# Crowsinc/LiveVisionKit

Measured on AMD Instinct MI355X. Metric: stabilized frames/sec (one 4K YUV420 stream per GPU, steady state), higher is better.
Workload: dtype f32

## Files before the change

include/lvk_hip.h:

```cpp
#ifndef LVK_HIP_H
#define LVK_HIP_H

#include <stdint.h>
#include <stddef.h>

#ifdef __cplusplus
extern "C" {
#endif

#define LVK_HIP_OK              0
#define LVK_HIP_ERR_ARG        -1
#define LVK_HIP_ERR_RUNTIME    -2
#define LVK_HIP_ERR_NO_DEVICE  -3

typedef struct lvk_hip_ctx lvk_hip_ctx;


int  lvk_hip_ctx_create(int device, lvk_hip_ctx** out);
int  lvk_hip_ctx_create_on_stream(int device, void* hip_stream, lvk_hip_ctx** out);
void lvk_hip_ctx_destroy(lvk_hip_ctx* ctx);
int  lvk_hip_sync(lvk_hip_ctx* ctx);
void* lvk_hip_stream(lvk_hip_ctx* ctx);
const char* lvk_hip_last_error(lvk_hip_ctx* ctx);
const char* lvk_hip_version(void);
// ... 154 lines not shown
int  lvk_hip_stab_push_yuv420_host(lvk_hip_stab* stab, const void* h_y, int y_step, const void* h_u, int u_step, const void* h_v, int v_step, int nv12,
                                   int rows, int cols, uint64_t timestamp,
                                   void* oh_y, int oy_step, void* oh_u, int ou_step, void* oh_v, int ov_step, int o_rows,
                                   int* produced, uint64_t* out_timestamp, lvk_frame_info* emitted);
int  lvk_hip_stab_push_obs_host(lvk_hip_stab* stab, int video_format,
                                const void* const h_planes[3], const int steps[3], int rows, int cols, uint64_t timestamp,
                                void* const oh_planes[3], const int o_steps[3], int o_rows,
                                int* produced, uint64_t* out_timestamp, lvk_frame_info* emitted);
int  lvk_hip_stab_prefetch_yuv420_host(lvk_hip_stab* stab, const void* h_y, int y_step, const void* h_u, int u_step, const void* h_v, int v_step,
                                       int nv12, int rows, int cols);
int  lvk_hip_stab_prefetch_cancel(lvk_hip_stab* stab);
int  lvk_hip_stab_set_overlap(lvk_hip_stab* stab, int enable);
int  lvk_hip_stab_set_bulk_context(lvk_hip_stab* stab, lvk_hip_ctx* bulk);
void* lvk_hip_stab_output_stream(lvk_hip_stab* stab);
int  lvk_hip_stab_set_remap_precision(lvk_hip_stab* stab, int precision);
int  lvk_hip_stab_get_remap_precision(const lvk_hip_stab* stab);


typedef struct lvk_deblock_settings
{
    uint32_t detection_levels;
    uint32_t block_size;
    uint32_t filter_size;
    float filter_scaling;
} lvk_deblock_settings;

typedef struct lvk_hip_deblock lvk_hip_deblock;

void lvk_hip_deblock_default_settings(lvk_deblock_settings* s);
int  lvk_hip_deblock_create(lvk_hip_ctx* ctx, const lvk_deblock_settings* settings, lvk_hip_deblock** out);
int  lvk_hip_deblock_configure(lvk_hip_deblock* deb, const lvk_deblock_settings* settings);
void lvk_hip_deblock_destroy(lvk_hip_deblock* deb);
int  lvk_hip_deblock_apply(lvk_hip_deblock* deb, void* d_frame, int step, int rows, int cols, int format, int region_xywh[4]);
int  lvk_hip_deblock_draw_influence(const lvk_hip_deblock* deb, void* d_frame, int step, int rows, int cols, int format);
int  lvk_hip_deblock_filter_region(const lvk_hip_deblock* deb, int region_xywh[4]);

int  lvk_hip_cas(lvk_hip_ctx* ctx, const void* d_src, int src_step, int rows, int cols, int format, void* d_dst, int dst_step, float sharpness);

int  lvk_hip_reformat(lvk_hip_ctx* ctx, const void* d_src, int src_step, int rows, int cols, int src_format, void* d_dst, int dst_step,
                      int dst_format);

int  lvk_hip_fsr_easu(lvk_hip_ctx* ctx, const void* d_src, int src_step, int rows, int cols, int format, const int region_xywh[4], void* d_dst,
                      int dst_step, int out_rows, int out_cols);
int  lvk_hip_fsr_geometry(int rows, int cols, int out_rows, int out_cols, float multiplier, int maintain_aspect_ratio, const int crop_ltrb[4],
                          int region_xywh[4], int out_rows_cols[2], int* skip);
int  lvk_hip_text_size(const char* text, int scale, int thickness, int wh[2], int* baseline);



int  lvk_hip_stab_prefetch(lvk_hip_stab* stab, const void* d_frame, int step, int rows, int cols, int format);
int  lvk_hip_stab_prefetch_yuv420(lvk_hip_stab* stab, const void* d_y, int y_step, const void* d_u, int u_step, const void* d_v, int v_step,
                                  int nv12, int rows, int cols);
long long lvk_hip_stab_lookahead_frames(lvk_hip_stab* stab);

int lvk_hip_remap_homography_gray(lvk_hip_ctx* ctx, const void* d_src, int src_step, int src_rows, int src_cols,
                                  void* d_dst, int dst_step, int dst_rows, int dst_cols, int off_x, int off_y, const float H[9], uint8_t bg);
int lvk_hip_remap_mesh_gray(lvk_hip_ctx* ctx, const void* d_src, int src_step, int src_rows, int src_cols, void* d_dst, int dst_step,
                            const float* mesh, int mesh_rows, int mesh_cols, uint8_t bg);
int lvk_hip_remap_map_gray(lvk_hip_ctx* ctx, const void* d_src, int src_step, int rows, int cols, void* d_dst, int dst_step,
                           const void* d_map, int map_step, uint8_t bg);
int lvk_hip_warpmesh_apply_gray(lvk_hip_ctx* ctx, const void* d_src, int src_step, int rows, int cols, void* d_dst, int dst_step,
                                const float* mesh, int mesh_rows, int mesh_cols, uint8_t bg);
int lvk_hip_warpmesh_apply_lens_gray(lvk_hip_ctx* ctx, const void* d_src, int src_step, int rows, int cols, void* d_dst, int dst_step,
                                     const float* mesh, int mesh_rows, int mesh_cols, uint8_t bg, const lvk_camera_params* lens);
int  lvk_hip_stab_push_gray(lvk_hip_stab* stab, const void* d_frame, int step, int rows, int cols, uint64_t timestamp,
                            void* d_out, int out_step, int out_rows, int* produced, uint64_t* out_timestamp, const void** released,
                            lvk_frame_info* emitted);
int  lvk_hip_stab_push_gray_host(lvk_hip_stab* stab, const void* h_frame, int step, int rows, int cols, uint64_t timestamp,
                                 void* oh_out, int out_step, int out_rows, int* produced, uint64_t* out_timestamp, lvk_frame_info* emitted);

int lvk_hip_remap_homography_c4(lvk_hip_ctx* ctx, const void* d_src, int src_step, int src_rows, int src_cols,
                                void* d_dst, int dst_step, int dst_rows, int dst_cols, int off_x, int off_y, const float H[9], const uint8_t bg[4]);
int lvk_hip_remap_mesh_c4(lvk_hip_ctx* ctx, const void* d_src, int src_step, int src_rows, int src_cols, void* d_dst, int dst_step,
                          const float* mesh, int mesh_rows, int mesh_cols, const uint8_t bg[4]);
int lvk_hip_remap_map_c4(lvk_hip_ctx* ctx, const void* d_src, int src_step, int rows, int cols, void* d_dst, int dst_step,
                         const void* d_map, int map_step, const uint8_t bg[4]);
int lvk_hip_warpmesh_apply_c4(lvk_hip_ctx* ctx, const void* d_src, int src_step, int rows, int cols, void* d_dst, int dst_step,
                              const float* mesh, int mesh_rows, int mesh_cols, const uint8_t bg[4]);
int lvk_hip_warpmesh_apply_lens_c4(lvk_hip_ctx* ctx, const void* d_src, int src_step, int rows, int cols, void* d_dst, int dst_step,
                                   const float* mesh, int mesh_rows, int mesh_cols, const uint8_t bg[4], const lvk_camera_params* lens);
int  lvk_hip_stab_set_background_alpha(lvk_hip_stab* stab, int alpha);
int  lvk_hip_stab_push_c4(lvk_hip_stab* stab, const void* d_frame, int step, int rows, int cols, uint64_t timestamp, int format,
                          void* d_out, int out_step, int out_rows, int* produced, uint64_t* out_timestamp, const void** released,
                          lvk_frame_info* emitted);
int  lvk_hip_stab_push_c4_host(lvk_hip_stab* stab, const void* h_frame, int step, int rows, int cols, uint64_t timestamp, int format,
                               void* oh_out, int out_step, int out_rows, int* produced, uint64_t* out_timestamp, lvk_frame_info* emitted);

int lvk_hip_upscale_gray(lvk_hip_ctx* ctx, const void* d_src, int src_step, int src_rows, int src_cols, void* d_dst, int dst_step, int dst_rows, int dst_cols);
int lvk_hip_upscale_c4(lvk_hip_ctx* ctx, const void* d_src, int src_step, int src_rows, int src_cols, void* d_dst, int dst_step, int dst_rows, int dst_cols);
int lvk_hip_sharpen_gray(lvk_hip_ctx* ctx, const void* d_src, int src_step, int rows, int cols, void* d_dst, int dst_step, float sharpness);
int lvk_hip_sharpen_c4(lvk_hip_ctx* ctx, const void* d_src, int src_step, int rows, int cols, void* d_dst, int dst_step, float sharpness);

int lvk_hip_cas_gray(lvk_hip_ctx* ctx, const void* d_src, int src_step, int rows, int cols, void* d_dst, int dst_step, float sharpness);
int lvk_hip_fsr_easu_gray(lvk_hip_ctx* ctx, const void* d_src, int src_step, int rows, int cols, const int region_xywh[4],
                          void* d_dst, int dst_step, int out_rows, int out_cols);
int lvk_hip_fsr_easu_gray_path(int rw, int rh, int out_rows, int out_cols);


#define LVK_SCHED_PUSH_FREE_RUNNING   0
#define LVK_SCHED_PUSH_SYNCHRONISED   1
#define LVK_SCHED_INGEST_ON_TRACKER   2
#define LVK_SCHED_INGEST_ON_BULK      3
#define LVK_SCHED_INGEST_INLINE       4
#define LVK_SCHED_REMAP_PERSISTENT    5
#define LVK_SCHED_REMAP_FULL          6
#define LVK_SCHED_WAIT_SIGNAL_WORD    7
#define LVK_SCHED_WAIT_EVENT          8
#define LVK_SCHED_WAIT_WORD_TIMEOUT   9
#define LVK_SCHED_COUNT              10
int  lvk_hip_stab_schedule_counters(lvk_hip_stab* stab, long long out[LVK_SCHED_COUNT], int reset);

int  lvk_hip_stab_get_stats(const lvk_hip_stab* stab, lvk_stab_stats* out);
int  lvk_hip_stab_detector_frames(const lvk_hip_stab* stab, long long* on_device, long long* on_host);
int  lvk_hip_stab_get_meshes(const lvk_hip_stab* stab, float* motion, float* correction, int cap_floats);
int  lvk_hip_stab_get_features(const lvk_hip_stab* stab, float* xy_resp_age, int cap);


#define LVK_STAGE_DOWNSCALE 0
#define LVK_STAGE_PYRAMID   1
#define LVK_STAGE_FAST      2
#define LVK_STAGE_PYRLK     3
#define LVK_STAGE_MOTION    4
#define LVK_STAGE_REMAP     5
#define LVK_STAGE_INGEST    6
#define LVK_STAGE_EGRESS    7
#define LVK_STAGE_COUNT     8
int  lvk_hip_stab_set_profiling(lvk_hip_stab* stab, int enable);
int  lvk_hip_stab_get_profile(lvk_hip_stab* stab, double total_ms[LVK_STAGE_COUNT], long long launches[LVK_STAGE_COUNT]);

int lvk_hip_native_rcp(lvk_hip_ctx* ctx, const float* d_in, float* d_out, size_t n);

typedef struct lvk_hip_mesh_solver lvk_hip_mesh_solver;
int  lvk_hip_mesh_solver_create(lvk_hip_ctx* ctx, int cols, int rows, float gen_region_w, float gen_region_h,
                                float temporal_smoothing, float local_smoothing, int max_points, lvk_hip_mesh_solver** out);
void lvk_hip_mesh_solver_destroy(lvk_hip_mesh_solver* solver);
int  lvk_hip_mesh_solver_reset(lvk_hip_mesh_solver* solver);
int  lvk_hip_mesh_solver_solve(lvk_hip_mesh_solver* solver, const float* tracked, const float* matched, int n, float region_w, float region_h,
                               float temporal_now, float threshold, uint8_t* inliers, float* offsets);

int lvk_hip_luma_area_resize(lvk_hip_ctx* ctx, const void* d_src, int src_step, int pix_stride, int channel,
                             int srows, int scols, void* d_dst, int dst_step, int drows, int dcols);

int lvk_hip_pyr_down(lvk_hip_ctx* ctx, const void* d_src, int src_step, int rows, int cols, void* d_dst, int dst_step);
int lvk_hip_scharr(lvk_hip_ctx* ctx, const void* d_src, int src_step, int rows, int cols, void* d_dst);

int lvk_hip_build_pyramid(lvk_hip_ctx* ctx, const void* d_img, int step, int rows, int cols, int max_level, int win_w, int win_h,
                          uint8_t* levels, int16_t* derivs, int* level_rows, int* level_cols);

int lvk_hip_fast_detect(lvk_hip_ctx* ctx, const void* d_img, int step, int rows, int cols,
                        const int* regions, int nregions, uint32_t* out, int cap, int* counts);

int lvk_hip_pyrlk(lvk_hip_ctx* ctx, const void* d_prev, int prev_step, const void* d_next, int next_step, int rows, int cols,
                  const float* prev_pts, int n, float* next_pts, uint8_t* status,
                  int win_w, int win_h, int max_level, int max_count, double epsilon, double min_eig_threshold);

int lvk_hip_estimate_global_motion(lvk_hip_ctx* ctx, const float* pts1, const float* pts2, int n, double threshold,
                                   double region_w, double region_h, int full_homography, double H[9], uint8_t* mask);

int lvk_hip_estimate_global_motion_lo(lvk_hip_ctx* ctx, const float* pts1, const float* pts2, int n, double threshold,
                                      double region_w, double region_h, int full_homography, int lo_mode, double H[9], uint8_t* mask,
                                      int lo_info[2]);

int lvk_hip_fast_filter(lvk_hip_ctx* ctx, const float* prev, const float* matched, const uint8_t* status, int n, float* out_prev, float* out_matched);

#define LVK_TRACK_CHAIN_GUARD 64
#define LVK_TRACK_CHAIN_FILL  0xA5
typedef struct lvk_track_chain_desc
{
    const float* prev; const float* matched; const uint8_t* status; const float* und;
    const void* d_prev_img; int prev_step; const void* d_next_img; int next_step; int rows, cols;
    int win_w, win_h, max_level, max_count; double epsilon, min_eig;
    const lvk_camera_params* lens; int lens_rows, lens_cols; double lens_sx, lens_sy;
    int n_bound, count_on_device, n_word;
    int full, model_on_device, full_word;
    int separate_compact, host_signal;
    double threshold; int region_w, region_h;
} lvk_track_chain_desc;
typedef struct lvk_track_chain_result
{
    double H[9]; int rc, signalled, count_dev, count_host;
    uint8_t* mask; float* pairs_dev; float* mirror_matched; uint8_t* mirror_status;
    float* next_pts; uint8_t* flow_status; float* flow_und;
} lvk_track_chain_result;
int lvk_hip_track_chain(lvk_hip_ctx* ctx, const lvk_track_chain_desc* desc, lvk_track_chain_result* result);

int lvk_hip_deblock_get_grid(lvk_hip_deblock* deb, uint8_t* mean, uint8_t* grid, float* keep_block, int capacity, int extent_xy[2]);


int lvk_hip_cas_const(float sharpness, float* peak);

int lvk_hip_cvt_code_target(int code, int src_format, int dcn);

int lvk_hip_fsr_easu_const(int rw, int rh, int W, int H, int ow, int oh, float con[16]);

int lvk_hip_fsr_easu_path(int rw, int rh, int out_rows, int out_cols);

enum
{
    LVK_AREA_PATH_FAST_DW_8x8_C3_BGR = 0, LVK_AREA_PATH_FAST_DW_8x8_C3_RGB = 1, LVK_AREA_PATH_FAST_DW_4x4_C3_BGR = 2, LVK_AREA_PATH_FAST_DW_4x4_C3_RGB = 3,
    LVK_AREA_PATH_FAST_DW_8x8_C3 = 4, LVK_AREA_PATH_FAST_DW_4x4_C3 = 5, LVK_AREA_PATH_FAST_DW_8x8_C1 = 6, LVK_AREA_PATH_FAST_DW_4x4_C1 = 7,
    LVK_AREA_PATH_FAST = 8, LVK_AREA_PATH_TILE_4 = 9, LVK_AREA_PATH_TILE_8 = 10, LVK_AREA_PATH_TAPS_4 = 11, LVK_AREA_PATH_TAPS_8 = 12,
    LVK_AREA_PATH_GENERAL = 13, LVK_AREA_PATH_ENLARGE = 14, LVK_AREA_PATH_COUNT = 15
};
int lvk_hip_area_resize_path(lvk_hip_ctx* ctx, const void* d_src, int src_step, int pix_stride, int channel,
// ... 25 lines not shown
```

livevisionkit_amd/_native.py:

```python
import ctypes
import os

_HERE = os.path.dirname(os.path.abspath(__file__))
LIB_PATH = os.environ.get("LVK_HIP_LIB") or os.path.join(_HERE, "liblvk_hip.so")

_c = ctypes
_P = _c.c_void_p
_SIG = {
    "lvk_hip_ctx_create": (_c.c_int, [_c.c_int, _c.POINTER(_P)]),
    "lvk_hip_ctx_create_on_stream": (_c.c_int, [_c.c_int, _P, _c.POINTER(_P)]),
    "lvk_hip_ctx_destroy": (None, [_P]),
    "lvk_hip_sync": (_c.c_int, [_P]),
    "lvk_hip_stream": (_P, [_P]),
    "lvk_hip_last_error": (_c.c_char_p, [_P]),
    "lvk_hip_version": (_c.c_char_p, []),
    "lvk_hip_abi_version": (_c.c_int, []),
    "lvk_hip_device_count": (_c.c_int, []),
    "lvk_hip_device_usable": (_c.c_int, [_c.c_int]),
    "lvk_hip_malloc": (_c.c_int, [_P, _c.c_size_t, _c.POINTER(_P)]),
    "lvk_hip_free": (_c.c_int, [_P, _P]),
    "lvk_hip_trim": (_c.c_int, [_P]),
    "lvk_hip_ctx_wait": (_c.c_int, [_P, _P]),
    "lvk_hip_upload": (_c.c_int, [_P, _P, _P, _c.c_size_t]),
    "lvk_hip_download": (_c.c_int, [_P, _P, _P, _c.c_size_t]),
# ... 17 lines not shown
    "lvk_hip_stab_set_remap_precision": (_c.c_int, [_P, _c.c_int]),
    "lvk_hip_stab_get_remap_precision": (_c.c_int, [_P]),
    "lvk_hip_remap_homography_c4": (_c.c_int, [_P, _P, _c.c_int, _c.c_int, _c.c_int, _P, _c.c_int, _c.c_int, _c.c_int,
                                               _c.c_int, _c.c_int, _c.POINTER(_c.c_float), _c.POINTER(_c.c_uint8)]),
    "lvk_hip_remap_mesh_c4": (_c.c_int, [_P, _P, _c.c_int, _c.c_int, _c.c_int, _P, _c.c_int, _c.POINTER(_c.c_float), _c.c_int, _c.c_int, _c.POINTER(_c.c_uint8)]),
    "lvk_hip_remap_map_c4": (_c.c_int, [_P, _P, _c.c_int, _c.c_int, _c.c_int, _P, _c.c_int, _P, _c.c_int, _c.POINTER(_c.c_uint8)]),
    "lvk_hip_warpmesh_apply_c4": (_c.c_int, [_P, _P, _c.c_int, _c.c_int, _c.c_int, _P, _c.c_int, _c.POINTER(_c.c_float), _c.c_int, _c.c_int, _c.POINTER(_c.c_uint8)]),
    "lvk_hip_warpmesh_apply_lens_c4": (_c.c_int, [_P, _P, _c.c_int, _c.c_int, _c.c_int, _P, _c.c_int, _c.POINTER(_c.c_float), _c.c_int, _c.c_int, _c.POINTER(_c.c_uint8), _P]),
    "lvk_hip_stab_set_background_alpha": (_c.c_int, [_P, _c.c_int]),
    "lvk_hip_stab_push_c4": (_c.c_int, [_P, _P, _c.c_int, _c.c_int, _c.c_int, _c.c_uint64, _c.c_int, _P, _c.c_int, _c.c_int,
                                        _c.POINTER(_c.c_int), _c.POINTER(_c.c_uint64), _c.POINTER(_P), _P]),
    "lvk_hip_stab_push_c4_host": (_c.c_int, [_P, _P, _c.c_int, _c.c_int, _c.c_int, _c.c_uint64, _c.c_int, _P, _c.c_int, _c.c_int,
                                             _c.POINTER(_c.c_int), _c.POINTER(_c.c_uint64), _P]),
    "lvk_hip_upscale": (_c.c_int, [_P, _P, _c.c_int, _c.c_int, _c.c_int, _P, _c.c_int, _c.c_int, _c.c_int, _c.c_int]),
    "lvk_hip_sharpen": (_c.c_int, [_P, _P, _c.c_int, _c.c_int, _c.c_int, _P, _c.c_int, _c.c_float]),
    "lvk_hip_upscale_gray": (_c.c_int, [_P, _P, _c.c_int, _c.c_int, _c.c_int, _P, _c.c_int, _c.c_int, _c.c_int]),
    "lvk_hip_upscale_c4": (_c.c_int, [_P, _P, _c.c_int, _c.c_int, _c.c_int, _P, _c.c_int, _c.c_int, _c.c_int]),
    "lvk_hip_sharpen_gray": (_c.c_int, [_P, _P, _c.c_int, _c.c_int, _c.c_int, _P, _c.c_int, _c.c_float]),
    "lvk_hip_sharpen_c4": (_c.c_int, [_P, _P, _c.c_int, _c.c_int, _c.c_int, _P, _c.c_int, _c.c_float]),
    "lvk_hip_native_rcp": (_c.c_int, [_P, _P, _P, _c.c_size_t]),
    "lvk_hip_mesh_solver_create": (_c.c_int, [_P, _c.c_int, _c.c_int, _c.c_float, _c.c_float, _c.c_float, _c.c_float, _c.c_int, _c.POINTER(_P)]),
    "lvk_hip_mesh_solver_destroy": (None, [_P]),
    "lvk_hip_mesh_solver_reset": (_c.c_int, [_P]),
    "lvk_hip_mesh_solver_solve": (_c.c_int, [_P, _c.POINTER(_c.c_float), _c.POINTER(_c.c_float), _c.c_int, _c.c_float, _c.c_float, _c.c_float, _c.c_float,
                                             _c.POINTER(_c.c_uint8), _c.POINTER(_c.c_float)]),
    "lvk_hip_lens_map_create": (_c.c_int, [_P, _P, _c.c_int, _c.c_int, _c.POINTER(_P), _c.POINTER(_c.c_int)]),
    "lvk_hip_lens_map_destroy": (_c.c_int, [_P, _P]),
    "lvk_hip_warpmesh_apply_lens": (_c.c_int, [_P, _P, _c.c_int, _c.c_int, _c.c_int, _P, _c.c_int, _c.POINTER(_c.c_float), _c.c_int, _c.c_int, _c.POINTER(_c.c_uint8), _c.c_int, _P]),
    "lvk_hip_lens_undistort_points": (_c.c_int, [_P, _P, _c.c_int, _c.c_int, _c.c_double, _c.c_double, _c.POINTER(_c.c_float), _c.c_int, _c.POINTER(_c.c_float)]),
    "lvk_hip_stab_set_lens": (_c.c_int, [_P, _P]),
    "lvk_hip_stab_output_stream": (_P, [_P]),
    "lvk_hip_fast_filter": (_c.c_int, [_P, _c.POINTER(_c.c_float), _c.POINTER(_c.c_float), _c.POINTER(_c.c_uint8), _c.c_int, _c.POINTER(_c.c_float), _c.POINTER(_c.c_float)]),
    "lvk_hip_stab_draw_trackers": (_c.c_int, [_P]),
    "lvk_hip_stab_draw_motion_mesh": (_c.c_int, [_P]),
    "lvk_hip_draw_grid": (_c.c_int, [_P, _P, _c.c_int, _c.c_int, _c.c_int, _c.c_int, _c.c_int, _c.POINTER(_c.c_uint8), _c.c_int]),
    "lvk_hip_draw_crosses": (_c.c_int, [_P, _P, _c.c_int, _c.c_int, _c.c_int, _c.POINTER(_c.c_float), _c.c_int, _c.c_float, _c.c_float,
                                        _c.POINTER(_c.c_uint8), _c.c_int, _c.c_int]),
    "lvk_hip_draw_points": (_c.c_int, [_P, _P, _c.c_int, _c.c_int, _c.c_int, _c.POINTER(_c.c_float), _c.c_int, _c.c_float, _c.c_float,
                                       _c.POINTER(_c.c_uint8), _c.c_int]),
    "lvk_hip_draw_rect": (_c.c_int, [_P, _P, _c.c_int, _c.c_int, _c.c_int, _c.POINTER(_c.c_int), _c.POINTER(_c.c_uint8), _c.c_int]),
    "lvk_hip_draw_text": (_c.c_int, [_P, _P, _c.c_int, _c.c_int, _c.c_int, _c.c_char_p, _c.c_int, _c.c_int, _c.POINTER(_c.c_uint8), _c.c_int, _c.c_int]),
    "lvk_hip_text_size": (_c.c_int, [_c.c_char_p, _c.c_int, _c.c_int, _c.POINTER(_c.c_int), _c.POINTER(_c.c_int)]),
    "lvk_hip_warpmesh_apply_yuv420": (_c.c_int, [_P, _P, _c.c_int, _c.c_int, _c.c_int, _P, _c.c_int, _P, _c.c_int, _P, _c.c_int, _c.c_int,
                                                 _c.POINTER(_c.c_float), _c.c_int, _c.c_int, _c.POINTER(_c.c_uint8)]),
    "lvk_hip_warpmesh_apply": (_c.c_int, [_P, _P, _c.c_int, _c.c_int, _c.c_int, _P, _c.c_int,
                                          _c.POINTER(_c.c_float), _c.c_int, _c.c_int, _c.POINTER(_c.c_uint8), _c.c_int]),
    "lvk_hip_luma_area_resize": (_c.c_int, [_P, _P, _c.c_int, _c.c_int, _c.c_int, _c.c_int, _c.c_int, _P, _c.c_int, _c.c_int, _c.c_int]),
    "lvk_hip_pyr_down": (_c.c_int, [_P, _P, _c.c_int, _c.c_int, _c.c_int, _P, _c.c_int]),
    "lvk_hip_scharr": (_c.c_int, [_P, _P, _c.c_int, _c.c_int, _c.c_int, _P]),
    "lvk_hip_build_pyramid": (_c.c_int, [_P, _P, _c.c_int, _c.c_int, _c.c_int, _c.c_int, _c.c_int, _c.c_int,
                                         _c.POINTER(_c.c_uint8), _c.POINTER(_c.c_int16), _c.POINTER(_c.c_int), _c.POINTER(_c.c_int)]),
    "lvk_hip_fast_detect": (_c.c_int, [_P, _P, _c.c_int, _c.c_int, _c.c_int, _c.POINTER(_c.c_int), _c.c_int,
                                       _c.POINTER(_c.c_uint32), _c.c_int, _c.POINTER(_c.c_int)]),
    "lvk_hip_pyrlk": (_c.c_int, [_P, _P, _c.c_int, _P, _c.c_int, _c.c_int, _c.c_int, _c.POINTER(_c.c_float), _c.c_int,
                                 _c.POINTER(_c.c_float), _c.POINTER(_c.c_uint8), _c.c_int, _c.c_int, _c.c_int, _c.c_int,
                                 _c.c_double, _c.c_double]),
    "lvk_hip_ingest_yuv420": (_c.c_int, [_P, _P, _c.c_int, _P, _c.c_int, _P, _c.c_int, _c.c_int, _c.c_int, _c.c_int, _P, _c.c_int]),
    "lvk_hip_egress_yuv420": (_c.c_int, [_P, _P, _c.c_int, _c.c_int, _c.c_int, _P, _c.c_int, _P, _c.c_int, _P, _c.c_int, _c.c_int]),
    "lvk_hip_ingest_obs": (_c.c_int, [_P, _c.c_int, _P * 3, _c.c_int * 3, _c.c_int, _c.c_int, _P, _c.c_int]),
    "lvk_hip_egress_obs": (_c.c_int, [_P, _c.c_int, _P, _c.c_int, _c.c_int, _c.c_int, _P * 3, _c.c_int * 3]),
    "lvk_hip_obs_frame_format": (_c.c_int, [_c.c_int]),
    "lvk_hip_estimate_global_motion": (_c.c_int, [_P, _c.POINTER(_c.c_float), _c.POINTER(_c.c_float), _c.c_int, _c.c_double,
                                                  _c.c_double, _c.c_double, _c.c_int, _c.POINTER(_c.c_double), _c.POINTER(_c.c_uint8)]),
    "lvk_hip_estimate_global_motion_lo": (_c.c_int, [_P, _c.POINTER(_c.c_float), _c.POINTER(_c.c_float), _c.c_int, _c.c_double,
                                                     _c.c_double, _c.c_double, _c.c_int, _c.c_int, _c.POINTER(_c.c_double), _c.POINTER(_c.c_uint8),
                                                     _c.POINTER(_c.c_int)]),
    "lvk_hip_track_chain": (_c.c_int, [_P, _P, _P]),
    "lvk_stab_default_settings": (None, [_P]),
    "lvk_hip_stab_create": (_c.c_int, [_P, _P, _c.POINTER(_P)]),
    "lvk_hip_stab_destroy": (None, [_P]),
    "lvk_hip_stab_configure": (_c.c_int, [_P, _P]),
    "lvk_hip_stab_restart": (_c.c_int, [_P]),
    "lvk_hip_stab_reset_context": (_c.c_int, [_P]),
    "lvk_hip_stab_ready": (_c.c_int, [_P]),
    "lvk_hip_stab_frame_delay": (_c.c_int, [_P]),
    "lvk_hip_stab_stable_region": (_c.c_int, [_P, _c.c_int, _c.c_int, _c.POINTER(_c.c_int)]),
    "lvk_hip_stab_next_output": (_c.c_int, [_P, _c.c_int, _c.c_int, _c.c_int, _P]),
    "lvk_hip_stab_push": (_c.c_int, [_P, _P, _c.c_int, _c.c_int, _c.c_int, _c.c_uint64, _c.c_int, _P, _c.c_int, _c.c_int,
                                     _c.POINTER(_c.c_int), _c.POINTER(_c.c_uint64), _c.POINTER(_P), _P]),
    "lvk_hip_stab_push_yuv420": (_c.c_int, [_P, _P, _c.c_int, _P, _c.c_int, _P, _c.c_int, _c.c_int, _c.c_int, _c.c_int, _c.c_uint64,
                                            _P, _c.c_int, _P, _c.c_int, _P, _c.c_int, _c.c_int, _c.POINTER(_c.c_int), _c.POINTER(_c.c_uint64), _P]),
    "lvk_hip_stab_push_obs": (_c.c_int, [_P, _c.c_int, _P * 3, _c.c_int * 3, _c.c_int, _c.c_int, _c.c_uint64, _P * 3, _c.c_int * 3, _c.c_int,
                                         _c.POINTER(_c.c_int), _c.POINTER(_c.c_uint64), _P]),
    "lvk_hip_stab_push_yuv420_host": (_c.c_int, [_P, _P, _c.c_int, _P, _c.c_int, _P, _c.c_int, _c.c_int, _c.c_int, _c.c_int, _c.c_uint64,
                                            _P, _c.c_int, _P, _c.c_int, _P, _c.c_int, _c.c_int, _c.POINTER(_c.c_int), _c.POINTER(_c.c_uint64), _P]),
    "lvk_hip_stab_push_obs_host": (_c.c_int, [_P, _c.c_int, _P * 3, _c.c_int * 3, _c.c_int, _c.c_int, _c.c_uint64, _P * 3, _c.c_int * 3, _c.c_int,
                                              _c.POINTER(_c.c_int), _c.POINTER(_c.c_uint64), _P]),
    "lvk_hip_stab_prefetch_yuv420_host": (_c.c_int, [_P, _P, _c.c_int, _P, _c.c_int, _P, _c.c_int, _c.c_int, _c.c_int, _c.c_int]),
    "lvk_hip_stab_prefetch_cancel": (_c.c_int, [_P]),
    "lvk_hip_stab_prefetch": (_c.c_int, [_P, _P, _c.c_int, _c.c_int, _c.c_int, _c.c_int]),
    "lvk_hip_stab_prefetch_yuv420": (_c.c_int, [_P, _P, _c.c_int, _P, _c.c_int, _P, _c.c_int, _c.c_int, _c.c_int, _c.c_int]),
    "lvk_hip_stab_lookahead_frames": (_c.c_longlong, [_P]),
    "lvk_hip_stab_schedule_counters": (_c.c_int, [_P, _c.POINTER(_c.c_longlong), _c.c_int]),
    "lvk_hip_stab_detector_frames": (_c.c_int, [_P, _c.POINTER(_c.c_longlong), _c.POINTER(_c.c_longlong)]),
    "lvk_hip_host_malloc": (_c.c_int, [_P, _c.c_size_t, _c.POINTER(_P)]),
    "lvk_hip_host_free": (_c.c_int, [_P, _P]),
    "lvk_hip_stab_get_stats": (_c.c_int, [_P, _P]),
    "lvk_hip_stab_get_meshes": (_c.c_int, [_P, _c.POINTER(_c.c_float), _c.POINTER(_c.c_float), _c.c_int]),
    "lvk_hip_stab_get_features": (_c.c_int, [_P, _c.POINTER(_c.c_float), _c.c_int]),
    "lvk_hip_stab_set_overlap": (_c.c_int, [_P, _c.c_int]),
    "lvk_hip_stab_set_bulk_context": (_c.c_int, [_P, _P]),
    "lvk_hip_stab_set_profiling": (_c.c_int, [_P, _c.c_int]),
    "lvk_hip_stab_get_profile": (_c.c_int, [_P, _c.POINTER(_c.c_double), _c.POINTER(_c.c_longlong)]),
    "lvk_hip_deblock_default_settings": (None, [_P]),
    "lvk_hip_deblock_create": (_c.c_int, [_P, _P, _c.POINTER(_P)]),
    "lvk_hip_deblock_configure": (_c.c_int, [_P, _P]),
    "lvk_hip_deblock_destroy": (None, [_P]),
    "lvk_hip_deblock_apply": (_c.c_int, [_P, _P, _c.c_int, _c.c_int, _c.c_int, _c.c_int, _c.POINTER(_c.c_int)]),
    "lvk_hip_deblock_draw_influence": (_c.c_int, [_P, _P, _c.c_int, _c.c_int, _c.c_int, _c.c_int]),
    "lvk_hip_deblock_filter_region": (_c.c_int, [_P, _c.POINTER(_c.c_int)]),
    "lvk_hip_deblock_get_grid": (_c.c_int, [_P, _c.POINTER(_c.c_uint8), _c.POINTER(_c.c_uint8), _c.POINTER(_c.c_float), _c.c_int, _c.POINTER(_c.c_int)]),
    "lvk_hip_cas": (_c.c_int, [_P, _P, _c.c_int, _c.c_int, _c.c_int, _c.c_int, _P, _c.c_int, _c.c_float]),
    "lvk_hip_cas_const": (_c.c_int, [_c.c_float, _c.POINTER(_c.c_float)]),
    "lvk_hip_reformat": (_c.c_int, [_P, _P, _c.c_int, _c.c_int, _c.c_int, _c.c_int, _P, _c.c_int, _c.c_int]),
    "lvk_hip_cvt_code_target": (_c.c_int, [_c.c_int, _c.c_int, _c.c_int]),
    "lvk_hip_fsr_easu": (_c.c_int, [_P, _P, _c.c_int, _c.c_int, _c.c_int, _c.c_int, _c.POINTER(_c.c_int), _P, _c.c_int, _c.c_int, _c.c_int]),
    "lvk_hip_fsr_geometry": (_c.c_int, [_c.c_int, _c.c_int, _c.c_int, _c.c_int, _c.c_float, _c.c_int, _c.POINTER(_c.c_int), _c.POINTER(_c.c_int),
                                        _c.POINTER(_c.c_int), _c.POINTER(_c.c_int)]),
    "lvk_hip_fsr_easu_const": (_c.c_int, [_c.c_int, _c.c_int, _c.c_int, _c.c_int, _c.c_int, _c.c_int, _c.POINTER(_c.c_float)]),
    "lvk_hip_fsr_easu_path": (_c.c_int, [_c.c_int, _c.c_int, _c.c_int, _c.c_int]),
    "lvk_hip_cas_gray": (_c.c_int, [_P, _P, _c.c_int, _c.c_int, _c.c_int, _P, _c.c_int, _c.c_float]),
    "lvk_hip_fsr_easu_gray": (_c.c_int, [_P, _P, _c.c_int, _c.c_int, _c.c_int, _c.POINTER(_c.c_int), _P, _c.c_int, _c.c_int, _c.c_int]),
    "lvk_hip_fsr_easu_gray_path": (_c.c_int, [_c.c_int, _c.c_int, _c.c_int, _c.c_int]),
    "lvk_hip_area_resize_path": (_c.c_int, [_P, _P, _c.c_int, _c.c_int, _c.c_int, _c.c_int, _c.c_int, _c.c_int, _c.c_int]),
    "lvk_hip_remap_map_yuv420": (_c.c_int, [_P, _P, _c.c_int, _c.c_int, _c.c_int, _P, _c.c_int, _P, _c.c_int, _P, _c.c_int, _c.c_int,
                                            _P, _c.c_int, _c.POINTER(_c.c_uint8)]),
    "lvk_hip_lens_create": (_c.c_int, [_P, _P, _c.c_int, _c.POINTER(_P)]),
    "lvk_hip_lens_configure": (_c.c_int, [_P, _P, _c.c_int]),
    "lvk_hip_lens_destroy": (None, [_P]),
    "lvk_hip_lens_view": (_c.c_int, [_P, _c.c_int, _c.c_int, _c.POINTER(_c.c_int)]),
    "lvk_hip_lens_apply": (_c.c_int, [_P, _P, _c.c_int, _c.c_int, _c.c_int, _c.c_int, _P, _c.c_int]),
    "lvk_hip_lens_apply_gray": (_c.c_int, [_P, _P, _c.c_int, _c.c_int, _c.c_int, _P, _c.c_int]),
    "lvk_hip_lens_apply_c4": (_c.c_int, [_P, _P, _c.c_int, _c.c_int, _c.c_int, _c.c_int, _P, _c.c_int]),
    "lvk_hip_lens_apply_yuv420": (_c.c_int, [_P, _P, _c.c_int, _P, _c.c_int, _P, _c.c_int, _P, _c.c_int, _P, _c.c_int, _P, _c.c_int,
                                             _c.c_int, _c.c_int, _c.c_int]),
}

_SIG_DEBLOCK_PX = {
    "lvk_hip_deblock_apply_gray": (_c.c_int, [_P, _P, _c.c_int, _c.c_int, _c.c_int, _c.POINTER(_c.c_int)]),
    "lvk_hip_deblock_apply_c4": (_c.c_int, [_P, _P, _c.c_int, _c.c_int, _c.c_int, _c.c_int, _c.POINTER(_c.c_int)]),
}

_SIG_DEBLOCK_420 = {
    "lvk_hip_deblock_apply_yuv420": (_c.c_int, [_P, _P, _c.c_int, _P, _c.c_int, _P, _c.c_int, _P, _c.c_int, _P, _c.c_int, _P, _c.c_int,
                                                _c.c_int, _c.c_int, _c.c_int, _c.POINTER(_c.c_int)]),
# ... 43 lines not shown
```

livevisionkit_amd/context.py:

```python
import ctypes

import numpy as np

from . import _native


class LvkHipError(RuntimeError):
    pass


def _f32(a):
    a = np.ascontiguousarray(a, dtype=np.float32)
    return a, a.ctypes.data_as(ctypes.POINTER(ctypes.c_float))


def _u8x3(bg):
    a = np.ascontiguousarray(bg, dtype=np.uint8).reshape(3)
    return a, a.ctypes.data_as(ctypes.POINTER(ctypes.c_uint8))


def _u8x4(bg):
    a = np.ascontiguousarray(bg, dtype=np.uint8).reshape(4)
    return a, a.ctypes.data_as(ctypes.POINTER(ctypes.c_uint8))

# ... 190 lines not shown
        return out

    def area_resize_path(self, frame, drows, dcols, channel=0):
        pix = frame.shape[2] if frame.dim() == 3 else 1
        path = self.lib.lvk_hip_area_resize_path(self.handle, frame.data_ptr(), frame.stride(0), pix, channel, frame.shape[0], frame.shape[1], drows, dcols)
        self._check(min(path, 0))
        return path

    def pyr_down(self, img, out=None):
        import torch
        if out is None:
            out = torch.empty(((img.shape[0] + 1) // 2, (img.shape[1] + 1) // 2), dtype=torch.uint8, device=img.device)
        self._check(self.lib.lvk_hip_pyr_down(self.handle, img.data_ptr(), img.stride(0), img.shape[0], img.shape[1],
                                              out.data_ptr(), out.stride(0)))
        return out

    def scharr(self, img, out=None):
        import torch
        if out is None:
            out = torch.empty((img.shape[0], img.shape[1], 2), dtype=torch.int16, device=img.device)
        self._check(self.lib.lvk_hip_scharr(self.handle, img.data_ptr(), img.stride(0), img.shape[0], img.shape[1], out.data_ptr()))
        return out

    def build_pyramid(self, img, max_level=3, win=(11, 11)):
        rows, cols = img.shape
        lv = np.zeros(rows * cols * 2, np.uint8); dv = np.zeros(rows * cols * 4, np.int16)
        lr = np.zeros(8, np.int32); lc = np.zeros(8, np.int32)
        n = self.lib.lvk_hip_build_pyramid(self.handle, img.data_ptr(), img.stride(0), rows, cols, max_level, win[0], win[1],
                                           lv.ctypes.data_as(ctypes.POINTER(ctypes.c_uint8)), dv.ctypes.data_as(ctypes.POINTER(ctypes.c_int16)),
                                           lr.ctypes.data_as(ctypes.POINTER(ctypes.c_int)), lc.ctypes.data_as(ctypes.POINTER(ctypes.c_int)))
        self._check(min(n, 0))
        out, lo, do = [], 0, 0
        for i in range(n):
            r, c = int(lr[i]), int(lc[i])
            out.append((lv[lo:lo + r * c].reshape(r, c).copy(), dv[do:do + r * c * 2].reshape(r, c, 2).copy()))
            lo += r * c; do += r * c * 2
        return out

    def fast_detect(self, img, regions, cap=None):
        rg = np.ascontiguousarray(regions, dtype=np.int32).reshape(-1, 6)
        n = rg.shape[0]
        cap = cap or int(max(1, (rg[:, 2] * rg[:, 3]).max()))
        out = np.zeros((n, cap), np.uint32)
        counts = np.zeros(n, np.int32)
        self._check(self.lib.lvk_hip_fast_detect(self.handle, img.data_ptr(), img.stride(0), img.shape[0], img.shape[1],
                                                 rg.ctypes.data_as(ctypes.POINTER(ctypes.c_int)), n,
                                                 out.ctypes.data_as(ctypes.POINTER(ctypes.c_uint32)), cap,
                                                 counts.ctypes.data_as(ctypes.POINTER(ctypes.c_int))))
        res = []
        for i in range(n):
            e = out[i, :min(cap, counts[i])]
            res.append(np.stack([e & 0xFFF, (e >> 12) & 0xFFF, e >> 24], axis=1).astype(np.int32))
        return res, counts

    def pyrlk(self, prev, nxt, pts, win=(11, 11), max_level=3, max_count=5, epsilon=0.01, min_eig=1e-4):
        pts = np.ascontiguousarray(pts, np.float32).reshape(-1, 2)
        out = np.zeros_like(pts)
        st = np.zeros(len(pts), np.uint8)
        self._check(self.lib.lvk_hip_pyrlk(self.handle, prev.data_ptr(), prev.stride(0), nxt.data_ptr(), nxt.stride(0),
                                           prev.shape[0], prev.shape[1],
                                           pts.ctypes.data_as(ctypes.POINTER(ctypes.c_float)), len(pts),
                                           out.ctypes.data_as(ctypes.POINTER(ctypes.c_float)),
                                           st.ctypes.data_as(ctypes.POINTER(ctypes.c_uint8)),
                                           win[0], win[1], max_level, max_count, float(epsilon), float(min_eig)))
        return out, st

    def estimate_global_motion(self, p1, p2, threshold, region=(480, 270), full_homography=True):
        p1 = np.ascontiguousarray(p1, np.float32).reshape(-1, 2); p2 = np.ascontiguousarray(p2, np.float32).reshape(-1, 2)
        H = np.zeros(9, np.float64); mask = np.zeros(len(p1), np.uint8)
        rc = self.lib.lvk_hip_estimate_global_motion(self.handle, p1.ctypes.data_as(ctypes.POINTER(ctypes.c_float)),
                                                     p2.ctypes.data_as(ctypes.POINTER(ctypes.c_float)), len(p1), float(threshold),
                                                     float(region[0]), float(region[1]), 1 if full_homography else 0,
                                                     H.ctypes.data_as(ctypes.POINTER(ctypes.c_double)),
                                                     mask.ctypes.data_as(ctypes.POINTER(ctypes.c_uint8)))
        if rc in (-1, -2, -3):
            self._check(rc)
        return rc, H.reshape(3, 3), mask

    def estimate_global_motion_lo(self, p1, p2, threshold, lo_mode, region=(480, 270), full_homography=True):
        p1 = np.ascontiguousarray(p1, np.float32).reshape(-1, 2); p2 = np.ascontiguousarray(p2, np.float32).reshape(-1, 2)
        H = np.zeros(9, np.float64); mask = np.zeros(len(p1), np.uint8); info = (ctypes.c_int * 2)(-1, -1)
        rc = self.lib.lvk_hip_estimate_global_motion_lo(self.handle, p1.ctypes.data_as(ctypes.POINTER(ctypes.c_float)),
                                                        p2.ctypes.data_as(ctypes.POINTER(ctypes.c_float)), len(p1), float(threshold),
                                                        float(region[0]), float(region[1]), 1 if full_homography else 0, int(lo_mode),
                                                        H.ctypes.data_as(ctypes.POINTER(ctypes.c_double)),
                                                        mask.ctypes.data_as(ctypes.POINTER(ctypes.c_uint8)), info)
        if rc in (-1, -2, -3):
            self._check(rc)
        return rc, H.reshape(3, 3), mask, info[0], info[1]

    def ingest_yuv420(self, y, u, v=None, out=None):
        import torch
        rows, cols = y.shape
        if out is None:
            out = torch.empty((rows, cols, 3), dtype=torch.uint8, device=y.device)
        nv12 = v is None
        self._check(self.lib.lvk_hip_ingest_yuv420(self.handle, *_planes420_args((y, u, v), nv12), 1 if nv12 else 0, rows, cols, out.data_ptr(), out.stride(0)))
        return out

    def egress_yuv420(self, frame, nv12=False, out=None):
        rows, cols = frame.shape[:2]
        if out is None:
            out = _planes420_empty(rows, cols, nv12, frame.device)
        y, u, v = out if not nv12 else (out[0], out[1], None)
        self._check(self.lib.lvk_hip_egress_yuv420(self.handle, frame.data_ptr(), frame.stride(0), rows, cols, *_planes420_args((y, u, v), nv12), 1 if nv12 else 0))
        return (y, u) if nv12 else (y, u, v)
# ... 252 lines not shown
```

livevisionkit_amd/csrc/fast.hip:

```cpp
#include "lvk_hip_internal.hpp"

namespace {

constexpr int TW = 64, TH = 8;
constexpr int AP = 4;
constexpr int IW = TW + 2 * AP, IH = TH + 2 * AP;
constexpr int SW = TW + 2, SH = TH + 2;

__device__ __forceinline__ int fast_score(const uint8_t* c, int stride, int threshold)
{
    const int v = c[0];
    int d[16];
    d[0] = v - c[3 * stride];          d[1] = v - c[1 + 3 * stride];   d[2] = v - c[2 + 2 * stride];   d[3] = v - c[3 + stride];
    d[4] = v - c[3];                   d[5] = v - c[3 - stride];       d[6] = v - c[2 - 2 * stride];   d[7] = v - c[1 - 3 * stride];
    d[8] = v - c[-3 * stride];         d[9] = v - c[-1 - 3 * stride];  d[10] = v - c[-2 - 2 * stride]; d[11] = v - c[-3 - stride];
    d[12] = v - c[-3];                 d[13] = v - c[-3 + stride];     d[14] = v - c[-2 + 2 * stride]; d[15] = v - c[-1 + 3 * stride];
    int lo2[16], hi2[16], lo4[16], hi4[16];
#pragma unroll
    for (int k = 0; k < 16; k++) { lo2[k] = min(d[k], d[(k + 1) & 15]); hi2[k] = max(d[k], d[(k + 1) & 15]); }
#pragma unroll
    for (int k = 0; k < 16; k++) { lo4[k] = min(lo2[k], lo2[(k + 2) & 15]); hi4[k] = max(hi2[k], hi2[(k + 2) & 15]); }
    int dark = -256, bright_neg = 256;
#pragma unroll
    for (int k = 0; k < 16; k++)
    {
        const int lo9 = min(min(lo4[k], lo4[(k + 4) & 15]), d[(k + 8) & 15]);
        const int hi9 = max(max(hi4[k], hi4[(k + 4) & 15]), d[(k + 8) & 15]);
        dark = max(dark, lo9);
        bright_neg = min(bright_neg, hi9);
    }
    const int m = max(dark, -bright_neg);
    return m > threshold ? m - 1 : 0;
}

struct FastRegionList { FastRegion r[LVK_FAST_INLINE_REGIONS]; };

struct FastCells { const uint16_t* col_of; const uint32_t* row_base; uint32_t* first; unsigned long long* best; int* region_count; };

__global__ __launch_bounds__(TW * TH)
void k_fast_detect(const uint8_t* __restrict__ img, int step, int rows, int cols,
                   const FastRegion* __restrict__ regions, FastRegionList inl, int n_inline, int segs_x,
                   unsigned long long* __restrict__ masks, uint8_t* __restrict__ scores, int max_rh, int max_rw, FastCells cells)
{
    LVK_TRACKER_PRIORITY();
    const FastRegion rg = n_inline ? inl.r[blockIdx.z] : regions[blockIdx.z];
    if (!rg.active) return;
    const int lx0 = blockIdx.x * TW, ly0 = blockIdx.y * TH;
    if (lx0 >= rg.w || ly0 >= rg.h) return;

    __shared__ uint8_t s_img[IH][IW];
    __shared__ uint8_t s_score[SH][SW];
    const int tid = threadIdx.y * TW + threadIdx.x;

    for (int i = tid; i < IW * IH; i += TW * TH)
    {
        const int ty = i / IW, tx = i - ty * IW;
        const int gx = min(max(rg.x + lx0 - AP + tx, 0), cols - 1);
        const int gy = min(max(rg.y + ly0 - AP + ty, 0), rows - 1);
        s_img[ty][tx] = img[(long)gy * step + gx];
    }
    __shared__ uint32_t s_cell_col[TW], s_cell_row[TH];
    if (cells.first)
    {
        if (tid < TW) s_cell_col[tid] = cells.col_of[min(rg.x + lx0 + tid, cols - 1)];
        else if (tid < TW + TH) s_cell_row[tid - TW] = cells.row_base[min(rg.y + ly0 + tid - TW, rows - 1)];
    }
    __syncthreads();

    for (int i = tid; i < SW * SH; i += TW * TH)
    {
        const int ty = i / SW, tx = i - ty * SW;
        const int lx = lx0 - 1 + tx, ly = ly0 - 1 + ty;
        int s = 0;
        if (lx >= 3 && lx < rg.w - 3 && ly >= 3 && ly < rg.h - 3)
            s = fast_score(&s_img[ty + AP - 1][tx + AP - 1], IW, rg.threshold);
        s_score[ty][tx] = (uint8_t)s;
    }
    __syncthreads();

    const int lx = lx0 + threadIdx.x, ly = ly0 + threadIdx.y;
    const int sx = threadIdx.x + 1, sy = threadIdx.y + 1;
    const int s = s_score[sy][sx];
    const bool keep = s > 0 &&
        s > s_score[sy][sx - 1] && s > s_score[sy][sx + 1] &&
        s > s_score[sy - 1][sx - 1] && s > s_score[sy - 1][sx] && s > s_score[sy - 1][sx + 1] &&
        s > s_score[sy + 1][sx - 1] && s > s_score[sy + 1][sx] && s > s_score[sy + 1][sx + 1];
    const unsigned long long mask = __ballot(keep);
    if (ly < rg.h)
    {
        if (threadIdx.x == 0) masks[((long)blockIdx.z * max_rh + ly) * segs_x + blockIdx.x] = mask;
        if (threadIdx.x == 0 && cells.first && mask) atomicAdd(&cells.region_count[blockIdx.z], __popcll(mask));
        if (keep) scores[((long)blockIdx.z * max_rh + ly) * max_rw + lx] = (uint8_t)s;
        if (keep && cells.first)
        {
            const uint32_t ci = s_cell_row[threadIdx.y] + s_cell_col[threadIdx.x];
            const uint32_t key = (uint32_t)(((int)blockIdx.z * max_rh + ly) * max_rw + lx);
            atomicMin(&cells.first[ci], key);
            const uint32_t rec = (uint32_t)(rg.x + lx) | ((uint32_t)(rg.y + ly) << 12) | ((uint32_t)s << 24);
            atomicMax(&cells.best[ci], ((unsigned long long)(((uint32_t)s << 24) | (0xFFFFFFu - key)) << 32) | rec);
        }
    }
}

__global__ __launch_bounds__(1024)
void k_fast_compact(const FastRegion* __restrict__ regions, FastRegionList inl, int n_inline, int segs_x,
                    const unsigned long long* __restrict__ masks, const uint8_t* __restrict__ scores, int max_rh, int max_rw,
                    uint32_t* __restrict__ out, int cap, int* __restrict__ counts)
{
    LVK_TRACKER_PRIORITY();
    const int r = blockIdx.x;
    const FastRegion rg = n_inline ? inl.r[r] : regions[r];
    if (!rg.active) { if (threadIdx.x == 0) counts[r] = 0; return; }
    const int rsegs = (rg.w + TW - 1) / TW;
    const int nseg = rg.h * rsegs;
    __shared__ int s_wave[16];
    __shared__ int s_base;
    if (threadIdx.x == 0) s_base = 0;
    __syncthreads();
    const int lane = threadIdx.x & 63, wave = threadIdx.x >> 6;
    for (int chunk = 0; chunk < nseg; chunk += 1024)
    {
        const int seg = chunk + threadIdx.x;
        int ly = 0, sg = 0;
        unsigned long long m = 0;
        if (seg < nseg)
        {
            ly = seg / rsegs; sg = seg - ly * rsegs;
            m = masks[((long)r * max_rh + ly) * segs_x + sg];
        }
        const int cnt = __popcll(m);
        int incl = cnt;
#pragma unroll
        for (int o = 1; o < 64; o <<= 1) { const int t = __shfl_up(incl, o); if (lane >= o) incl += t; }
        if (lane == 63) s_wave[wave] = incl;
        __syncthreads();
        int wave_off = 0;
        for (int w = 0; w < wave; w++) wave_off += s_wave[w];
        int pos = s_base + wave_off + incl - cnt;
        while (m)
        {
            const int bit = __ffsll((long long)m) - 1;
            m &= m - 1;
            const int lx = sg * TW + bit;
            if (pos < cap)
                out[(long)r * cap + pos] = (uint32_t)lx | ((uint32_t)ly << 12) | ((uint32_t)scores[((long)r * max_rh + ly) * max_rw + lx] << 24);
            pos++;
        }
        __syncthreads();
        if (threadIdx.x == 1023) s_base = s_base + wave_off + incl;
        __syncthreads();
    }
    if (threadIdx.x == 0) counts[r] = s_base;
}


struct FastInsertArgs
{
    const uint8_t* bucket;
    uint32_t* first; unsigned long long* best;
    int* region_count;
    int capacity, small_grid, n_held, min_samples; float uniformity, homography_threshold;
    int nkeys;
    float2* pts;
    uint32_t* new_kp;
    int* result;
    int* d_n; int* d_full;
    int* counts;
    uint32_t occ[128];
    int occ_bucket[16];
};

constexpr int INS_NT = 1024, INS_MAX_CELLS = 4096, INS_CPT = INS_MAX_CELLS / INS_NT, INS_MAX_KEYS = 1 << 18;

__host__ __device__ inline size_t ins_lds_bytes(int nkeys) { const size_t words = ((size_t)nkeys + 31) / 32; return words * 4 + ((words + 1) & ~(size_t)1) * 2; }

__global__ __launch_bounds__(INS_NT)
void k_fast_insert(int nregions, FastInsertArgs a)
{
    LVK_TRACKER_PRIORITY();
    extern __shared__ __attribute__((aligned(16))) uint8_t ins_smem[];
    const int bwords = (a.nkeys + 31) / 32;
    uint32_t* s_bits = reinterpret_cast<uint32_t*>(ins_smem);
    unsigned short* s_pre = reinterpret_cast<unsigned short*>(s_bits + bwords);
    __shared__ int s_wave[INS_NT / 64], s_bucket[16], s_count[LVK_FAST_INLINE_REGIONS];
    __shared__ uint32_t s_occ[INS_MAX_CELLS / 32];
    const int t = threadIdx.x, lane = t & 63, wave = t >> 6;

    uint32_t f[INS_CPT]; unsigned long long bk[INS_CPT]; uint32_t bu[INS_CPT];
#pragma unroll
    for (int k = 0; k < INS_CPT; k++)
    {
        const int ci = t + k * INS_NT;
        f[k] = ci < a.capacity ? a.first[ci] : 0xFFFFFFFFu;
        bk[k] = ci < a.capacity ? a.best[ci] : 0ull;
        bu[k] = ci < a.capacity ? a.bucket[ci] : 0u;
    }
    const int my_count = t < nregions ? a.region_count[t] : 0;
#pragma unroll 1
    for (int i = t; i < bwords; i += INS_NT) s_bits[i] = 0u;
    if (t < INS_MAX_CELLS / 32) s_occ[t] = a.occ[t];
    if (t < LVK_FAST_INLINE_REGIONS) s_count[t] = my_count;
    if (t < nregions && my_count) a.region_count[t] = 0;
    if (t < 16) s_bucket[t] = a.occ_bucket[t];
    __syncthreads();

#pragma unroll
    for (int k = 0; k < INS_CPT; k++)
    {
        const int ci = t + k * INS_NT;
        if (ci < a.capacity && f[k] != 0xFFFFFFFFu)
        {
            a.first[ci] = 0xFFFFFFFFu; a.best[ci] = 0ull;
            if ((s_occ[ci >> 5] >> (ci & 31)) & 1u) f[k] = 0xFFFFFFFFu;
            else { atomicOr(&s_bits[f[k] >> 5], 1u << (f[k] & 31)); atomicAdd(&s_bucket[bu[k] & 15u], 1); }
        }
    }
    __syncthreads();
    const int wpt = (bwords + INS_NT - 1) / INS_NT, wb0 = t * wpt, wb1 = min(wb0 + wpt, bwords);
    int mine = 0;
#pragma unroll 1
    for (int w = wb0; w < wb1; w++) mine += __popc(s_bits[w]);
    int incl = mine;
#pragma unroll
    for (int o = 1; o < 64; o <<= 1) { const int u = __shfl_up(incl, o); if (lane >= o) incl += u; }
    if (lane == 63) s_wave[wave] = incl;
    __syncthreads();
    int base = 0, n_new = 0;
#pragma unroll 2
    for (int q = 0; q < INS_NT / 64; q++) { const int u = s_wave[q]; n_new += u; if (q < wave) base += u; }
    int run = base + incl - mine;
#pragma unroll 1
    for (int w = wb0; w < wb1; w++) { s_pre[w] = (unsigned short)run; run += __popc(s_bits[w]); }
    __syncthreads();

#pragma unroll
    for (int k = 0; k < INS_CPT; k++)
        if (f[k] != 0xFFFFFFFFu)
        {
            const uint32_t w = f[k] >> 5, bit = f[k] & 31;
            const int pos = (int)s_pre[w] + __popc(s_bits[w] & ((1u << bit) - 1u));
            const uint32_t rec = (uint32_t)bk[k];
            a.pts[a.n_held + pos] = make_float2((float)(rec & 0xFFFu), (float)((rec >> 12) & 0xFFFu));
            a.new_kp[pos] = rec;
        }

    if (t < nregions) a.counts[t] = s_count[t];
    if (t == 0)
    {
        int m_used = 0;
        for (int b = 0; b < 16; b++) m_used += s_bucket[b];
        float q = 1.0f;
        if (m_used != 0)
        {
            if (a.small_grid) q = (float)m_used / (float)a.capacity;
            else
            {
                const int ideal = (int)((float)m_used / 16.0f);
                int excess = 0;
                for (int b = 0; b < 16; b++) excess += max(s_bucket[b] - ideal, 0);
                q = 1.0f - ((float)excess / (float)(m_used - ideal));
            }
        }
        int total = 0;
        for (int r = 0; r < nregions; r++) total += s_count[r];
        const int n_total = a.n_held + n_new;
        const int n_eff = (n_total < a.min_samples || q < a.uniformity) ? 0 : n_total;
        const int full = q > a.homography_threshold ? 1 : 0;
        a.result[0] = n_new; a.result[1] = n_eff; a.result[2] = __float_as_int(q); a.result[3] = full; a.result[4] = total;
        *a.d_n = n_eff; *a.d_full = full;
    }
}

}

int lvk_fast_workspace_bytes(int nregions, int max_rw, int max_rh, size_t* masks_bytes, size_t* scores_bytes)
{
    const int segs_x = (max_rw + TW - 1) / TW;
    *masks_bytes = (size_t)nregions * max_rh * segs_x * sizeof(unsigned long long);
    *scores_bytes = (size_t)nregions * max_rh * max_rw;
    return segs_x;
}

int lvk_launch_fast(lvk_hip_ctx* ctx, const void* d_img, int step, int rows, int cols,
                    const FastRegion* d_regions, int nregions, int max_rw, int max_rh,
                    void* d_masks, void* d_scores, uint32_t* d_out, int cap, int* d_counts, const FastRegion* host_regions)
{
    LVK_HIP_REQUIRE(ctx, d_img && d_regions && nregions > 0 && max_rw > 0 && max_rh > 0 && max_rw < 4096 && max_rh < 4096);
    const int segs_x = (max_rw + TW - 1) / TW;
    const dim3 block(TW, TH), grid(segs_x, (max_rh + TH - 1) / TH, nregions);
    FastRegionList inl{};
    const int n_inline = (host_regions && nregions <= LVK_FAST_INLINE_REGIONS) ? nregions : 0;
    for (int i = 0; i < n_inline; i++) inl.r[i] = host_regions[i];
    hipLaunchKernelGGL(k_fast_detect, grid, block, 0, ctx->stream, (const uint8_t*)d_img, step, rows, cols, d_regions, inl, n_inline, segs_x,
                       (unsigned long long*)d_masks, (uint8_t*)d_scores, max_rh, max_rw, FastCells{});
    hipLaunchKernelGGL(k_fast_compact, dim3(nregions), dim3(1024), 0, ctx->stream, d_regions, inl, n_inline, segs_x,
                       (const unsigned long long*)d_masks, (const uint8_t*)d_scores, max_rh, max_rw, d_out, cap, d_counts);
    LVK_HIP_CHECK(ctx, hipGetLastError());
    return LVK_HIP_OK;
}


int lvk_launch_fast_insert(lvk_hip_ctx* ctx, const void* d_img, int step, int rows, int cols, const FastRegion* host_regions, int nregions,
                           int max_rw, int max_rh, void* d_masks, void* d_scores, const FastInsertDesc& d)
{
    LVK_HIP_REQUIRE(ctx, d_img && host_regions && nregions > 0 && nregions <= LVK_FAST_INLINE_REGIONS && max_rw > 0 && max_rh > 0);
    LVK_HIP_REQUIRE(ctx, lvk_fast_insert_fits(d.capacity, nregions, max_rw, max_rh, cols, rows));
    LVK_HIP_REQUIRE(ctx, d.pts && d.new_kp && d.result && d.d_n && d.d_full && d.counts && d.occ && d.cell_first && d.cell_best && d.region_count && d.occ_bucket && d.col_of && d.row_base && d.bucket);
    const int segs_x = (max_rw + TW - 1) / TW;
    FastRegionList inl{};
    for (int i = 0; i < nregions; i++) inl.r[i] = host_regions[i];
    const int nkeys = nregions * max_rh * max_rw;
    const size_t lds = ins_lds_bytes(nkeys);
    if (lds > 48 * 1024)
        LVK_HIP_CHECK(ctx, hipFuncSetAttribute(reinterpret_cast<const void*>(k_fast_insert), hipFuncAttributeMaxDynamicSharedMemorySize, (int)lds));
    const dim3 block(TW, TH), grid(segs_x, (max_rh + TH - 1) / TH, nregions);
    hipLaunchKernelGGL(k_fast_detect, grid, block, 0, ctx->stream, (const uint8_t*)d_img, step, rows, cols, (const FastRegion*)nullptr, inl, nregions, segs_x,
                       (unsigned long long*)d_masks, (uint8_t*)d_scores, max_rh, max_rw, FastCells{d.col_of, d.row_base, d.cell_first, (unsigned long long*)d.cell_best, d.region_count});
    FastInsertArgs a{d.bucket, d.cell_first, (unsigned long long*)d.cell_best, d.region_count, d.capacity, d.small_grid ? 1 : 0, d.n_held, d.min_samples, d.uniformity, d.homography_threshold, nkeys,
                     d.pts, d.new_kp, d.result, d.d_n, d.d_full, d.counts, {}, {}};
    for (int i = 0; i < (d.capacity + 31) / 32; i++) a.occ[i] = d.occ[i];
    for (int i = 0; i < 16; i++) a.occ_bucket[i] = d.occ_bucket[i];
    hipLaunchKernelGGL(k_fast_insert, dim3(1), dim3(INS_NT), lds, ctx->stream, nregions, a);
    LVK_HIP_CHECK(ctx, hipGetLastError());
    return LVK_HIP_OK;
}

bool lvk_fast_insert_fits(int cells, int nregions, int max_rw, int max_rh, int cols, int rows)
{
    if (!(cells > 0 && cells <= INS_MAX_CELLS && nregions > 0 && nregions <= LVK_FAST_INLINE_REGIONS && cols < 4096 && rows < 4096 && max_rw < 4096 && max_rh < 4096)) return false;
    const long nkeys = (long)nregions * max_rh * max_rw;
    return nkeys <= INS_MAX_KEYS && ins_lds_bytes((int)nkeys) <= 60 * 1024;
}
int lvk_fast_cells_reset(lvk_hip_ctx* ctx, uint32_t* d_first, void* d_best, int cells, int* d_region_count)
{
    LVK_HIP_CHECK(ctx, hipMemsetAsync(d_region_count, 0, LVK_FAST_INLINE_REGIONS * sizeof(int), ctx->stream));
    LVK_HIP_CHECK(ctx, hipMemsetAsync(d_first, 0xFF, (size_t)cells * sizeof(uint32_t), ctx->stream));
    LVK_HIP_CHECK(ctx, hipMemsetAsync(d_best, 0, (size_t)cells * sizeof(unsigned long long), ctx->stream));
    return LVK_HIP_OK;
}

extern "C" {

int lvk_hip_fast_detect(lvk_hip_ctx* ctx, const void* d_img, int step, int rows, int cols,
                        const int* regions, int nregions, uint32_t* out, int cap, int* counts)
{
    LVK_HIP_ENTRY(ctx);
    LVK_HIP_REQUIRE(ctx, regions && out && counts && nregions > 0 && cap > 0 && rows > 0 && cols > 0 && step >= cols);
    std::vector<FastRegion> rg((size_t)nregions);
    int max_rw = 1, max_rh = 1;
    for (int i = 0; i < nregions; i++)
    {
        rg[i] = FastRegion{regions[6 * i], regions[6 * i + 1], regions[6 * i + 2], regions[6 * i + 3], regions[6 * i + 4], regions[6 * i + 5]};
        LVK_HIP_REQUIRE(ctx, rg[i].x >= 0 && rg[i].y >= 0 && rg[i].w > 0 && rg[i].h > 0 && rg[i].x + rg[i].w <= cols && rg[i].y + rg[i].h <= rows);
        max_rw = std::max(max_rw, rg[i].w); max_rh = std::max(max_rh, rg[i].h);
    }
    size_t mb, sb;
    lvk_fast_workspace_bytes(nregions, max_rw, max_rh, &mb, &sb);
    void *d_masks = nullptr, *d_scores = nullptr, *d_regions = nullptr; uint32_t* d_out = nullptr; int* d_counts = nullptr;
    LVK_HIP_CHECK(ctx, hipMalloc(&d_masks, mb));
    LVK_HIP_CHECK(ctx, hipMalloc(&d_scores, sb));
    LVK_HIP_CHECK(ctx, hipMalloc(&d_regions, rg.size() * sizeof(FastRegion)));
    LVK_HIP_CHECK(ctx, hipMalloc((void**)&d_out, (size_t)nregions * cap * sizeof(uint32_t)));
    LVK_HIP_CHECK(ctx, hipMalloc((void**)&d_counts, nregions * sizeof(int)));
    LVK_HIP_CHECK(ctx, hipMemcpyAsync(d_regions, rg.data(), rg.size() * sizeof(FastRegion), hipMemcpyHostToDevice, ctx->stream));
    int rc = lvk_launch_fast(ctx, d_img, step, rows, cols, (const FastRegion*)d_regions, nregions, max_rw, max_rh, d_masks, d_scores, d_out, cap, d_counts);
    if (rc == LVK_HIP_OK)
    {
        LVK_HIP_CHECK(ctx, hipMemcpyAsync(out, d_out, (size_t)nregions * cap * sizeof(uint32_t), hipMemcpyDeviceToHost, ctx->stream));
        LVK_HIP_CHECK(ctx, hipMemcpyAsync(counts, d_counts, nregions * sizeof(int), hipMemcpyDeviceToHost, ctx->stream));
        LVK_HIP_CHECK(ctx, hipStreamSynchronize(ctx->stream));
    }
    (void)hipFree(d_masks); (void)hipFree(d_scores); (void)hipFree(d_regions); (void)hipFree(d_out); (void)hipFree(d_counts);
    return rc;
}

}
```

livevisionkit_amd/csrc/host_logic.hpp:

```cpp
#pragma once

#include <cmath>
#include <cstdint>
#include <cstddef>
#include <vector>
#include <deque>
#include <algorithm>

#include "lvk_hip.h"
#include "lvk/WarpMeshCore.hpp"

namespace lvkh {

inline int cv_round(float v) { return (int)lrintf(v); }

struct Feature { float x, y, response; int age; };

using WarpMeshF = lvk::detail::WarpMeshF;

inline bool perspective_transform(const float src[8], const float dst[8], double M[9])
{
    double A[8][8], B[8];
    for (int i = 0; i < 4; i++)
    {
// ... 92 lines not shown
        m_kd.resize(n);
        double total = 0;
        for (size_t i = 0; i < n; i++) { const double x = (double)i - (double)(n - 1) * 0.5; m_kd[i] = std::exp(s2 * x * x); total += m_kd[i]; }
        total = 1. / total;

        float weight = 1.0f;
        m_trace = m_path.front();
        for (size_t i = 1; i < n; i++)
        {
            weight -= (float)(m_kd[i - 1] * total);
            m_trace.scale_add(m_path[i], weight);
        }
        WarpMeshF corr = m_trace;
        corr -= m_position;

        float drift = 0.0f;
        for (size_t i = 0; i + 1 < corr.off.size(); i += 2)
        {
            drift = std::max(drift, std::fabs(corr.off[i]) / m_margin_x);
            drift = std::max(drift, std::fabs(corr.off[i + 1]) / m_margin_y);
        }
        if (drift > 1.0f) { corr.clamp(m_margin_x, m_margin_y); drift = 1.0f; }

        const double d = (double)drift;
        const double target = d >= 0.7 ? 0.0 : (d <= 0.3 ? (double)m_steps : d);
        m_factor = m_factor + m_rate * (target - m_factor);
        return corr;
    }

    void restart()
    {
        for (WarpMeshF& m : m_path) m.set_identity();
        m_position.set_identity();
        m_trace.set_identity();
    }

    const WarpMeshF& scene_crop() const { return m_crop; }
    double smoothing_factor() const { return m_factor; }
    void margins(float out[4]) const { out[0] = m_margin_x; out[1] = m_margin_y; out[2] = m_margin_w; out[3] = m_margin_h; }

private:
    size_t centre() const { return (m_path.size() - 1) / 2; }
    bool m_configured = false;
    std::deque<WarpMeshF> m_path;
    WarpMeshF m_trace, m_position, m_crop;
    double m_factor = 0.0, m_base = 0.0;
    float m_margin_x = 0, m_margin_y = 0, m_margin_w = 1, m_margin_h = 1, m_steps = 20.0f, m_rate = 0.04f;
    std::vector<double> m_kd;
};

class FeatureGridH
{
public:
    struct Zone { float x, y, w, h; int threshold; size_t load; bool ran; };

    void configure(const lvk_stab_settings& s)
    {
        m_w = s.detection_width; m_h = s.detection_height;
        const int gc = cv_round((float)m_w * s.max_feature_density), gr = cv_round((float)m_h * s.max_feature_density);
        if (gc != m_gc || gr != m_gr || m_cells.empty()) { m_gc = gc; m_gr = gr; m_cells.assign((size_t)gc * gr, -1); m_used = 0; m_used_cells.clear(); }
        m_cw = (float)m_w / (float)m_gc; m_ch = (float)m_h / (float)m_gr;
        m_bucket.assign((size_t)m_gc * m_gr, 0);
        if (m_gc > 4 && m_gr > 4)
        {
            const float sw = (float)m_gc / 4.0f, sh = (float)m_gr / 4.0f;
            for (int y = 0; y < m_gr; y++)
                for (int x = 0; x < m_gc; x++) m_bucket[(size_t)y * m_gc + x] = (uint8_t)((size_t)((float)y / sh) * 4 + (size_t)((float)x / sw));
        }
        m_zc = s.detection_regions_x; m_zr = s.detection_regions_y;
        m_zw = (float)m_w / (float)m_zc; m_zh = (float)m_h / (float)m_zr;
        m_icw = 1.0 / (double)m_cw; m_ich = 1.0 / (double)m_ch; m_izw = 1.0 / (double)m_zw; m_izh = 1.0 / (double)m_zh;
        m_col_of.resize((size_t)m_w); m_row_of.resize((size_t)m_h);
        for (int x = 0; x < m_w; x++) m_col_of[(size_t)x] = (uint16_t)(size_t)((float)x / m_cw);
        for (int y = 0; y < m_h; y++) m_row_of[(size_t)y] = (uint16_t)(size_t)((float)y / m_ch);
        m_row_base.resize((size_t)m_h);
        for (int y = 0; y < m_h; y++) m_row_base[(size_t)y] = (uint32_t)m_row_of[(size_t)y] * (uint32_t)m_gc;
        held.reserve(capacity()); m_used_cells.reserve(capacity());
        zones.clear();
        for (int r = 0; r < m_zr; r++)
            for (int c = 0; c < m_zc; c++)
                zones.push_back(Zone{(float)c * m_zw, (float)r * m_zh, m_zw, m_zh, 10 , 0, false});
        const float per_zone = (float)((size_t)m_gc * m_gr) / (float)(m_zc * m_zr);
        m_min_load = (size_t)(per_zone * (s.min_feature_density / s.max_feature_density));
        m_target = (size_t)(s.accumulation_rate * per_zone);
        m_force = s.force_detection != 0;
    }

    size_t capacity() const { return (size_t)m_gc * m_gr; }

    void plan(std::vector<FastRegion>& out)
    {
        out.resize(zones.size());
        for (size_t i = 0; i < zones.size(); i++)
        {
            Zone& z = zones[i];
            z.ran = m_force || z.load <= m_min_load;
            out[i] = FastRegion{cv_round(z.x), cv_round(z.y), cv_round(z.w), cv_round(z.h), z.threshold, z.ran ? 1 : 0};
        }
    }

    void absorb(size_t zone, const uint32_t* kp, int count)
    {
        Zone& z = zones[zone];
        const bool integral = z.x == std::floor(z.x) && z.y == std::floor(z.y) && z.x >= 0.0f && z.y >= 0.0f;
        int i = 0;
        if (integral && z.x < 65536.0f && z.y < 65536.0f)
        {
            const unsigned zx = (unsigned)z.x, zy = (unsigned)z.y, w = (unsigned)m_col_of.size(), h = (unsigned)m_row_of.size();
            const uint16_t* col_of = m_col_of.data(); const uint32_t* row_base = m_row_base.data();
            long* cells = m_cells.data();
            for (; i < count; i++)
            {
                const uint32_t k = kp[i];
                const unsigned xi = (k & 0xFFFu) + zx, yi = ((k >> 12) & 0xFFFu) + zy;
                if (xi >= w || yi >= h) break;
                const uint32_t ci = row_base[yi] + col_of[xi];
                const float response = (float)(k >> 24);
                const long cell = cells[ci];
                if (cell < 0)
                {
                    cells[ci] = (long)held.size(); m_used++; m_used_cells.push_back(ci);
                    held.push_back(Feature{(float)xi, (float)yi, response, 0});
                }
                else
                {
                    Feature& best = held[(size_t)cell];
                    if (response > best.response && best.age <= 0) best = Feature{(float)xi, (float)yi, response, 0};
                }
            }
        }
        for (; i < count; i++)
        {
            Feature f{(float)(kp[i] & 0xFFFu) + z.x, (float)((kp[i] >> 12) & 0xFFFu) + z.y, (float)(kp[i] >> 24), 0};
            const size_t xi = (size_t)f.x, yi = (size_t)f.y;
            const size_t ci = (integral && xi < m_col_of.size() && yi < m_row_of.size()) ? (size_t)m_row_of[yi] * (size_t)m_gc + m_col_of[xi] : cell_of(f.x, f.y);
            long& cell = m_cells[ci];
            if (cell < 0) { cell = (long)held.size(); m_used++; m_used_cells.push_back((uint32_t)(&cell - m_cells.data())); held.push_back(f); }
            else if (f.response > held[(size_t)cell].response && held[(size_t)cell].age <= 0) held[(size_t)cell] = f;
        }
        feedback(z, (size_t)count);
    }

    void feedback(Zone& z, size_t n) const
    {
        if (n > m_target + 150) z.threshold = std::min(z.threshold + 5, 250);
        else if (n < m_target - 150) z.threshold = z.threshold > 10 ? std::max(z.threshold - 5, 10) : std::min(z.threshold + 5, 10);
    }

    static constexpr int kDeviceMaxCells = 4096;
    size_t used_cells() const { return m_used; }
    int grid_cols() const { return m_gc; }
// ... 169 lines not shown
```

livevisionkit_amd/csrc/imgproc.hip:

```cpp
#include "lvk_hip_internal.hpp"

#include <cmath>
#include <algorithm>

namespace {

__device__ __forceinline__ int reflect101(int p, int len)
{
    if (len == 1) return 0;
    while (p < 0 || p >= len) { p = (p < 0) ? -p : 2 * (len - 1) - p; }
    return p;
}

__device__ __forceinline__ uint8_t sat_u8_rint(float v)
{
    const float r = __builtin_rintf(v);
    return (uint8_t)(int)__builtin_fminf(__builtin_fmaxf(r, 0.0f), 255.0f);
}

__device__ __forceinline__ int gray_of(const uint8_t* __restrict__ p, int channel)
{
    if (channel >= 0) return p[channel];
    const int b = channel == -1 ? p[0] : p[2], g = p[1], r = channel == -1 ? p[2] : p[0];
    return (b * 3735 + g * 19235 + r * 9798 + (1 << 14)) >> 15;
}

__global__ __launch_bounds__(256)
void k_area_fast(const uint8_t* __restrict__ src, int src_step, int pix_stride, int channel,
                 uint8_t* __restrict__ dst, int dst_step, int drows, int dcols, int sx, int sy)
{
    LVK_TRACKER_PRIORITY();
    const int x = blockIdx.x * 64 + threadIdx.x;
    const int y = blockIdx.y * 4 + threadIdx.y;
    if (x >= dcols || y >= drows) return;
    const uint8_t* p = src + (long)(y * sy) * src_step + (long)(x * sx) * pix_stride;
    int sum = 0;
    for (int ky = 0; ky < sy; ky++, p += src_step)
        for (int kx = 0; kx < sx; kx++)
            sum += gray_of(p + kx * pix_stride, channel);
    uint8_t out;
    if (sx == 2 && sy == 2) out = (uint8_t)((sum + 2) >> 2);
    else out = sat_u8_rint((float)sum * (1.f / (float)(sx * sy)));
    dst[(long)y * dst_step + x] = out;
}

__global__ __launch_bounds__(256)
void k_area_enlarge(const uint8_t* __restrict__ src, int src_step, int pix_stride, int channel,
                    uint8_t* __restrict__ dst, int dst_step, int drows, int dcols, const int4* __restrict__ xtab, const int4* __restrict__ ytab)
{
    LVK_TRACKER_PRIORITY();
    const int x = blockIdx.x * 64 + threadIdx.x;
    const int y = blockIdx.y * 4 + threadIdx.y;
    if (x >= dcols || y >= drows) return;
    const int4 tx = xtab[x], ty = ytab[y];
    const uint8_t* r0 = src + (long)ty.x * src_step; const uint8_t* r1 = src + (long)ty.y * src_step;
    const int h0 = gray_of(r0 + (long)tx.x * pix_stride, channel) * tx.z + gray_of(r0 + (long)tx.y * pix_stride, channel) * tx.w;
    const int h1 = gray_of(r1 + (long)tx.x * pix_stride, channel) * tx.z + gray_of(r1 + (long)tx.y * pix_stride, channel) * tx.w;
    dst[(long)y * dst_step + x] = (uint8_t)((((ty.z * (h0 >> 4)) >> 16) + ((ty.w * (h1 >> 4)) >> 16) + 2) >> 2);
}

template <int SX, int SY, int PIX, int MODE = 0>
__global__ __launch_bounds__(256)
void k_area_fast_dw(const uint8_t* __restrict__ src, int src_step, uint8_t* __restrict__ dst, int dst_step, int drows, int dcols)
{
    LVK_TL(0);
// ... 143 lines not shown
    float sum = 0.0f;
#pragma unroll
    for (int j = 0; j < MAXT; j++)
    {
        float buf = 0.0f;
#pragma unroll
        for (int k = 0; k < MAXT; k++) buf = buf + (float)tile[ys[j] + xs[k]] * xw[k];
        sum = sum + yw[j] * buf;
    }
    dst[(long)y * dst_step + x] = sat_u8_rint(sum);
}

__global__ __launch_bounds__(256)
void k_pyr_down(const uint8_t* __restrict__ src, int src_step, int rows, int cols,
                uint8_t* __restrict__ dst, int dst_step, int drows, int dcols)
{
    const int x = blockIdx.x * 64 + threadIdx.x;
    const int y = blockIdx.y * 4 + threadIdx.y;
    if (x >= dcols || y >= drows) return;
    int xi[5];
#pragma unroll
    for (int k = 0; k < 5; k++) xi[k] = reflect101(2 * x - 2 + k, cols);
    int acc = 0;
#pragma unroll
    for (int ky = 0; ky < 5; ky++)
    {
        const uint8_t* row = src + (long)reflect101(2 * y - 2 + ky, rows) * src_step;
        const int h = row[xi[0]] + row[xi[4]] + 4 * (row[xi[1]] + row[xi[3]]) + 6 * row[xi[2]];
        const int w = (ky == 0 || ky == 4) ? 1 : (ky == 2 ? 6 : 4);
        acc += w * h;
    }
    dst[(long)y * dst_step + x] = (uint8_t)((acc + 128) >> 8);
}

__global__ __launch_bounds__(256)
void k_scharr(const uint8_t* __restrict__ src, int src_step, int rows, int cols, short2* __restrict__ dst)
{
    const int x = blockIdx.x * 64 + threadIdx.x;
    const int y = blockIdx.y * 4 + threadIdx.y;
    if (x >= cols || y >= rows) return;
    const uint8_t* r0 = src + (long)(y > 0 ? y - 1 : (rows > 1 ? 1 : 0)) * src_step;
    const uint8_t* r1 = src + (long)y * src_step;
    const uint8_t* r2 = src + (long)(y < rows - 1 ? y + 1 : (rows > 1 ? rows - 2 : 0)) * src_step;
    const int xm = x > 0 ? x - 1 : (cols > 1 ? 1 : 0);
    const int xp = x < cols - 1 ? x + 1 : (cols > 1 ? cols - 2 : 0);
    const int t0m = (r0[xm] + r2[xm]) * 3 + r1[xm] * 10, t0p = (r0[xp] + r2[xp]) * 3 + r1[xp] * 10;
    const int t1m = r2[xm] - r0[xm], t1c = r2[x] - r0[x], t1p = r2[xp] - r0[xp];
    short2 o;
    o.x = (short)(t0p - t0m);
    o.y = (short)((t1p + t1m) * 3 + t1c * 10);
    dst[(long)y * cols + x] = o;
}

constexpr int T3 = 4;
constexpr int F2 = 2 * (T3 - 1) + 5, F1 = 2 * (F2 - 1) + 5, F0 = 2 * (F1 - 1) + 5;
constexpr int F0P = F0 + 3, F1P = F1 + 3, F2P = F2 + 1;

__device__ __forceinline__ int pyr_tap(const uint8_t* t, int pitch, int ox, int oy, int x, int y, int cols, int rows)
{
    int xi[5];
#pragma unroll
    for (int k = 0; k < 5; k++) xi[k] = reflect101(2 * x - 2 + k, cols) - ox;
    int acc = 0;
#pragma unroll
    for (int ky = 0; ky < 5; ky++)
    {
        const uint8_t* row = t + (reflect101(2 * y - 2 + ky, rows) - oy) * pitch;
        const int h = row[xi[0]] + row[xi[4]] + 4 * (row[xi[1]] + row[xi[3]]) + 6 * row[xi[2]];
        acc += ((ky == 0 || ky == 4) ? 1 : (ky == 2 ? 6 : 4)) * h;
    }
    return (acc + 128) >> 8;
}

__global__ __launch_bounds__(256)
void k_pyr_fused3(PyrArgs a)
{
    LVK_TL(1);
    LVK_TRACKER_PRIORITY();
    __shared__ uint8_t t0[F0 * F0P], t1[F1 * F1P], t2[F2 * F2P];
    const int tid = threadIdx.x;
    const int x3 = blockIdx.x * T3, y3 = blockIdx.y * T3;
    const int o2x = 2 * x3 - 2, o2y = 2 * y3 - 2, o1x = 2 * o2x - 2, o1y = 2 * o2y - 2, o0x = 2 * o1x - 2, o0y = 2 * o1y - 2;
    const PyrLevel L0 = a.lv[0], L1 = a.lv[1], L2 = a.lv[2], L3 = a.lv[3];

    {
        constexpr int N0 = (F0 * F0 + 255) / 256;
        uint8_t v[N0];
#pragma unroll
        for (int k = 0; k < N0; k++)
        {
            const int i = min(tid + 256 * k, F0 * F0 - 1);
            const int ty = i / F0, tx = i - ty * F0;
            const int gx = min(max(o0x + tx, 0), L0.cols - 1), gy = min(max(o0y + ty, 0), L0.rows - 1);
            v[k] = L0.img[(long)gy * L0.step + gx];
        }
#pragma unroll
        for (int k = 0; k < N0; k++)
        {
            const int i = tid + 256 * k;
            const int ty = i / F0, tx = i - ty * F0;
            const int gx = o0x + tx, gy = o0y + ty;
            if (i < F0 * F0 && gx >= 0 && gy >= 0 && gx < L0.cols && gy < L0.rows) t0[ty * F0P + tx] = v[k];
        }
    }
    __syncthreads();
    for (int i = tid; i < F1 * F1; i += 256)
    {
        const int ty = i / F1, tx = i - ty * F1;
        const int gx = o1x + tx, gy = o1y + ty;
        if (gx >= 0 && gy >= 0 && gx < L1.cols && gy < L1.rows)
        {
            const int v = pyr_tap(t0, F0P, o0x, o0y, gx, gy, L0.cols, L0.rows);
            t1[ty * F1P + tx] = (uint8_t)v;
            if (gx >= 4 * x3 && gx < 4 * x3 + 4 * T3 && gy >= 4 * y3 && gy < 4 * y3 + 4 * T3)
                const_cast<uint8_t*>(L1.img)[(long)gy * L1.step + gx] = (uint8_t)v;
        }
    }
    __syncthreads();
    for (int i = tid; i < F2 * F2; i += 256)
    {
        const int ty = i / F2, tx = i - ty * F2;
        const int gx = o2x + tx, gy = o2y + ty;
        if (gx >= 0 && gy >= 0 && gx < L2.cols && gy < L2.rows)
        {
            const int v = pyr_tap(t1, F1P, o1x, o1y, gx, gy, L1.cols, L1.rows);
            t2[ty * F2P + tx] = (uint8_t)v;
            if (gx >= 2 * x3 && gx < 2 * x3 + 2 * T3 && gy >= 2 * y3 && gy < 2 * y3 + 2 * T3)
                const_cast<uint8_t*>(L2.img)[(long)gy * L2.step + gx] = (uint8_t)v;
        }
    }
    __syncthreads();
    if (tid < T3 * T3)
    {
        const int gx = x3 + (tid % T3), gy = y3 + (tid / T3);
        if (gx < L3.cols && gy < L3.rows)
            const_cast<uint8_t*>(L3.img)[(long)gy * L3.step + gx] = (uint8_t)pyr_tap(t2, F2P, o2x, o2y, gx, gy, L2.cols, L2.rows);
    }
}

__global__ __launch_bounds__(256)
void k_scharr_all(PyrArgs a)
{
    const PyrLevel L = a.lv[blockIdx.z];
    const int x = blockIdx.x * 64 + threadIdx.x;
    const int y = blockIdx.y * 4 + threadIdx.y;
    if (x >= L.cols || y >= L.rows) return;
    const int rows = L.rows, cols = L.cols;
    const uint8_t* r0 = L.img + (long)(y > 0 ? y - 1 : (rows > 1 ? 1 : 0)) * L.step;
    const uint8_t* r1 = L.img + (long)y * L.step;
    const uint8_t* r2 = L.img + (long)(y < rows - 1 ? y + 1 : (rows > 1 ? rows - 2 : 0)) * L.step;
    const int xm = x > 0 ? x - 1 : (cols > 1 ? 1 : 0);
    const int xp = x < cols - 1 ? x + 1 : (cols > 1 ? cols - 2 : 0);
    const int t0m = (r0[xm] + r2[xm]) * 3 + r1[xm] * 10, t0p = (r0[xp] + r2[xp]) * 3 + r1[xp] * 10;
    const int t1m = r2[xm] - r0[xm], t1c = r2[x] - r0[x], t1p = r2[xp] - r0[xp];
    short2 o;
    o.x = (short)(t0p - t0m);
    o.y = (short)((t1p + t1m) * 3 + t1c * 10);
    const_cast<short2*>(L.deriv)[(long)y * cols + x] = o;
}

void build_area_tab(int ssize, int dsize, std::vector<int2>& range, std::vector<AreaTabEntry>& tab)
{
    const double scale = (double)ssize / dsize;
    range.resize(dsize);
    tab.clear();
    for (int dx = 0; dx < dsize; dx++)
    {
        const int start = (int)tab.size();
        const double fsx1 = dx * scale, fsx2 = fsx1 + scale;
        const double cell = std::min(scale, ssize - fsx1);
        int sx1 = (int)std::ceil(fsx1), sx2 = (int)std::floor(fsx2);
        sx2 = std::min(sx2, ssize - 1);
        sx1 = std::min(sx1, sx2);
        if (sx1 - fsx1 > 1e-3) tab.push_back({sx1 - 1, (float)((sx1 - fsx1) / cell)});
        for (int sx = sx1; sx < sx2; sx++) tab.push_back({sx, (float)(1.0 / cell)});
        if (fsx2 - sx2 > 1e-3) tab.push_back({sx2, (float)(std::min(std::min(fsx2 - sx2, 1.0), cell) / cell)});
        range[dx] = make_int2(start, (int)tab.size() - start);
    }
}

void build_enlarge_tab(int ssize, int dsize, bool horizontal, std::vector<int4>& tab)
{
    const double inv = (double)dsize / ssize, scale = 1. / inv;
    auto to_short = [](float v) -> int { const long r = lrintf(v); return (int)(r < -32768 ? -32768 : r > 32767 ? 32767 : r); };
    tab.resize((size_t)dsize);
    bool tail = false;
    for (int d = 0; d < dsize; d++)
    {
        int s0 = (int)std::floor(d * scale);
        float f = (float)((d + 1) - (s0 + 1) * inv);
// ... 113 lines not shown
    case LVK_AREA_PATH_FAST_DW_8x8_C3:     LVK_AREA_DW(8, 8, 3, 0); break;
    case LVK_AREA_PATH_FAST_DW_4x4_C3:     LVK_AREA_DW(4, 4, 3, 0); break;
    case LVK_AREA_PATH_FAST_DW_8x8_C1:     LVK_AREA_DW(8, 8, 1, 0); break;
    case LVK_AREA_PATH_FAST_DW_4x4_C1:     LVK_AREA_DW(4, 4, 1, 0); break;
    case LVK_AREA_PATH_FAST:
        hipLaunchKernelGGL(k_area_fast, grid, block, 0, ctx->stream, src, src_step, pix_stride, channel, dst, dst_step, drows, dcols, scols / dcols, srows / drows);
        break;
    case LVK_AREA_PATH_TILE_4:  LVK_AREA_TABS(k_area_general_tile<4>, scols); break;
    case LVK_AREA_PATH_TILE_8:  LVK_AREA_TABS(k_area_general_tile<8>, scols); break;
    case LVK_AREA_PATH_TAPS_4:  LVK_AREA_TABS(k_area_general_taps<4>, pix_stride, channel); break;
    case LVK_AREA_PATH_TAPS_8:  LVK_AREA_TABS(k_area_general_taps<8>, pix_stride, channel); break;
    case LVK_AREA_PATH_GENERAL: LVK_AREA_TABS(k_area_general, pix_stride, channel); break;
    case LVK_AREA_PATH_ENLARGE:
    {
        const int4 *xt, *yt;
        int rc;
        if ((rc = lvk_get_enlargetab(ctx, scols, dcols, true, &xt)) != LVK_HIP_OK) return rc;
        if ((rc = lvk_get_enlargetab(ctx, srows, drows, false, &yt)) != LVK_HIP_OK) return rc;
        hipLaunchKernelGGL(k_area_enlarge, grid, block, 0, ctx->stream, src, src_step, pix_stride, channel, dst, dst_step, drows, dcols, xt, yt);
        break;
    }
    default: return ctx->fail(LVK_HIP_ERR_ARG, "no such downscale form");
    }
#undef LVK_AREA_DW
#undef LVK_AREA_TABS
    LVK_HIP_CHECK(ctx, hipGetLastError());
    return LVK_HIP_OK;
}

int lvk_launch_pyr_down(lvk_hip_ctx* ctx, const void* d_src, int src_step, int rows, int cols, void* d_dst, int dst_step)
{
    LVK_HIP_REQUIRE(ctx, d_src && d_dst && rows > 0 && cols > 0);
    const int drows = (rows + 1) / 2, dcols = (cols + 1) / 2;
    LVK_HIP_REQUIRE(ctx, src_step >= cols && dst_step >= dcols);
    const dim3 block(64, 4), grid((dcols + 63) / 64, (drows + 3) / 4);
    hipLaunchKernelGGL(k_pyr_down, grid, block, 0, ctx->stream, (const uint8_t*)d_src, src_step, rows, cols, (uint8_t*)d_dst, dst_step, drows, dcols);
    LVK_HIP_CHECK(ctx, hipGetLastError());
    return LVK_HIP_OK;
}

int lvk_launch_scharr(lvk_hip_ctx* ctx, const void* d_src, int src_step, int rows, int cols, void* d_dst)
{
    LVK_HIP_REQUIRE(ctx, d_src && d_dst && rows > 0 && cols > 0 && src_step >= cols);
    const dim3 block(64, 4), grid((cols + 63) / 64, (rows + 3) / 4);
    hipLaunchKernelGGL(k_scharr, grid, block, 0, ctx->stream, (const uint8_t*)d_src, src_step, rows, cols, (short2*)d_dst);
    LVK_HIP_CHECK(ctx, hipGetLastError());
    return LVK_HIP_OK;
}

int lvk_launch_pyramid(lvk_hip_ctx* ctx, const PyrArgs& args, bool derivs)
{
    int rc;
    if (args.nlevels == 4)
    {
        const dim3 grid((args.lv[3].cols + T3 - 1) / T3, (args.lv[3].rows + T3 - 1) / T3);
        hipLaunchKernelGGL(k_pyr_fused3, grid, dim3(256), 0, ctx->stream, args);
    }
    else
        for (int i = 1; i < args.nlevels; i++)
            if ((rc = lvk_launch_pyr_down(ctx, args.lv[i - 1].img, args.lv[i - 1].step, args.lv[i - 1].rows, args.lv[i - 1].cols,
                                          const_cast<uint8_t*>(args.lv[i].img), args.lv[i].step)) != LVK_HIP_OK) return rc;
    if (derivs)
    {
        const dim3 sgrid((args.lv[0].cols + 63) / 64, (args.lv[0].rows + 3) / 4, args.nlevels);
        hipLaunchKernelGGL(k_scharr_all, sgrid, dim3(64, 4), 0, ctx->stream, args);
    }
    LVK_HIP_CHECK(ctx, hipGetLastError());
    return LVK_HIP_OK;
}

extern "C" {

int lvk_hip_luma_area_resize(lvk_hip_ctx* ctx, const void* d_src, int src_step, int pix_stride, int channel,
                             int srows, int scols, void* d_dst, int dst_step, int drows, int dcols)
{
    LVK_HIP_ENTRY(ctx);
    return lvk_launch_luma_area_resize(ctx, d_src, src_step, pix_stride, channel, srows, scols, d_dst, dst_step, drows, dcols);
}

int lvk_hip_area_resize_path(lvk_hip_ctx* ctx, const void* d_src, int src_step, int pix_stride, int channel, int srows, int scols, int drows, int dcols)
{
    LVK_HIP_ENTRY(ctx);
    AreaTabs t;
    return lvk_area_resize_path(ctx, d_src, src_step, pix_stride, channel, srows, scols, drows, dcols, &t);
}

int lvk_hip_pyr_down(lvk_hip_ctx* ctx, const void* d_src, int src_step, int rows, int cols, void* d_dst, int dst_step)
{
    LVK_HIP_ENTRY(ctx);
    return lvk_launch_pyr_down(ctx, d_src, src_step, rows, cols, d_dst, dst_step);
}

int lvk_hip_scharr(lvk_hip_ctx* ctx, const void* d_src, int src_step, int rows, int cols, void* d_dst)
{
    LVK_HIP_ENTRY(ctx);
    return lvk_launch_scharr(ctx, d_src, src_step, rows, cols, d_dst);
}

}

LVK_TL_EXPORT(imgproc)
```

livevisionkit_amd/csrc/lvk_hip_internal.hpp:

```cpp
#pragma once

#include <hip/hip_runtime.h>
#include <cstdint>
#include <cstdio>
#include <string>
#include <vector>
#include <functional>
#include <map>
#include <set>
#include <mutex>
#include <utility>

#include "lvk_hip.h"
#include "planes420.hpp"

struct LinTabEntry { int s0, s1; float a0, a1; };
struct Lin8Entry { int s0, s1, a0, a1; };
struct AreaTabEntry { int si; float alpha; };
struct FastRegion { int x, y, w, h, threshold, active; };
constexpr int LVK_FAST_INLINE_REGIONS = 8;

constexpr int LVK_MAX_PYR_LEVELS = 8;
struct PyrLevel { const uint8_t* img; const short2* deriv; int rows, cols, step; };
struct PyrArgs { PyrLevel lv[LVK_MAX_PYR_LEVELS]; int nlevels; };
// ... 98 lines not shown
        }
    }
};
#define LVK_TL(slot) LvkTimelineScope lvk_tl_scope_(slot)
#define LVK_TL_EXPORT(unit)                                                                                     \
    extern "C" int lvk_tl_read_##unit(long long* out)                                                           \
    {                                                                                                           \
        unsigned idx[LVK_TL_SLOTS];                                                                             \
        if (hipDeviceSynchronize() != hipSuccess) return -1;                                                    \
        if (hipMemcpyFromSymbol(idx, HIP_SYMBOL(lvk_tl_head), sizeof(idx)) != hipSuccess) return -1;           \
        for (int s = 0; s < LVK_TL_SLOTS; s++) out[(size_t)s * (1 + 2 * LVK_TL_RING)] = idx[s];                 \
        for (int s = 0; s < LVK_TL_SLOTS; s++)                                                                  \
            if (hipMemcpyFromSymbol(out + (size_t)s * (1 + 2 * LVK_TL_RING) + 1, HIP_SYMBOL(lvk_tl_log), sizeof(long long) * 2 * LVK_TL_RING, \
                                    sizeof(long long) * 2 * LVK_TL_RING * s) != hipSuccess) return -1;         \
        return 0;                                                                                               \
    }
#else
#define LVK_TL(slot) do { } while (0)
#define LVK_TL_EXPORT(unit)
#endif

#define LVK_HIP_REQUIRE(ctx, cond)                                                                    \
    do { if (!(cond)) return (ctx)->fail(LVK_HIP_ERR_ARG, "pre-condition failed: " #cond); } while (0)

inline int lvk_format_channels(int format)
{
    switch (format)
    {
    case LVK_FORMAT_BGR: case LVK_FORMAT_RGB: case LVK_FORMAT_YUV: return 3;
    case LVK_FORMAT_BGRA: case LVK_FORMAT_RGBA: return 4;
    case LVK_FORMAT_GRAY: return 1;
    default: return 0;
    }
}

inline bool lvk_pitched_overlap(const void* a, int a_step, int a_rows, long long a_row_bytes, const void* b, int b_step, int b_rows, long long b_row_bytes)
{
    return yuv420::overlap(yuv420::span_of(a, a_step, a_rows, a_row_bytes), yuv420::span_of(b, b_step, b_rows, b_row_bytes));
}

int lvk_stage_params(lvk_hip_ctx* ctx, hipStream_t stream, const void* host, size_t bytes, void** d_out, int* slot = nullptr);
int lvk_stage_consumed(lvk_hip_ctx* ctx, int slot, hipStream_t stream);

int lvk_get_lintab(lvk_hip_ctx* ctx, int msize, int fsize, bool vertical, const LinTabEntry** d_out);

int lvk_get_areatab(lvk_hip_ctx* ctx, int ssize, int dsize, const int2** d_range, const AreaTabEntry** d_tab, int* max_taps = nullptr, int* span64 = nullptr, int* span4 = nullptr);

int lvk_launch_luma_area_resize(lvk_hip_ctx* ctx, const void* d_src, int src_step, int pix_stride, int channel,
                                int srows, int scols, void* d_dst, int dst_step, int drows, int dcols);
int lvk_launch_pyr_down(lvk_hip_ctx* ctx, const void* d_src, int src_step, int rows, int cols, void* d_dst, int dst_step);
int lvk_launch_scharr(lvk_hip_ctx* ctx, const void* d_src, int src_step, int rows, int cols, void* d_dst);
struct PyrArgs;
int lvk_launch_pyramid(lvk_hip_ctx* ctx, const PyrArgs& args, bool derivs = false);

int lvk_fast_workspace_bytes(int nregions, int max_rw, int max_rh, size_t* masks_bytes, size_t* scores_bytes);
int lvk_launch_fast(lvk_hip_ctx* ctx, const void* d_img, int step, int rows, int cols,
                    const FastRegion* d_regions, int nregions, int max_rw, int max_rh,
                    void* d_masks, void* d_scores, uint32_t* d_out, int cap, int* d_counts, const FastRegion* host_regions = nullptr);

struct FastInsertDesc
{
    const uint16_t* col_of; const uint32_t* row_base; const uint8_t* bucket;
    uint32_t* cell_first; void* cell_best ; int* region_count;
    const uint32_t* occ;
    const int* occ_bucket;
    int capacity; bool small_grid; int n_held, min_samples; float uniformity, homography_threshold;
    float2* pts; uint32_t* new_kp; int* result; int* d_n; int* d_full; int* counts;
};
int lvk_launch_fast_insert(lvk_hip_ctx* ctx, const void* d_img, int step, int rows, int cols, const FastRegion* host_regions, int nregions,
                           int max_rw, int max_rh, void* d_masks, void* d_scores, const FastInsertDesc& d);
bool lvk_fast_insert_fits(int cells, int nregions, int max_rw, int max_rh, int cols, int rows);
int lvk_fast_cells_reset(lvk_hip_ctx* ctx, uint32_t* d_first, void* d_best, int cells, int* d_region_count );

struct LensModel;
int lvk_pyramid_geometry(int rows, int cols, int max_level, int win_w, int win_h, int* lrows, int* lcols);
int lvk_launch_pyrlk(lvk_hip_ctx* ctx, const PyrArgs& prev, const PyrArgs& next, const float2* d_prev_pts, int n,
                     float2* d_next_pts, uint8_t* d_status, int win_w, int win_h, int max_count, double epsilon, double min_eig,
                     float2* d_prev_copy = nullptr,
                     const LensModel* lens = nullptr, double lens_sx = 0.0, double lens_sy = 0.0, float2* d_und = nullptr,
                     const int* d_n = nullptr);

struct DevicePyramid
{
    uint8_t* img_base = nullptr;
    uint8_t* deriv_base = nullptr;
    PyrArgs args{};
    int allocate(lvk_hip_ctx* ctx, int rows, int cols, int max_level, int win_w, int win_h);
    int build(lvk_hip_ctx* ctx, bool derivs = false);
    void release();
};

struct LvkHostSignal { unsigned* flag; unsigned seq; };

size_t lvk_ransac_workspace_bytes(int n);
int lvk_launch_ransac(lvk_hip_ctx* ctx, const float2* d_p1, const float2* d_p2, int n, double threshold, double region_w, double region_h,
                      bool full_homography, void* d_ws, double* d_H, int* d_ninl, uint8_t* d_mask, const int* d_n = nullptr,
                      const int* d_full = nullptr,
                      LvkHostSignal done = LvkHostSignal{nullptr, 0},
                      int lo_mode = 0);
int lvk_launch_match_compact(lvk_hip_ctx* ctx, const float2* d_prev, const float2* d_matched, const uint8_t* d_status, int n,
                             float2* d_p1, float2* d_p2, int* d_count, int* h_count, float2* h_matched, uint8_t* h_status,
                             const float2* d_und = nullptr, float region_w = 0.0f, float region_h = 0.0f,
                             const int* d_n_raw = nullptr);
constexpr int LVK_COMPACT_RANSAC_MAX = 2048;
int lvk_launch_compact_ransac(lvk_hip_ctx* ctx, const float2* d_prev, const float2* d_matched, const uint8_t* d_status, int n,
                              float2* d_p1, float2* d_p2, int* d_count, int* h_count, float2* h_matched, uint8_t* h_status,
                              const float2* d_und, float region_wf, float region_hf,
                              double threshold, double region_w, double region_h, bool full_homography, void* d_ws, double* d_H, int* d_ninl, uint8_t* d_mask,
                              const int* d_n_raw = nullptr, const int* d_full = nullptr, LvkHostSignal done = LvkHostSignal{nullptr, 0});

struct LvkTrackChain
{
    const PyrArgs* prev_pyr = nullptr; const PyrArgs* next_pyr = nullptr;
    const float2* h_pts = nullptr;
    int win_w = 0, win_h = 0, max_count = 0; double epsilon = 0.0, min_eig = 0.0;
    const LensModel* lens = nullptr; double lens_sx = 0.0, lens_sy = 0.0;
    int n = 0; const int* d_n = nullptr;
    bool full = false; const int* d_full = nullptr;
    float2* d_pts = nullptr; float2* d_matched = nullptr; uint8_t* d_status = nullptr;
    float2* d_und = nullptr;
    float2* d_p1 = nullptr; float2* d_p2 = nullptr; int* d_count = nullptr;
    int* h_count = nullptr; float2* h_matched = nullptr; uint8_t* h_status = nullptr;
    int region_w = 0, region_h = 0; double threshold = 0.0;
// ... 118 lines not shown
```

livevisionkit_amd/csrc/stab_lookahead.hip:

```cpp
#include "stab_state.hpp"

using namespace lvkstab;

int lvk_hip_stab::launch_build_ahead(DevicePyramid& P, int cur_w, int cur_h)
{
    const LumaAhead a = ahead_announced;
    ahead_announced = LumaAhead();
    int rc;
    int pe = prof_begin(LVK_STAGE_DOWNSCALE);
    if ((rc = lvk_launch_luma_area_resize(ctx, a.luma, a.step, a.pix, a.channel, a.rows, a.cols, const_cast<uint8_t*>(P.args.lv[0].img), P.args.lv[0].step, cur_h, cur_w)) != LVK_HIP_OK) return rc;
    prof_end(pe);
    pe = prof_begin(LVK_STAGE_PYRAMID);
    if ((rc = P.build(ctx)) != LVK_HIP_OK) return rc;
    prof_end(pe);
    if (!ahead_read_done) LVK_HIP_CHECK(ctx, hipEventCreateWithFlags(&ahead_read_done, hipEventDisableTiming));
    LVK_HIP_CHECK(ctx, hipEventRecord(ahead_read_done, ctx->stream));
    ahead_read_armed = true;
    ahead_built = a; ahead_built_for = push_seq + 1;
    return LVK_HIP_OK;
}

extern "C" {

static int stab_announce(lvk_hip_stab* st, const void* luma, int step, int pix, int channel, int rows, int cols)
{
    st->ahead_announced.luma = luma; st->ahead_announced.step = step; st->ahead_announced.pix = pix; st->ahead_announced.channel = channel;
    st->ahead_announced.rows = rows; st->ahead_announced.cols = cols;
    return LVK_HIP_OK;
}

int lvk_hip_stab_prefetch(lvk_hip_stab* st, const void* d_frame, int step, int rows, int cols, int format)
{
    if (!st) return LVK_HIP_ERR_ARG;
    lvk_hip_ctx* ctx = st->ctx;
    LVK_HIP_REQUIRE(ctx, d_frame && rows > 0 && cols > 0 && step >= 3 * cols);
    LVK_HIP_REQUIRE(ctx, format == LVK_FORMAT_YUV || format == LVK_FORMAT_BGR || format == LVK_FORMAT_RGB);
    return stab_announce(st, d_frame, step, 3, format == LVK_FORMAT_YUV ? 0 : (format == LVK_FORMAT_BGR ? -1 : -2), rows, cols);
}

int lvk_hip_stab_prefetch_yuv420(lvk_hip_stab* st, const void* d_y, int y_step, const void* d_u, int u_step, const void* d_v, int v_step, int nv12, int rows, int cols)
{
    if (!st) return LVK_HIP_ERR_ARG;
    lvk_hip_ctx* ctx = st->ctx;
    LVK_HIP_REQUIRE(ctx, d_y && d_u && (nv12 || d_v) && rows > 0 && cols > 0 && rows % 2 == 0 && cols % 2 == 0);
    LVK_HIP_REQUIRE(ctx, y_step >= cols && u_step >= (nv12 ? cols : cols / 2) && (nv12 || v_step >= cols / 2));
    return stab_announce(st, d_y, y_step, 1, 0, rows, cols);
}

long long lvk_hip_stab_lookahead_frames(lvk_hip_stab* st) { return st ? (long long)st->lookahead_frames : 0; }

int lvk_hip_stab_prefetch_cancel(lvk_hip_stab* st)
{
    if (!st) return LVK_HIP_ERR_ARG;
    lvk_device_guard device_guard(st->ctx);
    st->forget_device_lookahead();
    { const int rc = st->finish_device_lookahead_reads(); if (rc != LVK_HIP_OK) return rc; }
    return st->cancel_lookahead();
}

}
```

livevisionkit_amd/csrc/stab_state.hpp:

```cpp
#pragma once
#include "lvk_hip_internal.hpp"
#include "host_logic.hpp"

#include <chrono>
#include <cstdio>
#include <cstdlib>
#include <cstring>
#include <deque>
#include <functional>
#include <thread>

namespace lvkstab {

using lvkh::Feature;
using lvkh::WarpMeshF;

constexpr int LK_WIN = 11, LK_LEVELS = 3, LK_ITERS = 5;
constexpr double LK_EPS = 0.01, LK_MIN_EIG = 1e-4;
constexpr float HOMOGRAPHY_DISTRIBUTION_THRESHOLD = 0.6f;
constexpr float QA_UPDATE_RATE = 0.1f, QA_BLEND_STEP = 0.05f;

inline void lvk_cpu_relax()
{
#if defined(__x86_64__) || defined(__i386__)
    __builtin_ia32_pause();
#elif defined(__aarch64__)
    asm volatile("yield" ::: "memory");
#else
    std::this_thread::yield();
#endif
}

inline float step_toward(float current, float target, float amount)
{
    return current > target ? std::max(current - amount, target) : std::min(current + amount, target);
}

struct HostTrace
{
    enum { ENTER, DOWN_PYR_LAUNCH, FAST_SYNC, GRID, LK_LAUNCH, LK_SYNC, FILTER, RANSAC_LAUNCH, RANSAC_SYNC, POST, SMOOTH, REMAP_LAUNCH, EXIT, EMIT_WAITS, EMIT_KERNEL, EMIT_EVENT, EXIT_PRE, EXIT_WAIT, N };
    bool on = std::getenv("LVK_HIP_HOST_TRACE") != nullptr;
    double acc[N] = {0}; long cnt[N] = {0};
    std::chrono::steady_clock::time_point last;
    void begin() { if (on) last = std::chrono::steady_clock::now(); }
    void mark(int k)
    {
        if (!on) return;
        const auto now = std::chrono::steady_clock::now();
        acc[k] += std::chrono::duration<double, std::micro>(now - last).count(); cnt[k]++; last = now;
    }
    void dump() const
    {
        if (!on) return;
        static const char* names[N] = {"enter", "downscale+pyramid launch", "fast launch+sync", "grid (host)", "lk upload+launch", "lk sync", "filter (host)",
                                       "ransac upload+launch", "ransac sync", "post (host)", "qa+smoother (host)", "remap launch", "exit",
                                       "  emit: stream waits", "  emit: remap kernel launch", "  emit: slot event record", "  exit: up to the conversion wait", "  exit: conversion wait"};
        double total = 0; long frames = cnt[DOWN_PYR_LAUNCH] ? cnt[DOWN_PYR_LAUNCH] : 1;
        for (int i = 0; i < N; i++) total += acc[i];
        std::fprintf(stderr, "[lvk host trace] %ld frames, %.1f us/frame inside push\n", frames, total / frames);
        for (int i = 0; i < N; i++) if (cnt[i]) std::fprintf(stderr, "  %-28s %8.1f us/frame (%ld marks)\n", names[i], acc[i] / frames, cnt[i]);
    }
};

struct QueuedFrame { const void* d_ptr; int step, rows, cols; uint64_t ts; int format; };


struct OutPlanes420 { void* y; int y_step; void* u; int u_step; void* v; int v_step; int nv12; bool used; int rows_cap = 0; int vf = 0; void* p[3] = {nullptr, nullptr, nullptr}; int s[3] = {0, 0, 0}; };

struct HostPlane { const void* p; int step, width, rows; };

inline int host_planes_of(int vf, const void* const planes[3], const int steps[3], int rows, int cols, HostPlane out[3])
{
    auto set = [&](int i, int w, int r, bool tight = false) { out[i] = HostPlane{planes[i], tight ? w : steps[i], w, r}; };
    switch (vf)
    {
    case LVK_VIDEO_FORMAT_I420: case LVK_VIDEO_FORMAT_I40A: set(0, cols, rows); set(1, cols / 2, rows / 2); set(2, cols / 2, rows / 2); return 3;
    case LVK_VIDEO_FORMAT_NV12: set(0, cols, rows); set(1, cols, rows / 2); return 2;
    case LVK_VIDEO_FORMAT_I422: case LVK_VIDEO_FORMAT_I42A: set(0, cols, rows); set(1, cols / 2, rows); set(2, cols / 2, rows); return 3;
    case LVK_VIDEO_FORMAT_I444: case LVK_VIDEO_FORMAT_YUVA: set(0, cols, rows); set(1, cols, rows); set(2, cols, rows); return 3;
    case LVK_VIDEO_FORMAT_YUY2: case LVK_VIDEO_FORMAT_YVYU: case LVK_VIDEO_FORMAT_UYVY: set(0, 2 * cols, rows); return 1;
    case LVK_VIDEO_FORMAT_AYUV: set(0, 4 * cols, rows); return 1;
    case LVK_VIDEO_FORMAT_BGR3: set(0, 3 * cols, rows); return 1;
    case LVK_VIDEO_FORMAT_RGBA: case LVK_VIDEO_FORMAT_BGRA: case LVK_VIDEO_FORMAT_BGRX: set(0, 3 * cols, rows, true); return 1;
    default: return 0;
    }
}

}

struct lvk_hip_stab
{
    using Feature = lvkstab::Feature; using WarpMeshF = lvkstab::WarpMeshF; using QueuedFrame = lvkstab::QueuedFrame; using HostTrace = lvkstab::HostTrace;
    using OutPlanes420 = lvkstab::OutPlanes420; using HostPlane = lvkstab::HostPlane;
    lvk_hip_ctx* ctx = nullptr;
    lvk_stab_settings s{};
    bool configured = false;
    bool buffers_ok = false;

    DevicePyramid pyr[2];
    int cur = 0;
    int pyr_w = 0, pyr_h = 0;
    int prev_w = 0, prev_h = 0, cur_w = 0, cur_h = 0;
    bool initialized = false;
    size_t cap_features = 0;
    int fast_cap = 0, fast_max_rw = 0, fast_max_rh = 0, fast_regions = 0;
    void* d_fast_masks = nullptr; void* d_fast_scores = nullptr;
    float2 *d_pts = nullptr, *d_matched = nullptr, *d_p1 = nullptr; uint8_t* d_status = nullptr;
    void* d_ransac_ws = nullptr;
    int* d_count = nullptr;
    uint16_t* d_grid_col = nullptr; uint32_t* d_grid_row = nullptr; uint8_t* d_grid_bucket = nullptr;
    uint32_t* d_cell_first = nullptr; void* d_cell_best = nullptr; int* d_region_count = nullptr;
    int* d_n_points = nullptr; int* d_full = nullptr;
    uint32_t* h_occ = nullptr; uint32_t* h_new_kp = nullptr; int* h_insert = nullptr;
    bool device_grid = [] { const char* e = std::getenv("LVK_HIP_HOST_GRID"); return !(e && e[0] == '1'); }();
    long device_grid_frames = 0, host_grid_frames = 0;
    float2* d_und = nullptr;
    uint32_t* h_fast_out = nullptr; int* h_fast_counts = nullptr; FastRegion* h_regions = nullptr;
    float2 *h_pts = nullptr, *h_matched = nullptr, *h_p1 = nullptr; uint8_t* h_status = nullptr;
    double* h_H = nullptr; int* h_ninl = nullptr; uint8_t* h_mask = nullptr;
    int* h_count = nullptr;
    float2* h_und = nullptr;

    bool lens = false;
    lvk_camera_params lens_params{};
    LensModel lens_model{}; LensArgs lens_args{};
    int lens_rows = 0, lens_cols = 0;
    int ensure_lens(int rows, int cols)
    {
        if (!lens || (rows == lens_rows && cols == lens_cols)) return LVK_HIP_OK;
        if (lvk_lens_model_build(lens_params, rows, cols, lens_model) != LVK_HIP_OK) return fail(LVK_HIP_ERR_ARG, "invalid camera profile for this frame size");
        std::memcpy(lens_args.f, lens_model.f, sizeof(lens_args.f));
        lens_rows = rows; lens_cols = cols;
        return LVK_HIP_OK;
    }

    HostTrace trace;

    lvkh::FeatureGridH grid;
    lvkh::PathSmootherH smoother;
    struct MeshGen { int cols = 0, rows = 0; float w = 0, h = 0, temporal = 0, local = 0; } mesh_gen;
    lvk_mesh_solver_dev* mesh_dev = nullptr;
    void* d_mesh_scratch = nullptr; float* h_offsets = nullptr; int* h_mesh_status = nullptr; size_t h_offsets_floats = 0;
    lvk_stab_settings tracker_s{};
    std::vector<Feature> tracked;
    std::vector<FastRegion> plan;
    std::deque<QueuedFrame> queue;
    size_t queue_capacity = 1;
    bool next_output(const QueuedFrame& in, QueuedFrame* f) const
    {
        const size_t n = queue.size(), drop = n == queue_capacity ? 1 : 0;
        if (n - drop + 1 != queue_capacity) return false;
        if (f) *f = n > drop ? queue[drop] : in;
        return true;
    }
    float tracking_stability = 0.0f, scene_quality = 0.0f, trust = 0.0f;
    float last_distribution = 0.0f; int last_detected = 0, last_matched = 0;
    double last_H[9] = {1, 0, 0, 0, 1, 0, 0, 0, 1};
    WarpMeshF last_motion, last_correction;

    int remap_precision = LVK_REMAP_EXACT;
    uint8_t background_alpha = 0;

    bool overlap = false;
    hipStream_t remap_stream = nullptr;
    bool remap_stream_owned = false;
    hipEvent_t remap_done[2] = {nullptr, nullptr};
    int remap_slot = 0;
    const void* pending_release = nullptr;
// ... 8 lines not shown
    long signal_spin_us = [] { const char* e = std::getenv("LVK_HIP_SIGNAL_SPIN_US"); return e ? std::max(0L, std::atol(e)) : 400L; }();
    bool signal_test_lose = [] { const char* e = std::getenv("LVK_HIP_SIGNAL_TEST_LOSE"); return e && e[0] == '1'; }();
    bool ingest_on_tracker = false, tracker_ingest_capable = false;
    bool bulk_busy_at_push = false;
    bool caller_runs_free = false;
    int assume_caller = [] { const char* e = std::getenv("LVK_HIP_ASSUME_CALLER"); return !e ? 0 : (e[0] == 'f' ? 1 : (e[0] == 's' ? 2 : 0)); }();
    int free_streak = 0, sync_streak = 0;
    std::chrono::steady_clock::time_point last_push_end{};
    long long sched[LVK_SCHED_COUNT] = {0};
    int ingest_placement = [] { const char* e = std::getenv("LVK_HIP_INGEST_PLACEMENT"); return !e ? 0 : (e[0] == 't' ? 1 : (e[0] == 'b' ? 2 : 0)); }();
    std::vector<hipEvent_t> slot_read_done;
    std::vector<char> slot_read_armed;
    int slot_index(const void* p) const { for (size_t i = 0; i < pool_all.size(); i++) if (pool_all[i] == p) return (int)i; return -1; }
    int pending_slot = -1;
    hipEvent_t caller_ready = nullptr;
    bool caller_wait_pending = false;
    int mark_caller_work()
    {
        if (!(overlap && s.stabilize_output && remap_stream)) return LVK_HIP_OK;
        if (hipStreamQuery(ctx->stream) == hipSuccess) { caller_wait_pending = false; return LVK_HIP_OK; }
        (void)hipGetLastError();
        if (!caller_ready) LVK_HIP_CHECK(ctx, hipEventCreateWithFlags(&caller_ready, hipEventDisableTiming));
        LVK_HIP_CHECK(ctx, hipEventRecord(caller_ready, ctx->stream));
        caller_wait_pending = true;
        return LVK_HIP_OK;
    }
    int bulk_stream_sees_caller_work()
    {
        if (!caller_wait_pending) return LVK_HIP_OK;
        caller_wait_pending = false;
        LVK_HIP_CHECK(ctx, hipStreamWaitEvent(remap_stream, caller_ready, 0));
        return LVK_HIP_OK;
    }
    std::deque<const void*> orphaned;

    bool profiling = false;
    unsigned prof_mask = ~0u;
    unsigned prof_every = 1, prof_tick = 0;
    struct EvPair { hipEvent_t a, b; int kind; };
    std::vector<EvPair> ev_pool; size_t ev_used = 0;
    double prof_ms[LVK_STAGE_COUNT] = {0}; long prof_n[LVK_STAGE_COUNT] = {0};
    int prof_begin(int kind, hipStream_t stream = nullptr);
    void prof_end(int idx, hipStream_t stream = nullptr);
    int prof_collect();

    int fail(int code, const std::string& msg) { return ctx->fail(code, msg); }
    void free_tracker_buffers();
    int alloc_tracker_buffers();
    int alloc_pyramids();
    int configure(const lvk_stab_settings& st);
    void tracker_restart();
    void reset_context() { tracker_restart(); smoother.restart(); }
    int post_n = -1, post_m = 0;
    bool post_error = false;
    void finish_post();
    int track(const QueuedFrame& f, const void* luma, int luma_step, int luma_pix, int luma_channel, WarpMeshF& motion, bool& have_motion);

    struct HostIO
    {
        static constexpr int K_IN = 2, K_OUT = 3;
        hipStream_t up = nullptr, down = nullptr, down2 = nullptr;
        struct Pending { bool valid = false; int slot = 0; void* y; void* u; void* v; int ys, us, vs, nv12; } pending;
        int rows = 0, cols = 0;
        size_t in_bytes = 0;
        void* d_in[K_IN] = {nullptr, nullptr}; void* d_out[K_OUT] = {nullptr, nullptr, nullptr};
        hipEvent_t y_done[K_IN] = {}, c_done[K_IN] = {}, out_ready[K_OUT] = {}, down_done[K_OUT] = {};
        bool down_armed[K_OUT] = {false, false, false};
        bool y_is_c[K_IN] = {false, false};
        struct Ahead { int slot; const void* key[3]; int rows, cols, nv12; };
        std::deque<Ahead> ahead;
        const uint8_t* last_dst_lo = nullptr; const uint8_t* last_dst_hi = nullptr;
        int in_next = 0, out_next = 0, last_down = -1;
        std::chrono::steady_clock::time_point last_end{};
    } hostio;
    bool host_free_running_hint = false;
    std::vector<void*> gray_host_live;
    hipEvent_t gray_up_done = nullptr, gray_fence = nullptr;
    bool gray_host_owns(const void* p) const { return std::find(gray_host_live.begin(), gray_host_live.end(), p) != gray_host_live.end(); }
    bool gray_host_entry_now = false;
    void free_gray_host();
    bool host_direct_now = false;
    hipEvent_t ingest_wait[2] = {nullptr, nullptr};
    hipEvent_t remap_wait = nullptr;
    int ensure_hostio(int rows, int cols, size_t in_bytes = 0);
    int require_pinned(const void* p, size_t bytes, const char* what)
    {
        if (!p || bytes == 0) return LVK_HIP_OK;
        for (const uint8_t* q : {(const uint8_t*)p, (const uint8_t*)p + (bytes - 1)})
        {
            hipPointerAttribute_t attr{};
            const hipError_t e = hipPointerGetAttributes(&attr, q);
            if (e != hipSuccess) (void)hipGetLastError();
            if (e != hipSuccess || (attr.type != hipMemoryTypeHost && attr.type != hipMemoryTypeManaged && attr.type != hipMemoryTypeDevice))
                return fail(LVK_HIP_ERR_ARG, std::string(what) + ": the planes of the host entry points must be PINNED host memory "
                                             "(lvk_hip_host_malloc, hipHostMalloc or hipHostRegister) over their whole extent; this pointer is pageable memory");
        }
        return LVK_HIP_OK;
    }
    int require_pinned_planes(const HostPlane* pl, int n, const char* what)
    {
        if (n <= 0 || !pl[0].p) return LVK_HIP_OK;
        auto extent = [](const HostPlane& h) { return (size_t)h.step * (h.rows - 1) + h.width; };
        bool contiguous = true; size_t total = 0;
        for (int i = 0; i < n; i++)
        {
            contiguous = contiguous && pl[i].step == pl[i].width && (const uint8_t*)pl[i].p == (const uint8_t*)pl[0].p + total;
// ... 70 lines not shown
```

livevisionkit_amd/csrc/stabilizer.hip:

```cpp
#include "stab_state.hpp"

using namespace lvkstab;

int lvk_hip_stab::track(const QueuedFrame& f, const void* luma, int luma_step, int luma_pix, int luma_channel, WarpMeshF& motion, bool& have_motion)
{
    have_motion = false;
    tracking_stability = 0.0f;
    last_detected = last_matched = 0; last_distribution = 0.0f;
    hipStream_t st = ctx->stream;
    int rc;

    cur ^= 1;
    std::swap(prev_w, cur_w); std::swap(prev_h, cur_h);
    cur_w = s.detection_width; cur_h = s.detection_height;
    DevicePyramid& C = pyr[cur];
    DevicePyramid& P = pyr[cur ^ 1];
    int pe = 0;
    const bool built_ahead = ahead_built_for == push_seq && ahead_built.same(luma, luma_step, luma_pix, luma_channel, f.rows, f.cols) && pyr_w == cur_w && pyr_h == cur_h;
    ahead_built = LumaAhead(); ahead_built_for = 0;
    if (built_ahead) lookahead_frames++;
    else
    {
        pe = prof_begin(LVK_STAGE_DOWNSCALE);
        if ((rc = lvk_launch_luma_area_resize(ctx, luma, luma_step, luma_pix, luma_channel, f.rows, f.cols, const_cast<uint8_t*>(C.args.lv[0].img), C.args.lv[0].step, cur_h, cur_w)) != LVK_HIP_OK) return rc;
        prof_end(pe);
        pe = prof_begin(LVK_STAGE_PYRAMID);
        if ((rc = C.build(ctx)) != LVK_HIP_OK) return rc;
        prof_end(pe);
    }
    trace.mark(HostTrace::DOWN_PYR_LAUNCH);
    finish_post();
    if (post_error) { post_error = false; return fail(LVK_HIP_ERR_RUNTIME, "GPU-side fast_filter disagrees with the host's"); }
    auto leave_early = [&]() -> int { if (luma_pix != 3) LVK_HIP_CHECK(ctx, hipStreamSynchronize(st)); return LVK_HIP_OK; };
    if (!initialized || cur_w != prev_w || cur_h != prev_h) { initialized = true; return leave_early(); }

    grid.plan(plan);
    bool any = false;
    for (size_t i = 0; i < plan.size(); i++) { h_regions[i] = plan[i]; any = any || plan[i].active; }
    const size_t n_held = grid.held.size();
    const size_t n_bound = std::min(cap_features, n_held + (grid.capacity() - grid.used_cells()));
    const bool dev_insert = any && device_grid && grid.device_insert_ok() && (int)plan.size() <= LVK_FAST_INLINE_REGIONS &&
                            lvk_fast_insert_fits((int)grid.capacity(), (int)plan.size(), fast_max_rw, fast_max_rh, cur_w, cur_h) && n_bound >= 1 && n_bound <= 4096;
    float distribution = 0.0f;
    if (dev_insert)
    {
        for (size_t i = 0; i < n_held; i++) h_pts[i] = make_float2(grid.held[i].x, grid.held[i].y);
        int occ_bucket[16];
        grid.occupancy(h_occ, occ_bucket);
        const FastInsertDesc d{d_grid_col, d_grid_row, d_grid_bucket, d_cell_first, d_cell_best, d_region_count, h_occ, occ_bucket, (int)grid.capacity(), grid.grid_cols() <= 4 || grid.grid_rows() <= 4, (int)n_held,
                               s.min_motion_samples, s.uniformity_threshold, HOMOGRAPHY_DISTRIBUTION_THRESHOLD, h_pts, h_new_kp, h_insert, d_n_points, d_full, h_fast_counts};
        pe = prof_begin(LVK_STAGE_FAST);
        if ((rc = lvk_launch_fast_insert(ctx, C.args.lv[0].img, C.args.lv[0].step, cur_h, cur_w, h_regions, (int)plan.size(), fast_max_rw, fast_max_rh,
                                         d_fast_masks, d_fast_scores, d)) != LVK_HIP_OK) return rc;
        prof_end(pe);
        device_grid_frames++;
    }
    else
    {
    if (any)
    {
        pe = prof_begin(LVK_STAGE_FAST);
        if ((rc = lvk_launch_fast(ctx, C.args.lv[0].img, C.args.lv[0].step, cur_h, cur_w, h_regions, (int)plan.size(), fast_max_rw, fast_max_rh,
                                  d_fast_masks, d_fast_scores, h_fast_out, fast_cap, h_fast_counts, h_regions)) != LVK_HIP_OK) return rc;
        prof_end(pe);
        LVK_HIP_CHECK(ctx, hipStreamSynchronize(st));
        trace.mark(HostTrace::FAST_SYNC);
        host_grid_frames++;
    }
    for (size_t i = 0; i < plan.size(); i++)
        if (plan[i].active) grid.absorb(i, h_fast_out + i * (size_t)fast_cap, std::min(h_fast_counts[i], fast_cap));
    distribution = grid.finish(tracked);
    last_distribution = distribution; last_detected = (int)tracked.size();
    if (tracked.size() < (size_t)s.min_motion_samples || distribution < s.uniformity_threshold) { tracked.clear(); return leave_early(); }
    if (tracked.size() > cap_features) return fail(LVK_HIP_ERR_RUNTIME, "feature count exceeds the suppression grid capacity");
    }

    trace.mark(HostTrace::GRID);
    int n = dev_insert ? (int)n_bound : (int)tracked.size();
    if (!dev_insert) for (int i = 0; i < n; i++) h_pts[i] = make_float2(tracked[i].x, tracked[i].y);
    const int* dn = dev_insert ? d_n_points : nullptr;
    const int* dfull = dev_insert ? d_full : nullptr;
    const bool full = distribution > HOMOGRAPHY_DISTRIBUTION_THRESHOLD;
    const bool chained = n <= 4096;
    const bool field = s.track_local_motions != 0;
    LvkHostSignal done{nullptr, 0};
    if (chained && !field && !caller_runs_free)
    {
        if (!h_chain_flag) { LVK_HIP_CHECK(ctx, hipHostMalloc((void**)&h_chain_flag, 64, hipHostMallocCoherent)); *h_chain_flag = 0; }
        done = LvkHostSignal{h_chain_flag, ++chain_seq};
    }
    pe = prof_begin(LVK_STAGE_PYRLK);
    if (chained)
    {
        struct Stage { lvk_hip_stab* self; int* pe; } stage{this, &pe};
        LvkTrackChain c;
        c.prev_pyr = &P.args; c.next_pyr = &C.args; c.h_pts = h_pts;
        c.win_w = LK_WIN; c.win_h = LK_WIN; c.max_count = LK_ITERS; c.epsilon = LK_EPS; c.min_eig = LK_MIN_EIG;
        c.lens = lens ? &lens_model : nullptr; c.lens_sx = (double)f.cols / (double)cur_w; c.lens_sy = (double)f.rows / (double)cur_h;
        c.n = n; c.d_n = dn; c.full = full; c.d_full = dfull;
        c.d_pts = d_pts; c.d_matched = d_matched; c.d_status = d_status; c.d_und = lens ? d_und : nullptr;
        c.d_p1 = d_p1; c.d_p2 = d_p1 + cap_features; c.d_count = d_count; c.h_count = h_count; c.h_matched = h_matched; c.h_status = h_status;
        c.region_w = cur_w; c.region_h = cur_h; c.threshold = s.acceptance_threshold;
        c.separate_compact = field; c.estimate = !field;
        c.d_ws = d_ransac_ws; c.h_H = h_H; c.h_ninl = h_ninl; c.h_mask = h_mask; c.done = done;
        c.stage_boundary = [](void* u) { Stage* g = (Stage*)u; g->self->prof_end(*g->pe); *g->pe = g->self->prof_begin(LVK_STAGE_MOTION); };
        c.user = &stage;
        if ((rc = lvk_launch_track_chain(ctx, c)) != LVK_HIP_OK) return rc;
        if (field)
// ... 36 lines not shown
        const unsigned expect = signal_test_lose ? done.seq + 0x40000000u : done.seq;
        const auto t0 = std::chrono::steady_clock::now();
        const auto budget = std::chrono::microseconds(signal_spin_us);
        for (unsigned spins = 0;; spins++)
        {
            if (__atomic_load_n(done.flag, __ATOMIC_ACQUIRE) == expect) { have_results = true; break; }
            if ((spins & 63u) == 63u && std::chrono::steady_clock::now() - t0 > budget) break;
            lvk_cpu_relax();
        }
        sched[have_results ? LVK_SCHED_WAIT_SIGNAL_WORD : LVK_SCHED_WAIT_WORD_TIMEOUT]++;
    }
    if (!have_results)
    {
        if (chain_event_armed) LVK_HIP_CHECK(ctx, hipEventSynchronize(chain_done));
        else LVK_HIP_CHECK(ctx, hipStreamSynchronize(st));
        sched[LVK_SCHED_WAIT_EVENT]++;
    }
    trace.mark(HostTrace::LK_SYNC);

    if (dev_insert)
    {
        const int n_new = h_insert[0];
        float q_dev; std::memcpy(&q_dev, &h_insert[2], sizeof(float));
        if (n_new < 0 || (size_t)n_new > grid.capacity()) return fail(LVK_HIP_ERR_RUNTIME, "device suppression grid returned an impossible count");
        distribution = grid.finish_device(tracked, h_new_kp, n_new, h_fast_counts, fast_cap);
        last_distribution = distribution; last_detected = (int)tracked.size();
        if (distribution != q_dev || tracked.size() != n_held + (size_t)n_new)
            return fail(LVK_HIP_ERR_RUNTIME, "device suppression grid disagrees with the host's bookkeeping");
        if (tracked.size() < (size_t)s.min_motion_samples || distribution < s.uniformity_threshold) { tracked.clear(); return LVK_HIP_OK; }
        if (tracked.size() > cap_features) return fail(LVK_HIP_ERR_RUNTIME, "feature count exceeds the suppression grid capacity");
        n = (int)tracked.size();
    }
    if (chained)
    {
        const int m = *h_count;
        last_matched = m;
        if (m < 0 || m > n) return fail(LVK_HIP_ERR_RUNTIME, "GPU-side fast_filter returned an impossible count");
        if ((size_t)m < (size_t)s.min_motion_samples) { tracked.clear(); return LVK_HIP_OK; }
        motion = WarpMeshF(s.motion_height, s.motion_width);
        if (field)
        {
            if (*h_mesh_status != 0) { tracked.clear(); return LVK_HIP_OK; }
            std::memcpy(motion.off.data(), h_offsets, motion.off.size() * sizeof(float));
        }
        else
        {
            std::memcpy(last_H, h_H, sizeof(last_H));
            motion.from_homography(last_H, (float)cur_w, (float)cur_h);
        }
        size_t inliers = 0;
        for (int i = 0; i < m; i++) inliers += h_mask[i] ? 1 : 0;
        tracking_stability = (float)inliers / (float)m;
        have_motion = true;
        post_n = n; post_m = m;
        trace.mark(HostTrace::POST);
        return LVK_HIP_OK;
    }

    if (lens && !chained)
    {
        const float w = (float)cur_w, h = (float)cur_h;
        auto inside = [&](const float2& p) { return p.x >= 0.0f && p.x < w && p.y >= 0.0f && p.y < h; };
        for (int k = 0; k < n; k++)
            if (!(inside(h_und[k]) && inside(h_und[n + k]))) h_status[k] = 0;
    }
    int m = n;
    for (int k = n - 1; k >= 0; k--)
        if (!h_status[k])
        {
            m--;
            std::swap(tracked[k], tracked[m]);
            std::swap(h_pts[k], h_pts[m]);
            std::swap(h_matched[k], h_matched[m]);
            if (lens && !chained) { std::swap(h_und[k], h_und[m]); std::swap(h_und[n + k], h_und[n + m]); }
        }
    tracked.resize(m);
    last_matched = m;
    if (chained && *h_count != m) return fail(LVK_HIP_ERR_RUNTIME, "GPU-side fast_filter disagrees with the host's");
    if ((size_t)m < (size_t)s.min_motion_samples) { tracked.clear(); return LVK_HIP_OK; }

    trace.mark(HostTrace::FILTER);
    motion = WarpMeshF(s.motion_height, s.motion_width);
    const float2* e1 = lens ? h_und : h_pts;
    const float2* e2 = lens ? h_und + n : h_matched;
    if (s.track_local_motions)
    {
        std::memcpy(h_p1, e1, m * sizeof(float2));
        std::memcpy(h_p1 + m, e2, m * sizeof(float2));
        LVK_HIP_CHECK(ctx, hipMemcpyAsync(d_p1, h_p1, 2 * (size_t)m * sizeof(float2), hipMemcpyHostToDevice, st));
        if ((rc = lvk_launch_mesh_solve(mesh_dev, st, d_mesh_scratch, d_p1, d_p1 + m, nullptr, m, 0, (float)cur_w, (float)cur_h,
                                        s.temporal_smoothing, s.acceptance_threshold, h_offsets, h_mask, h_mesh_status)) != LVK_HIP_OK) return rc;
        LVK_HIP_CHECK(ctx, hipStreamSynchronize(st));
        if (*h_mesh_status != 0)
        {
            tracked.clear();
            return LVK_HIP_OK;
        }
        std::memcpy(motion.off.data(), h_offsets, motion.off.size() * sizeof(float));
        size_t inl = 0;
        for (int i = 0; i < m; i++) inl += h_mask[i] ? 1 : 0;
        tracking_stability = (float)inl / (float)m;
        for (int i = m - 1; i >= 0; i--)
        {
            if (h_mask[i]) { tracked[i].age++; tracked[i].x = h_matched[i].x; tracked[i].y = h_matched[i].y; }
            else { std::swap(tracked[i], tracked.back()); tracked.pop_back(); }
        }
        grid.propagate(tracked);
// ... 603 lines not shown
```

livevisionkit_amd/stabilization.py:

```python
import ctypes
import time

import numpy as np

from . import _native
from .context import Context, _remap_precision

_c = ctypes

FORMAT_BGR, FORMAT_BGRA, FORMAT_RGB, FORMAT_RGBA, FORMAT_YUV, FORMAT_GRAY = range(6)
CHANNELS = {FORMAT_BGR: 3, FORMAT_BGRA: 4, FORMAT_RGB: 3, FORMAT_RGBA: 4, FORMAT_YUV: 3, FORMAT_GRAY: 1}


def frame_args(frame, channels, kind="uint8"):
    if (frame.dim() != 3 or frame.shape[2] != channels or frame.stride(2) != 1 or frame.stride(1) != channels
            or frame.dtype.itemsize != 1):
        raise ValueError("a packed %s frame [rows, cols, %d] with contiguous rows is required" % (kind, channels))
    return frame.data_ptr(), frame.stride(0)


def gray_frame_args(frame):
    if frame.dim() != 2 or frame.stride(1) != 1 or frame.dtype.itemsize != 1:
        raise ValueError("a packed 8UC1 frame [rows, cols] with contiguous rows is required")
    return frame.data_ptr(), frame.stride(0)
# ... 227 lines not shown
            self.ctx._check(rc)
        return (dst["planes"], ots.value) if produced.value else (None, None)

    def prepare_obs(self, fmt, planes):
        ptrs, steps = self.ctx._obs_args(planes)
        return {"vf": _c.c_int(self.ctx.VIDEO_FORMATS[fmt]), "ptrs": ptrs, "steps": steps, "rows": _c.c_int(planes[0].shape[0]), "cols": _c.c_int(planes[0].shape[1]),
                "planes": planes}

    def apply_obs_prepared(self, src, timestamp, dst):
        produced = self._produced; ots = self._ots
        rc = self.lib.lvk_hip_stab_push_obs(self.handle, src["vf"], src["ptrs"], src["steps"], src["rows"], src["cols"], timestamp,
                                            dst["ptrs"], dst["steps"], dst["rows"], self._produced_ref, self._ots_ref, None)
        if rc != 0:
            self.ctx._check(rc)
        return (dst["planes"], ots.value) if produced.value else (None, None)

    def host_planes(self, rows, cols, nv12=False):
        import numpy as np
        n = rows * cols * 3 // 2
        p = _c.c_void_p()
        self.ctx._check(self.lib.lvk_hip_host_malloc(self.ctx.handle, n, _c.byref(p)))
        self._host_blocks = getattr(self, "_host_blocks", []); self._host_blocks.append(p)
        buf = np.ctypeslib.as_array((_c.c_uint8 * n).from_address(p.value))
        y = buf[:rows * cols].reshape(rows, cols)
        if nv12:
            return y, buf[rows * cols:].reshape(rows // 2, cols // 2, 2)
        q = rows * cols // 4
        return y, buf[rows * cols:rows * cols + q].reshape(rows // 2, cols // 2), buf[rows * cols + q:].reshape(rows // 2, cols // 2)

    def prepare_yuv420_host(self, planes):
        nv12 = len(planes) == 2
        y, u = planes[0], planes[1]
        v = u if nv12 else planes[2]
        args = (_c.c_void_p(y.ctypes.data), _c.c_int(y.strides[0]), _c.c_void_p(u.ctypes.data), _c.c_int(u.strides[0]),
                _c.c_void_p(v.ctypes.data), _c.c_int(v.strides[0]))
        return {"args": args, "nv12": _c.c_int(1 if nv12 else 0), "rows": _c.c_int(y.shape[0]), "cols": _c.c_int(y.shape[1]), "planes": planes}

    def prefetch_yuv420_host_prepared(self, src):
        rc = self.lib.lvk_hip_stab_prefetch_yuv420_host(self.handle, *src["args"], src["nv12"], src["rows"], src["cols"])
        if rc != 0:
            self.ctx._check(rc)

    def prefetch(self, frame, fmt=FORMAT_YUV):
        self.ctx._check(self.lib.lvk_hip_stab_prefetch(self.handle, frame.data_ptr(), frame.stride(0), frame.shape[0], frame.shape[1], fmt))

    def prefetch_yuv420_prepared(self, src):
        rc = self.lib.lvk_hip_stab_prefetch_yuv420(self.handle, *src["args"], src["nv12"], src["rows"], src["cols"])
        if rc != 0:
            self.ctx._check(rc)

    def lookahead_frames(self):
        return int(self.lib.lvk_hip_stab_lookahead_frames(self.handle))

    def prefetch_cancel(self):
        self.ctx._check(self.lib.lvk_hip_stab_prefetch_cancel(self.handle))

    def apply_yuv420_host_prepared(self, src, timestamp, dst):
        produced = self._produced; ots = self._ots
        rc = self.lib.lvk_hip_stab_push_yuv420_host(self.handle, *src["args"], src["nv12"], src["rows"], src["cols"], timestamp,
                                                    *dst["args"], dst["rows"], self._produced_ref, self._ots_ref, None)
        if rc != 0:
            self.ctx._check(rc)
        return (dst["planes"], ots.value) if produced.value else (None, None)

    def host_plane_gray(self, rows, cols, pitch_extra=0):
        import numpy as np
        step = cols + pitch_extra
        p = _c.c_void_p()
        self.ctx._check(self.lib.lvk_hip_host_malloc(self.ctx.handle, rows * step, _c.byref(p)))
        self._host_blocks = getattr(self, "_host_blocks", []); self._host_blocks.append(p)
        return np.ctypeslib.as_array((_c.c_uint8 * (rows * step)).from_address(p.value)).reshape(rows, step)[:, :cols]

    def apply_gray_host(self, plane, timestamp=0, out=None):
        t0 = time.perf_counter()
        rows, cols = plane.shape
        if out is None:
            due = self.next_output(rows, cols, FORMAT_GRAY)
            out = self.host_plane_gray(due[0], due[1]) if due else None
        produced = _c.c_int(0); ots = _c.c_uint64(0); info = FrameInfo()
        optr, ostep, orows = (out.ctypes.data, out.strides[0], out.shape[0]) if out is not None else (None, 0, 0)
        rc = self.lib.lvk_hip_stab_push_gray_host(self.handle, plane.ctypes.data, plane.strides[0], rows, cols, int(timestamp), optr, ostep, orows,
                                                  _c.byref(produced), _c.byref(ots), _c.byref(info))
        self.ctx._check(rc)
        self._timer._add(time.perf_counter() - t0)
        if not produced.value:
            return None, None
        self.last_format = info.format
        return out[:info.rows, :info.cols], ots.value

    def host_plane_c4(self, rows, cols, pitch_extra=0):
        import numpy as np
        step = 4 * cols + pitch_extra
        p = _c.c_void_p()
        self.ctx._check(self.lib.lvk_hip_host_malloc(self.ctx.handle, rows * step, _c.byref(p)))
        self._host_blocks = getattr(self, "_host_blocks", []); self._host_blocks.append(p)
        block = np.ctypeslib.as_array((_c.c_uint8 * (rows * step)).from_address(p.value))
        return np.lib.stride_tricks.as_strided(block, (rows, cols, 4), (step, 4, 1))

    def apply_c4_host(self, plane, timestamp=0, out=None, fmt=FORMAT_BGRA):
        t0 = time.perf_counter()
        rows, cols = plane.shape[:2]
        if out is None:
            due = self.next_output(rows, cols, fmt)
            out = self.host_plane_c4(due[0], due[1]) if due else None
        produced = _c.c_int(0); ots = _c.c_uint64(0); info = FrameInfo()
        optr, ostep, orows = (out.ctypes.data, out.strides[0], out.shape[0]) if out is not None else (None, 0, 0)
# ... 162 lines not shown
```

Measured before the change: 9848.

## Fuse FAST detection and pyramid build into one combined kernel launch

```diff
diff --git a/include/lvk_hip.h b/include/lvk_hip.h
--- a/include/lvk_hip.h
+++ b/include/lvk_hip.h
@@ -230,6 +230,7 @@
 int  lvk_hip_stab_prefetch_yuv420(lvk_hip_stab* stab, const void* d_y, int y_step, const void* d_u, int u_step, const void* d_v, int v_step,
                                   int nv12, int rows, int cols);
 long long lvk_hip_stab_lookahead_frames(lvk_hip_stab* stab);
+long long lvk_hip_stab_detect_frame_launches(lvk_hip_stab* stab);
 
 int lvk_hip_remap_homography_gray(lvk_hip_ctx* ctx, const void* d_src, int src_step, int src_rows, int src_cols,
                                   void* d_dst, int dst_step, int dst_rows, int dst_cols, int off_x, int off_y, const float H[9], uint8_t bg);
@@ -328,6 +329,10 @@
 int lvk_hip_fast_detect(lvk_hip_ctx* ctx, const void* d_img, int step, int rows, int cols,
                         const int* regions, int nregions, uint32_t* out, int cap, int* counts);
 
+int lvk_hip_pyramid_fast_detect(lvk_hip_ctx* ctx, const void* d_img, int step, int rows, int cols, int max_level, int win_w, int win_h,
+                                uint8_t* levels, int16_t* derivs, int* level_rows, int* level_cols,
+                                const int* regions, int nregions, uint32_t* out, int cap, int* counts);
+
 int lvk_hip_pyrlk(lvk_hip_ctx* ctx, const void* d_prev, int prev_step, const void* d_next, int next_step, int rows, int cols,
                   const float* prev_pts, int n, float* next_pts, uint8_t* status,
                   int win_w, int win_h, int max_level, int max_count, double epsilon, double min_eig_threshold);
diff --git a/livevisionkit_amd/_native.py b/livevisionkit_amd/_native.py
--- a/livevisionkit_amd/_native.py
+++ b/livevisionkit_amd/_native.py
@@ -93,6 +93,9 @@
                                          _c.POINTER(_c.c_uint8), _c.POINTER(_c.c_int16), _c.POINTER(_c.c_int), _c.POINTER(_c.c_int)]),
     "lvk_hip_fast_detect": (_c.c_int, [_P, _P, _c.c_int, _c.c_int, _c.c_int, _c.POINTER(_c.c_int), _c.c_int,
                                        _c.POINTER(_c.c_uint32), _c.c_int, _c.POINTER(_c.c_int)]),
+    "lvk_hip_pyramid_fast_detect": (_c.c_int, [_P, _P, _c.c_int, _c.c_int, _c.c_int, _c.c_int, _c.c_int, _c.c_int,
+                                               _c.POINTER(_c.c_uint8), _c.POINTER(_c.c_int16), _c.POINTER(_c.c_int), _c.POINTER(_c.c_int),
+                                               _c.POINTER(_c.c_int), _c.c_int, _c.POINTER(_c.c_uint32), _c.c_int, _c.POINTER(_c.c_int)]),
     "lvk_hip_pyrlk": (_c.c_int, [_P, _P, _c.c_int, _P, _c.c_int, _c.c_int, _c.c_int, _c.POINTER(_c.c_float), _c.c_int,
                                  _c.POINTER(_c.c_float), _c.POINTER(_c.c_uint8), _c.c_int, _c.c_int, _c.c_int, _c.c_int,
                                  _c.c_double, _c.c_double]),
@@ -132,6 +135,7 @@
     "lvk_hip_stab_prefetch": (_c.c_int, [_P, _P, _c.c_int, _c.c_int, _c.c_int, _c.c_int]),
     "lvk_hip_stab_prefetch_yuv420": (_c.c_int, [_P, _P, _c.c_int, _P, _c.c_int, _P, _c.c_int, _c.c_int, _c.c_int, _c.c_int]),
     "lvk_hip_stab_lookahead_frames": (_c.c_longlong, [_P]),
+    "lvk_hip_stab_detect_frame_launches": (_c.c_longlong, [_P]),
     "lvk_hip_stab_schedule_counters": (_c.c_int, [_P, _c.POINTER(_c.c_longlong), _c.c_int]),
     "lvk_hip_stab_detector_frames": (_c.c_int, [_P, _c.POINTER(_c.c_longlong), _c.POINTER(_c.c_longlong)]),
     "lvk_hip_host_malloc": (_c.c_int, [_P, _c.c_size_t, _c.POINTER(_P)]),
diff --git a/livevisionkit_amd/context.py b/livevisionkit_amd/context.py
--- a/livevisionkit_amd/context.py
+++ b/livevisionkit_amd/context.py
@@ -266,6 +266,31 @@
             e = out[i, :min(cap, counts[i])]
             res.append(np.stack([e & 0xFFF, (e >> 12) & 0xFFF, e >> 24], axis=1).astype(np.int32))
         return res, counts
+
+    def pyramid_fast_detect(self, img, regions, cap=None, max_level=3, win=(11, 11)):
+        rows, cols = img.shape
+        rg = np.ascontiguousarray(regions, dtype=np.int32).reshape(-1, 6)
+        n = rg.shape[0]
+        cap = cap or int(max(1, (rg[:, 2] * rg[:, 3]).max()))
+        lv = np.zeros(rows * cols * 2, np.uint8); dv = np.zeros(rows * cols * 4, np.int16)
+        lr = np.zeros(8, np.int32); lc = np.zeros(8, np.int32)
+        out = np.zeros((n, cap), np.uint32); counts = np.zeros(n, np.int32)
+        nl = self.lib.lvk_hip_pyramid_fast_detect(self.handle, img.data_ptr(), img.stride(0), rows, cols, max_level, win[0], win[1],
+                                                  lv.ctypes.data_as(ctypes.POINTER(ctypes.c_uint8)), dv.ctypes.data_as(ctypes.POINTER(ctypes.c_int16)),
+                                                  lr.ctypes.data_as(ctypes.POINTER(ctypes.c_int)), lc.ctypes.data_as(ctypes.POINTER(ctypes.c_int)),
+                                                  rg.ctypes.data_as(ctypes.POINTER(ctypes.c_int)), n,
+                                                  out.ctypes.data_as(ctypes.POINTER(ctypes.c_uint32)), cap, counts.ctypes.data_as(ctypes.POINTER(ctypes.c_int)))
+        self._check(min(nl, 0))
+        pyr, lo, do = [], 0, 0
+        for i in range(nl):
+            r, c = int(lr[i]), int(lc[i])
+            pyr.append((lv[lo:lo + r * c].reshape(r, c).copy(), dv[do:do + r * c * 2].reshape(r, c, 2).copy()))
+            lo += r * c; do += r * c * 2
+        kps = []
+        for i in range(n):
+            e = out[i, :min(cap, counts[i])]
+            kps.append(np.stack([e & 0xFFF, (e >> 12) & 0xFFF, e >> 24], axis=1).astype(np.int32))
+        return pyr, kps, counts
 
     def pyrlk(self, prev, nxt, pts, win=(11, 11), max_level=3, max_count=5, epsilon=0.01, min_eig=1e-4):
         pts = np.ascontiguousarray(pts, np.float32).reshape(-1, 2)
diff --git a/livevisionkit_amd/csrc/detect_frame.hip b/livevisionkit_amd/csrc/detect_frame.hip
--- /dev/null
+++ b/livevisionkit_amd/csrc/detect_frame.hip
@@ -0,0 +1,97 @@
+#include "lvk_hip_internal.hpp"
+#include "fast_detect_core.hpp"
+#include "pyr_fused3_core.hpp"
+
+#include <algorithm>
+
+namespace {
+
+constexpr int DF_NT = lvk_fastk::TW * lvk_fastk::TH;
+constexpr int DF_LDS = lvk_fastk::LDS_BYTES > lvk_pyr3::LDS_BYTES ? lvk_fastk::LDS_BYTES : lvk_pyr3::LDS_BYTES;
+
+template <bool CELLS>
+__global__ __launch_bounds__(DF_NT)
+void k_detect_frame(lvk_fastk::FastDetectArgs f, int nd, PyrArgs p)
+{
+    LVK_TL(0);
+    LVK_TRACKER_PRIORITY();
+    __shared__ __attribute__((aligned(4))) uint8_t lds[DF_LDS];
+    const int b = blockIdx.x;
+    if (b < nd) lvk_fastk::fast_detect_block<DF_NT, CELLS>(f, b, threadIdx.x, lds);
+    else lvk_pyr3::pyr_fused3_block<DF_NT>(p, b - nd, threadIdx.x, lds);
+}
+
+}
+
+int lvk_launch_detect_frame(lvk_hip_ctx* ctx, const lvk_fastk::FastDetectArgs& f, int nd, const PyrArgs& p, bool cells)
+{
+    LVK_HIP_REQUIRE(ctx, nd > 0 && p.nlevels == 4 && p.lv[0].img == f.img && p.lv[0].step == f.step && p.lv[0].rows == f.rows && p.lv[0].cols == f.cols);
+    const dim3 grid(nd + lvk_pyr3::blocks(p)), block(DF_NT);
+    if (cells) hipLaunchKernelGGL(k_detect_frame<true>, grid, block, 0, ctx->stream, f, nd, p);
+    else hipLaunchKernelGGL(k_detect_frame<false>, grid, block, 0, ctx->stream, f, nd, p);
+    LVK_HIP_CHECK(ctx, hipGetLastError());
+    return LVK_HIP_OK;
+}
+
+extern "C" {
+
+int lvk_hip_pyramid_fast_detect(lvk_hip_ctx* ctx, const void* d_img, int step, int rows, int cols, int max_level, int win_w, int win_h,
+                                uint8_t* levels, int16_t* derivs, int* level_rows, int* level_cols,
+                                const int* regions, int nregions, uint32_t* out, int cap, int* counts)
+{
+    LVK_HIP_ENTRY(ctx);
+    LVK_HIP_REQUIRE(ctx, d_img && levels && derivs && level_rows && level_cols && rows > 0 && cols > 0 && step >= cols);
+    LVK_HIP_REQUIRE(ctx, regions && out && counts && nregions > 0 && cap > 0);
+    int lr[LVK_MAX_PYR_LEVELS], lc[LVK_MAX_PYR_LEVELS];
+    LVK_HIP_REQUIRE(ctx, lvk_pyramid_geometry(rows, cols, max_level, win_w, win_h, lr, lc) == 4);
+    std::vector<FastRegion> rg((size_t)nregions);
+    int max_rw = 1, max_rh = 1;
+    for (int i = 0; i < nregions; i++)
+    {
+        rg[i] = FastRegion{regions[6 * i], regions[6 * i + 1], regions[6 * i + 2], regions[6 * i + 3], regions[6 * i + 4], regions[6 * i + 5]};
+        LVK_HIP_REQUIRE(ctx, rg[i].x >= 0 && rg[i].y >= 0 && rg[i].w > 0 && rg[i].h > 0 && rg[i].x + rg[i].w <= cols && rg[i].y + rg[i].h <= rows);
+        max_rw = std::max(max_rw, rg[i].w); max_rh = std::max(max_rh, rg[i].h);
+    }
+    size_t mb, sb;
+    lvk_fast_workspace_bytes(nregions, max_rw, max_rh, &mb, &sb);
+    DevicePyramid P;
+    void *d_masks = nullptr, *d_scores = nullptr, *d_regions = nullptr; uint32_t* d_out = nullptr; int* d_counts = nullptr;
+    auto cleanup = [&]() { P.release(); (void)hipFree(d_masks); (void)hipFree(d_scores); (void)hipFree(d_regions); (void)hipFree(d_out); (void)hipFree(d_counts); };
+    auto run = [&]() -> int
+    {
+        int rc;
+        if ((rc = P.allocate(ctx, rows, cols, max_level, win_w, win_h)) != LVK_HIP_OK) return rc;
+        LVK_HIP_CHECK(ctx, hipMalloc(&d_masks, mb));
+        LVK_HIP_CHECK(ctx, hipMalloc(&d_scores, sb));
+        LVK_HIP_CHECK(ctx, hipMalloc(&d_regions, rg.size() * sizeof(FastRegion)));
+        LVK_HIP_CHECK(ctx, hipMalloc((void**)&d_out, (size_t)nregions * cap * sizeof(uint32_t)));
+        LVK_HIP_CHECK(ctx, hipMalloc((void**)&d_counts, nregions * sizeof(int)));
+        const PyrLevel& L0 = P.args.lv[0];
+        LVK_HIP_CHECK(ctx, hipMemcpy2DAsync(const_cast<uint8_t*>(L0.img), L0.step, d_img, step, cols, rows, hipMemcpyDeviceToDevice, ctx->stream));
+        LVK_HIP_CHECK(ctx, hipMemcpyAsync(d_regions, rg.data(), rg.size() * sizeof(FastRegion), hipMemcpyHostToDevice, ctx->stream));
+        if ((rc = lvk_launch_fast(ctx, L0.img, L0.step, rows, cols, (const FastRegion*)d_regions, nregions, max_rw, max_rh, d_masks, d_scores, d_out, cap, d_counts,
+                                  nullptr, &P.args)) != LVK_HIP_OK) return rc;
+        if ((rc = lvk_launch_scharr_all(ctx, P.args)) != LVK_HIP_OK) return rc;
+        size_t lo = 0, dofs = 0;
+        for (int i = 0; i < P.args.nlevels; i++)
+        {
+            const PyrLevel& L = P.args.lv[i];
+            LVK_HIP_CHECK(ctx, hipMemcpy2DAsync(levels + lo, L.cols, L.img, L.step, L.cols, L.rows, hipMemcpyDeviceToHost, ctx->stream));
+            LVK_HIP_CHECK(ctx, hipMemcpyAsync(derivs + dofs, L.deriv, (size_t)L.rows * L.cols * 4, hipMemcpyDeviceToHost, ctx->stream));
+            lo += (size_t)L.rows * L.cols; dofs += (size_t)L.rows * L.cols * 2;
+        }
+        LVK_HIP_CHECK(ctx, hipMemcpyAsync(out, d_out, (size_t)nregions * cap * sizeof(uint32_t), hipMemcpyDeviceToHost, ctx->stream));
+        LVK_HIP_CHECK(ctx, hipMemcpyAsync(counts, d_counts, nregions * sizeof(int), hipMemcpyDeviceToHost, ctx->stream));
+        LVK_HIP_CHECK(ctx, hipStreamSynchronize(ctx->stream));
+        for (int i = 0; i < P.args.nlevels; i++) { level_rows[i] = P.args.lv[i].rows; level_cols[i] = P.args.lv[i].cols; }
+        return P.args.nlevels;
+    };
+    const int rc = run();
+    if (rc < 0) (void)hipStreamSynchronize(ctx->stream);
+    cleanup();
+    return rc;
+}
+
+}
+
+LVK_TL_EXPORT(detect_frame)
diff --git a/livevisionkit_amd/csrc/fast.hip b/livevisionkit_amd/csrc/fast.hip
--- a/livevisionkit_amd/csrc/fast.hip
+++ b/livevisionkit_amd/csrc/fast.hip
@@ -1,105 +1,18 @@
 #include "lvk_hip_internal.hpp"
+#include "fast_detect_core.hpp"
+
+using namespace lvk_fastk;
 
 namespace {
 
-constexpr int TW = 64, TH = 8;
-constexpr int AP = 4;
-constexpr int IW = TW + 2 * AP, IH = TH + 2 * AP;
-constexpr int SW = TW + 2, SH = TH + 2;
-
-__device__ __forceinline__ int fast_score(const uint8_t* c, int stride, int threshold)
-{
-    const int v = c[0];
-    int d[16];
-    d[0] = v - c[3 * stride];          d[1] = v - c[1 + 3 * stride];   d[2] = v - c[2 + 2 * stride];   d[3] = v - c[3 + stride];
-    d[4] = v - c[3];                   d[5] = v - c[3 - stride];       d[6] = v - c[2 - 2 * stride];   d[7] = v - c[1 - 3 * stride];
-    d[8] = v - c[-3 * stride];         d[9] = v - c[-1 - 3 * stride];  d[10] = v - c[-2 - 2 * stride]; d[11] = v - c[-3 - stride];
-    d[12] = v - c[-3];                 d[13] = v - c[-3 + stride];     d[14] = v - c[-2 + 2 * stride]; d[15] = v - c[-1 + 3 * stride];
-    int lo2[16], hi2[16], lo4[16], hi4[16];
-#pragma unroll
-    for (int k = 0; k < 16; k++) { lo2[k] = min(d[k], d[(k + 1) & 15]); hi2[k] = max(d[k], d[(k + 1) & 15]); }
-#pragma unroll
-    for (int k = 0; k < 16; k++) { lo4[k] = min(lo2[k], lo2[(k + 2) & 15]); hi4[k] = max(hi2[k], hi2[(k + 2) & 15]); }
-    int dark = -256, bright_neg = 256;
-#pragma unroll
-    for (int k = 0; k < 16; k++)
-    {
-        const int lo9 = min(min(lo4[k], lo4[(k + 4) & 15]), d[(k + 8) & 15]);
-        const int hi9 = max(max(hi4[k], hi4[(k + 4) & 15]), d[(k + 8) & 15]);
-        dark = max(dark, lo9);
-        bright_neg = min(bright_neg, hi9);
-    }
-    const int m = max(dark, -bright_neg);
-    return m > threshold ? m - 1 : 0;
-}
-
-struct FastRegionList { FastRegion r[LVK_FAST_INLINE_REGIONS]; };
-
-struct FastCells { const uint16_t* col_of; const uint32_t* row_base; uint32_t* first; unsigned long long* best; int* region_count; };
-
+template <bool CELLS>
 __global__ __launch_bounds__(TW * TH)
-void k_fast_detect(const uint8_t* __restrict__ img, int step, int rows, int cols,
-                   const FastRegion* __restrict__ regions, FastRegionList inl, int n_inline, int segs_x,
-                   unsigned long long* __restrict__ masks, uint8_t* __restrict__ scores, int max_rh, int max_rw, FastCells cells)
-{
+void k_fast_detect(FastDetectArgs a)
+{
+    LVK_TL(0);
     LVK_TRACKER_PRIORITY();
-    const FastRegion rg = n_inline ? inl.r[blockIdx.z] : regions[blockIdx.z];
-    if (!rg.active) return;
-    const int lx0 = blockIdx.x * TW, ly0 = blockIdx.y * TH;
-    if (lx0 >= rg.w || ly0 >= rg.h) return;
-
-    __shared__ uint8_t s_img[IH][IW];
-    __shared__ uint8_t s_score[SH][SW];
-    const int tid = threadIdx.y * TW + threadIdx.x;
-
-    for (int i = tid; i < IW * IH; i += TW * TH)
-    {
-        const int ty = i / IW, tx = i - ty * IW;
-        const int gx = min(max(rg.x + lx0 - AP + tx, 0), cols - 1);
-        const int gy = min(max(rg.y + ly0 - AP + ty, 0), rows - 1);
-        s_img[ty][tx] = img[(long)gy * step + gx];
-    }
-    __shared__ uint32_t s_cell_col[TW], s_cell_row[TH];
-    if (cells.first)
-    {
-        if (tid < TW) s_cell_col[tid] = cells.col_of[min(rg.x + lx0 + tid, cols - 1)];
-        else if (tid < TW + TH) s_cell_row[tid - TW] = cells.row_base[min(rg.y + ly0 + tid - TW, rows - 1)];
-    }
-    __syncthreads();
-
-    for (int i = tid; i < SW * SH; i += TW * TH)
-    {
-        const int ty = i / SW, tx = i - ty * SW;
-        const int lx = lx0 - 1 + tx, ly = ly0 - 1 + ty;
-        int s = 0;
-        if (lx >= 3 && lx < rg.w - 3 && ly >= 3 && ly < rg.h - 3)
-            s = fast_score(&s_img[ty + AP - 1][tx + AP - 1], IW, rg.threshold);
-        s_score[ty][tx] = (uint8_t)s;
-    }
-    __syncthreads();
-
-    const int lx = lx0 + threadIdx.x, ly = ly0 + threadIdx.y;
-    const int sx = threadIdx.x + 1, sy = threadIdx.y + 1;
-    const int s = s_score[sy][sx];
-    const bool keep = s > 0 &&
-        s > s_score[sy][sx - 1] && s > s_score[sy][sx + 1] &&
-        s > s_score[sy - 1][sx - 1] && s > s_score[sy - 1][sx] && s > s_score[sy - 1][sx + 1] &&
-        s > s_score[sy + 1][sx - 1] && s > s_score[sy + 1][sx] && s > s_score[sy + 1][sx + 1];
-    const unsigned long long mask = __ballot(keep);
-    if (ly < rg.h)
-    {
-        if (threadIdx.x == 0) masks[((long)blockIdx.z * max_rh + ly) * segs_x + blockIdx.x] = mask;
-        if (threadIdx.x == 0 && cells.first && mask) atomicAdd(&cells.region_count[blockIdx.z], __popcll(mask));
-        if (keep) scores[((long)blockIdx.z * max_rh + ly) * max_rw + lx] = (uint8_t)s;
-        if (keep && cells.first)
-        {
-            const uint32_t ci = s_cell_row[threadIdx.y] + s_cell_col[threadIdx.x];
-            const uint32_t key = (uint32_t)(((int)blockIdx.z * max_rh + ly) * max_rw + lx);
-            atomicMin(&cells.first[ci], key);
-            const uint32_t rec = (uint32_t)(rg.x + lx) | ((uint32_t)(rg.y + ly) << 12) | ((uint32_t)s << 24);
-            atomicMax(&cells.best[ci], ((unsigned long long)(((uint32_t)s << 24) | (0xFFFFFFu - key)) << 32) | rec);
-        }
-    }
+    __shared__ __attribute__((aligned(4))) uint8_t lds[LDS_BYTES];
+    fast_detect_block<TW * TH, CELLS>(a, blockIdx.x, threadIdx.x, lds);
 }
 
 __global__ __launch_bounds__(1024)
@@ -177,6 +90,7 @@
 __global__ __launch_bounds__(INS_NT)
 void k_fast_insert(int nregions, FastInsertArgs a)
 {
+    LVK_TL(1);
     LVK_TRACKER_PRIORITY();
     extern __shared__ __attribute__((aligned(16))) uint8_t ins_smem[];
     const int bwords = (a.nkeys + 31) / 32;
@@ -281,19 +195,28 @@
     return segs_x;
 }
 
+template <bool CELLS>
+static int launch_detect(lvk_hip_ctx* ctx, const FastDetectArgs& a, int nregions, const PyrArgs* pyr)
+{
+    const int nd = a.segs_x * a.tiles_y * nregions;
+    if (pyr) return lvk_launch_detect_frame(ctx, a, nd, *pyr, CELLS);
+    hipLaunchKernelGGL(k_fast_detect<CELLS>, dim3(nd), dim3(TW * TH), 0, ctx->stream, a);
+    return LVK_HIP_OK;
+}
+
 int lvk_launch_fast(lvk_hip_ctx* ctx, const void* d_img, int step, int rows, int cols,
                     const FastRegion* d_regions, int nregions, int max_rw, int max_rh,
-                    void* d_masks, void* d_scores, uint32_t* d_out, int cap, int* d_counts, const FastRegion* host_regions)
+                    void* d_masks, void* d_scores, uint32_t* d_out, int cap, int* d_counts, const FastRegion* host_regions, const PyrArgs* fuse_pyr)
 {
     LVK_HIP_REQUIRE(ctx, d_img && d_regions && nregions > 0 && max_rw > 0 && max_rh > 0 && max_rw < 4096 && max_rh < 4096);
     const int segs_x = (max_rw + TW - 1) / TW;
-    const dim3 block(TW, TH), grid(segs_x, (max_rh + TH - 1) / TH, nregions);
-    FastRegionList inl{};
-    const int n_inline = (host_regions && nregions <= LVK_FAST_INLINE_REGIONS) ? nregions : 0;
-    for (int i = 0; i < n_inline; i++) inl.r[i] = host_regions[i];
-    hipLaunchKernelGGL(k_fast_detect, grid, block, 0, ctx->stream, (const uint8_t*)d_img, step, rows, cols, d_regions, inl, n_inline, segs_x,
-                       (unsigned long long*)d_masks, (uint8_t*)d_scores, max_rh, max_rw, FastCells{});
-    hipLaunchKernelGGL(k_fast_compact, dim3(nregions), dim3(1024), 0, ctx->stream, d_regions, inl, n_inline, segs_x,
+    FastDetectArgs a{(const uint8_t*)d_img, step, rows, cols, d_regions, {}, 0, segs_x, (max_rh + TH - 1) / TH,
+                     (unsigned long long*)d_masks, (uint8_t*)d_scores, max_rh, max_rw, FastCells{}};
+    a.n_inline = (host_regions && nregions <= LVK_FAST_INLINE_REGIONS) ? nregions : 0;
+    for (int i = 0; i < a.n_inline; i++) a.inl.r[i] = host_regions[i];
+    int rc;
+    if ((rc = launch_detect<false>(ctx, a, nregions, fuse_pyr)) != LVK_HIP_OK) return rc;
+    hipLaunchKernelGGL(k_fast_compact, dim3(nregions), dim3(1024), 0, ctx->stream, d_regions, a.inl, a.n_inline, segs_x,
                        (const unsigned long long*)d_masks, (const uint8_t*)d_scores, max_rh, max_rw, d_out, cap, d_counts);
     LVK_HIP_CHECK(ctx, hipGetLastError());
     return LVK_HIP_OK;
@@ -301,21 +224,21 @@
 
 
 int lvk_launch_fast_insert(lvk_hip_ctx* ctx, const void* d_img, int step, int rows, int cols, const FastRegion* host_regions, int nregions,
-                           int max_rw, int max_rh, void* d_masks, void* d_scores, const FastInsertDesc& d)
+                           int max_rw, int max_rh, const FastInsertDesc& d, const PyrArgs* fuse_pyr)
 {
     LVK_HIP_REQUIRE(ctx, d_img && host_regions && nregions > 0 && nregions <= LVK_FAST_INLINE_REGIONS && max_rw > 0 && max_rh > 0);
     LVK_HIP_REQUIRE(ctx, lvk_fast_insert_fits(d.capacity, nregions, max_rw, max_rh, cols, rows));
     LVK_HIP_REQUIRE(ctx, d.pts && d.new_kp && d.result && d.d_n && d.d_full && d.counts && d.occ && d.cell_first && d.cell_best && d.region_count && d.occ_bucket && d.col_of && d.row_base && d.bucket);
     const int segs_x = (max_rw + TW - 1) / TW;
-    FastRegionList inl{};
-    for (int i = 0; i < nregions; i++) inl.r[i] = host_regions[i];
+    FastDetectArgs fa{(const uint8_t*)d_img, step, rows, cols, nullptr, {}, nregions, segs_x, (max_rh + TH - 1) / TH, nullptr, nullptr, max_rh, max_rw,
+                      FastCells{d.col_of, d.row_base, d.cell_first, (unsigned long long*)d.cell_best, d.region_count}};
+    for (int i = 0; i < nregions; i++) fa.inl.r[i] = host_regions[i];
     const int nkeys = nregions * max_rh * max_rw;
     const size_t lds = ins_lds_bytes(nkeys);
     if (lds > 48 * 1024)
         LVK_HIP_CHECK(ctx, hipFuncSetAttribute(reinterpret_cast<const void*>(k_fast_insert), hipFuncAttributeMaxDynamicSharedMemorySize, (int)lds));
-    const dim3 block(TW, TH), grid(segs_x, (max_rh + TH - 1) / TH, nregions);
-    hipLaunchKernelGGL(k_fast_detect, grid, block, 0, ctx->stream, (const uint8_t*)d_img, step, rows, cols, (const FastRegion*)nullptr, inl, nregions, segs_x,
-                       (unsigned long long*)d_masks, (uint8_t*)d_scores, max_rh, max_rw, FastCells{d.col_of, d.row_base, d.cell_first, (unsigned long long*)d.cell_best, d.region_count});
+    int rc;
+    if ((rc = launch_detect<true>(ctx, fa, nregions, fuse_pyr)) != LVK_HIP_OK) return rc;
     FastInsertArgs a{d.bucket, d.cell_first, (unsigned long long*)d.cell_best, d.region_count, d.capacity, d.small_grid ? 1 : 0, d.n_held, d.min_samples, d.uniformity, d.homography_threshold, nkeys,
                      d.pts, d.new_kp, d.result, d.d_n, d.d_full, d.counts, {}, {}};
     for (int i = 0; i < (d.capacity + 31) / 32; i++) a.occ[i] = d.occ[i];
@@ -375,3 +298,5 @@
 }
 
 }
+
+LVK_TL_EXPORT(fast)
diff --git a/livevisionkit_amd/csrc/fast_detect_core.hpp b/livevisionkit_amd/csrc/fast_detect_core.hpp
--- /dev/null
+++ b/livevisionkit_amd/csrc/fast_detect_core.hpp
@@ -0,0 +1,146 @@
+#pragma once
+
+#include "lvk_hip_internal.hpp"
+
+namespace lvk_fastk {
+
+constexpr int TW = 64, TH = 8;
+constexpr int AP = 4;
+constexpr int IW = TW + 2 * AP, IH = TH + 2 * AP;
+constexpr int SW = TW + 2, SH = TH + 2;
+constexpr int LDS_SCORE = IW * IH, LDS_COL = (LDS_SCORE + SW * SH + 3) & ~3, LDS_ROW = LDS_COL + 4 * TW, LDS_BYTES = LDS_ROW + 4 * TH;
+
+__device__ __forceinline__ int fast_score(const uint8_t* c, int stride, int threshold)
+{
+    const int v = c[0];
+    int d[16];
+    d[0] = v - c[3 * stride];          d[1] = v - c[1 + 3 * stride];   d[2] = v - c[2 + 2 * stride];   d[3] = v - c[3 + stride];
+    d[4] = v - c[3];                   d[5] = v - c[3 - stride];       d[6] = v - c[2 - 2 * stride];   d[7] = v - c[1 - 3 * stride];
+    d[8] = v - c[-3 * stride];         d[9] = v - c[-1 - 3 * stride];  d[10] = v - c[-2 - 2 * stride]; d[11] = v - c[-3 - stride];
+    d[12] = v - c[-3];                 d[13] = v - c[-3 + stride];     d[14] = v - c[-2 + 2 * stride]; d[15] = v - c[-1 + 3 * stride];
+    int lo2[16], hi2[16], lo4[16], hi4[16];
+#pragma unroll
+    for (int k = 0; k < 16; k++) { lo2[k] = min(d[k], d[(k + 1) & 15]); hi2[k] = max(d[k], d[(k + 1) & 15]); }
+#pragma unroll
+    for (int k = 0; k < 16; k++) { lo4[k] = min(lo2[k], lo2[(k + 2) & 15]); hi4[k] = max(hi2[k], hi2[(k + 2) & 15]); }
+    int dark = -256, bright_neg = 256;
+#pragma unroll
+    for (int k = 0; k < 16; k++)
+    {
+        const int lo9 = min(min(lo4[k], lo4[(k + 4) & 15]), d[(k + 8) & 15]);
+        const int hi9 = max(max(hi4[k], hi4[(k + 4) & 15]), d[(k + 8) & 15]);
+        dark = max(dark, lo9);
+        bright_neg = min(bright_neg, hi9);
+    }
+    const int m = max(dark, -bright_neg);
+    return m > threshold ? m - 1 : 0;
+}
+
+struct FastRegionList { FastRegion r[LVK_FAST_INLINE_REGIONS]; };
+
+struct FastCells { const uint16_t* col_of; const uint32_t* row_base; uint32_t* first; unsigned long long* best; int* region_count; };
+
+struct FastDetectArgs
+{
+    const uint8_t* img; int step, rows, cols;
+    const FastRegion* regions; FastRegionList inl; int n_inline;
+    int segs_x, tiles_y;
+    unsigned long long* masks; uint8_t* scores; int max_rh, max_rw;
+    FastCells cells;
+};
+
+template <int NT, bool CELLS>
+__device__ __forceinline__ void fast_detect_block(const FastDetectArgs& a, int b, int tid, uint8_t* lds)
+{
+    static_assert(NT % 64 == 0 && NT >= TW + TH && (TW * TH) % NT == 0, "whole waves per 64-pixel row segment");
+    const int q = b / a.segs_x, bx = b - q * a.segs_x, bz = q / a.tiles_y, by = q - bz * a.tiles_y;
+    const FastRegion rg = a.n_inline ? a.inl.r[bz] : a.regions[bz];
+    if (!rg.active) return;
+    const int lx0 = bx * TW, ly0 = by * TH;
+    if (lx0 >= rg.w || ly0 >= rg.h) return;
+
+    uint8_t* s_img = lds;
+    uint8_t* s_score = lds + LDS_SCORE;
+    uint32_t* s_cell_col = reinterpret_cast<uint32_t*>(lds + LDS_COL);
+    uint32_t* s_cell_row = reinterpret_cast<uint32_t*>(lds + LDS_ROW);
+
+    {
+        constexpr int NI = (IW * IH + NT - 1) / NT;
+        uint8_t v[NI];
+#pragma unroll
+        for (int k = 0; k < NI; k++)
+        {
+            const int i = min(tid + NT * k, IW * IH - 1);
+            const int ty = i / IW, tx = i - ty * IW;
+            const int gx = min(max(rg.x + lx0 - AP + tx, 0), a.cols - 1);
+            const int gy = min(max(rg.y + ly0 - AP + ty, 0), a.rows - 1);
+            v[k] = a.img[(long)gy * a.step + gx];
+        }
+        uint32_t cell = 0;
+        if (CELLS)
+        {
+            if (tid < TW) cell = a.cells.col_of[min(rg.x + lx0 + tid, a.cols - 1)];
+            else if (tid < TW + TH) cell = a.cells.row_base[min(rg.y + ly0 + tid - TW, a.rows - 1)];
+        }
+#pragma unroll
+        for (int k = 0; k < NI; k++)
+        {
+            const int i = tid + NT * k;
+            if (i < IW * IH) s_img[i] = v[k];
+        }
+        if (CELLS)
+        {
+            if (tid < TW) s_cell_col[tid] = cell;
+            else if (tid < TW + TH) s_cell_row[tid - TW] = cell;
+        }
+    }
+    __syncthreads();
+
+    for (int i = tid; i < SW * SH; i += NT)
+    {
+        const int ty = i / SW, tx = i - ty * SW;
+        const int lx = lx0 - 1 + tx, ly = ly0 - 1 + ty;
+        int s = 0;
+        if (lx >= 3 && lx < rg.w - 3 && ly >= 3 && ly < rg.h - 3)
+            s = fast_score(&s_img[(ty + AP - 1) * IW + tx + AP - 1], IW, rg.threshold);
+        s_score[i] = (uint8_t)s;
+    }
+    __syncthreads();
+
+    for (int p = tid; p < TW * TH; p += NT)
+    {
+        const int tx = p & (TW - 1), ty = p / TW;
+        const int lx = lx0 + tx, ly = ly0 + ty;
+        const uint8_t* c = s_score + (ty + 1) * SW + tx + 1;
+        const int s = c[0];
+        const bool keep = s > 0 &&
+            s > c[-1] && s > c[1] &&
+            s > c[-SW - 1] && s > c[-SW] && s > c[-SW + 1] &&
+            s > c[SW - 1] && s > c[SW] && s > c[SW + 1];
+        const unsigned long long mask = __ballot(keep);
+        if (ly < rg.h)
+        {
+            if (!CELLS)
+            {
+                if (tx == 0) a.masks[((long)bz * a.max_rh + ly) * a.segs_x + bx] = mask;
+                if (keep) a.scores[((long)bz * a.max_rh + ly) * a.max_rw + lx] = (uint8_t)s;
+            }
+            else
+            {
+                if (tx == 0 && mask) atomicAdd(&a.cells.region_count[bz], __popcll(mask));
+                if (keep)
+                {
+                    const uint32_t ci = s_cell_row[ty] + s_cell_col[tx];
+                    const uint32_t key = (uint32_t)((bz * a.max_rh + ly) * a.max_rw + lx);
+                    atomicMin(&a.cells.first[ci], key);
+                    const uint32_t rec = (uint32_t)(rg.x + lx) | ((uint32_t)(rg.y + ly) << 12) | ((uint32_t)s << 24);
+                    atomicMax(&a.cells.best[ci], ((unsigned long long)(((uint32_t)s << 24) | (0xFFFFFFu - key)) << 32) | rec);
+                }
+            }
+        }
+    }
+}
+
+}
+
+int lvk_launch_detect_frame(lvk_hip_ctx* ctx, const lvk_fastk::FastDetectArgs& f, int nd, const PyrArgs& p, bool cells);
diff --git a/livevisionkit_amd/csrc/host_logic.hpp b/livevisionkit_amd/csrc/host_logic.hpp
--- a/livevisionkit_amd/csrc/host_logic.hpp
+++ b/livevisionkit_amd/csrc/host_logic.hpp
@@ -168,7 +168,7 @@
 class FeatureGridH
 {
 public:
-    struct Zone { float x, y, w, h; int threshold; size_t load; bool ran; };
+    struct Zone { float x, y, w, h; int threshold; size_t load; bool ran; size_t seen = 0;  };
 
     void configure(const lvk_stab_settings& s)
     {
@@ -195,7 +195,7 @@
         zones.clear();
         for (int r = 0; r < m_zr; r++)
             for (int c = 0; c < m_zc; c++)
-                zones.push_back(Zone{(float)c * m_zw, (float)r * m_zh, m_zw, m_zh, 10 , 0, false});
+                zones.push_back(Zone{(float)c * m_zw, (float)r * m_zh, m_zw, m_zh, 10 , 0, false, 0});
         const float per_zone = (float)((size_t)m_gc * m_gr) / (float)(m_zc * m_zr);
         m_min_load = (size_t)(per_zone * (s.min_feature_density / s.max_feature_density));
         m_target = (size_t)(s.accumulation_rate * per_zone);
@@ -211,8 +211,20 @@
         {
             Zone& z = zones[i];
             z.ran = m_force || z.load <= m_min_load;
+            z.seen = z.load;
             out[i] = FastRegion{cv_round(z.x), cv_round(z.y), cv_round(z.w), cv_round(z.h), z.threshold, z.ran ? 1 : 0};
         }
+    }
+
+    bool likely_due(bool pending, size_t tracked, size_t survivors) const
+    {
+        if (m_force) return true;
+        for (const Zone& z : zones)
+        {
+            if (!pending) { if (z.load <= m_min_load) return true; }
+            else if (!z.ran && tracked > 0 && z.seen * survivors <= m_min_load * tracked) return true;
+        }
+        return false;
     }
 
     void absorb(size_t zone, const uint32_t* kp, int count)
diff --git a/livevisionkit_amd/csrc/imgproc.hip b/livevisionkit_amd/csrc/imgproc.hip
--- a/livevisionkit_amd/csrc/imgproc.hip
+++ b/livevisionkit_amd/csrc/imgproc.hip
@@ -1,16 +1,12 @@
 #include "lvk_hip_internal.hpp"
+#include "pyr_fused3_core.hpp"
 
 #include <cmath>
 #include <algorithm>
 
+using namespace lvk_pyr3;
+
 namespace {
-
-__device__ __forceinline__ int reflect101(int p, int len)
-{
-    if (len == 1) return 0;
-    while (p < 0 || p >= len) { p = (p < 0) ? -p : 2 * (len - 1) - p; }
-    return p;
-}
 
 __device__ __forceinline__ uint8_t sat_u8_rint(float v)
 {
@@ -260,90 +256,13 @@
     dst[(long)y * cols + x] = o;
 }
 
-constexpr int T3 = 4;
-constexpr int F2 = 2 * (T3 - 1) + 5, F1 = 2 * (F2 - 1) + 5, F0 = 2 * (F1 - 1) + 5;
-constexpr int F0P = F0 + 3, F1P = F1 + 3, F2P = F2 + 1;
-
-__device__ __forceinline__ int pyr_tap(const uint8_t* t, int pitch, int ox, int oy, int x, int y, int cols, int rows)
-{
-    int xi[5];
-#pragma unroll
-    for (int k = 0; k < 5; k++) xi[k] = reflect101(2 * x - 2 + k, cols) - ox;
-    int acc = 0;
-#pragma unroll
-    for (int ky = 0; ky < 5; ky++)
-    {
-        const uint8_t* row = t + (reflect101(2 * y - 2 + ky, rows) - oy) * pitch;
-        const int h = row[xi[0]] + row[xi[4]] + 4 * (row[xi[1]] + row[xi[3]]) + 6 * row[xi[2]];
-        acc += ((ky == 0 || ky == 4) ? 1 : (ky == 2 ? 6 : 4)) * h;
-    }
-    return (acc + 128) >> 8;
-}
-
 __global__ __launch_bounds__(256)
 void k_pyr_fused3(PyrArgs a)
 {
     LVK_TL(1);
     LVK_TRACKER_PRIORITY();
-    __shared__ uint8_t t0[F0 * F0P], t1[F1 * F1P], t2[F2 * F2P];
-    const int tid = threadIdx.x;
-    const int x3 = blockIdx.x * T3, y3 = blockIdx.y * T3;
-    const int o2x = 2 * x3 - 2, o2y = 2 * y3 - 2, o1x = 2 * o2x - 2, o1y = 2 * o2y - 2, o0x = 2 * o1x - 2, o0y = 2 * o1y - 2;
-    const PyrLevel L0 = a.lv[0], L1 = a.lv[1], L2 = a.lv[2], L3 = a.lv[3];
-
-    {
-        constexpr int N0 = (F0 * F0 + 255) / 256;
-        uint8_t v[N0];
-#pragma unroll
-        for (int k = 0; k < N0; k++)
-        {
-            const int i = min(tid + 256 * k, F0 * F0 - 1);
-            const int ty = i / F0, tx = i - ty * F0;
-            const int gx = min(max(o0x + tx, 0), L0.cols - 1), gy = min(max(o0y + ty, 0), L0.rows - 1);
-            v[k] = L0.img[(long)gy * L0.step + gx];
-        }
-#pragma unroll
-        for (int k = 0; k < N0; k++)
-        {
-            const int i = tid + 256 * k;
-            const int ty = i / F0, tx = i - ty * F0;
-            const int gx = o0x + tx, gy = o0y + ty;
-            if (i < F0 * F0 && gx >= 0 && gy >= 0 && gx < L0.cols && gy < L0.rows) t0[ty * F0P + tx] = v[k];
-        }
-    }
-    __syncthreads();
-    for (int i = tid; i < F1 * F1; i += 256)
-    {
-        const int ty = i / F1, tx = i - ty * F1;
-        const int gx = o1x + tx, gy = o1y + ty;
-        if (gx >= 0 && gy >= 0 && gx < L1.cols && gy < L1.rows)
-        {
-            const int v = pyr_tap(t0, F0P, o0x, o0y, gx, gy, L0.cols, L0.rows);
-            t1[ty * F1P + tx] = (uint8_t)v;
-            if (gx >= 4 * x3 && gx < 4 * x3 + 4 * T3 && gy >= 4 * y3 && gy < 4 * y3 + 4 * T3)
-                const_cast<uint8_t*>(L1.img)[(long)gy * L1.step + gx] = (uint8_t)v;
-        }
-    }
-    __syncthreads();
-    for (int i = tid; i < F2 * F2; i += 256)
-    {
-        const int ty = i / F2, tx = i - ty * F2;
-        const int gx = o2x + tx, gy = o2y + ty;
-        if (gx >= 0 && gy >= 0 && gx < L2.cols && gy < L2.rows)
-        {
-            const int v = pyr_tap(t1, F1P, o1x, o1y, gx, gy, L1.cols, L1.rows);
-            t2[ty * F2P + tx] = (uint8_t)v;
-            if (gx >= 2 * x3 && gx < 2 * x3 + 2 * T3 && gy >= 2 * y3 && gy < 2 * y3 + 2 * T3)
-                const_cast<uint8_t*>(L2.img)[(long)gy * L2.step + gx] = (uint8_t)v;
-        }
-    }
-    __syncthreads();
-    if (tid < T3 * T3)
-    {
-        const int gx = x3 + (tid % T3), gy = y3 + (tid / T3);
-        if (gx < L3.cols && gy < L3.rows)
-            const_cast<uint8_t*>(L3.img)[(long)gy * L3.step + gx] = (uint8_t)pyr_tap(t2, F2P, o2x, o2y, gx, gy, L2.cols, L2.rows);
-    }
+    __shared__ uint8_t lds[LDS_BYTES];
+    pyr_fused3_block<256>(a, blockIdx.x, threadIdx.x, lds);
 }
 
 __global__ __launch_bounds__(256)
@@ -563,19 +482,20 @@
 {
     int rc;
     if (args.nlevels == 4)
-    {
-        const dim3 grid((args.lv[3].cols + T3 - 1) / T3, (args.lv[3].rows + T3 - 1) / T3);
-        hipLaunchKernelGGL(k_pyr_fused3, grid, dim3(256), 0, ctx->stream, args);
-    }
+        hipLaunchKernelGGL(k_pyr_fused3, dim3(blocks(args)), dim3(256), 0, ctx->stream, args);
     else
         for (int i = 1; i < args.nlevels; i++)
             if ((rc = lvk_launch_pyr_down(ctx, args.lv[i - 1].img, args.lv[i - 1].step, args.lv[i - 1].rows, args.lv[i - 1].cols,
                                           const_cast<uint8_t*>(args.lv[i].img), args.lv[i].step)) != LVK_HIP_OK) return rc;
-    if (derivs)
-    {
-        const dim3 sgrid((args.lv[0].cols + 63) / 64, (args.lv[0].rows + 3) / 4, args.nlevels);
-        hipLaunchKernelGGL(k_scharr_all, sgrid, dim3(64, 4), 0, ctx->stream, args);
-    }
+    if (derivs) return lvk_launch_scharr_all(ctx, args);
+    LVK_HIP_CHECK(ctx, hipGetLastError());
+    return LVK_HIP_OK;
+}
+
+int lvk_launch_scharr_all(lvk_hip_ctx* ctx, const PyrArgs& args)
+{
+    const dim3 sgrid((args.lv[0].cols + 63) / 64, (args.lv[0].rows + 3) / 4, args.nlevels);
+    hipLaunchKernelGGL(k_scharr_all, sgrid, dim3(64, 4), 0, ctx->stream, args);
     LVK_HIP_CHECK(ctx, hipGetLastError());
     return LVK_HIP_OK;
 }
diff --git a/livevisionkit_amd/csrc/lvk_hip_internal.hpp b/livevisionkit_amd/csrc/lvk_hip_internal.hpp
--- a/livevisionkit_amd/csrc/lvk_hip_internal.hpp
+++ b/livevisionkit_amd/csrc/lvk_hip_internal.hpp
@@ -174,11 +174,13 @@
 int lvk_launch_scharr(lvk_hip_ctx* ctx, const void* d_src, int src_step, int rows, int cols, void* d_dst);
 struct PyrArgs;
 int lvk_launch_pyramid(lvk_hip_ctx* ctx, const PyrArgs& args, bool derivs = false);
+int lvk_launch_scharr_all(lvk_hip_ctx* ctx, const PyrArgs& args);
 
 int lvk_fast_workspace_bytes(int nregions, int max_rw, int max_rh, size_t* masks_bytes, size_t* scores_bytes);
 int lvk_launch_fast(lvk_hip_ctx* ctx, const void* d_img, int step, int rows, int cols,
                     const FastRegion* d_regions, int nregions, int max_rw, int max_rh,
-                    void* d_masks, void* d_scores, uint32_t* d_out, int cap, int* d_counts, const FastRegion* host_regions = nullptr);
+                    void* d_masks, void* d_scores, uint32_t* d_out, int cap, int* d_counts, const FastRegion* host_regions = nullptr,
+                    const PyrArgs* fuse_pyr = nullptr);
 
 struct FastInsertDesc
 {
@@ -190,7 +192,7 @@
     float2* pts; uint32_t* new_kp; int* result; int* d_n; int* d_full; int* counts;
 };
 int lvk_launch_fast_insert(lvk_hip_ctx* ctx, const void* d_img, int step, int rows, int cols, const FastRegion* host_regions, int nregions,
-                           int max_rw, int max_rh, void* d_masks, void* d_scores, const FastInsertDesc& d);
+                           int max_rw, int max_rh, const FastInsertDesc& d, const PyrArgs* fuse_pyr = nullptr);
 bool lvk_fast_insert_fits(int cells, int nregions, int max_rw, int max_rh, int cols, int rows);
 int lvk_fast_cells_reset(lvk_hip_ctx* ctx, uint32_t* d_first, void* d_best, int cells, int* d_region_count );
 
diff --git a/livevisionkit_amd/csrc/pyr_fused3_core.hpp b/livevisionkit_amd/csrc/pyr_fused3_core.hpp
--- /dev/null
+++ b/livevisionkit_amd/csrc/pyr_fused3_core.hpp
@@ -0,0 +1,102 @@
+#pragma once
+
+#include "lvk_hip_internal.hpp"
+
+namespace lvk_pyr3 {
+
+__device__ __forceinline__ int reflect101(int p, int len)
+{
+    if (len == 1) return 0;
+    while (p < 0 || p >= len) { p = (p < 0) ? -p : 2 * (len - 1) - p; }
+    return p;
+}
+
+constexpr int T3 = 4;
+constexpr int F2 = 2 * (T3 - 1) + 5, F1 = 2 * (F2 - 1) + 5, F0 = 2 * (F1 - 1) + 5;
+constexpr int F0P = F0 + 3, F1P = F1 + 3, F2P = F2 + 1;
+constexpr int LDS_T1 = F0 * F0P, LDS_T2 = LDS_T1 + F1 * F1P, LDS_BYTES = LDS_T2 + F2 * F2P;
+
+__host__ __device__ inline int blocks_x(const PyrArgs& a) { return (a.lv[3].cols + T3 - 1) / T3; }
+__host__ __device__ inline int blocks(const PyrArgs& a) { return blocks_x(a) * ((a.lv[3].rows + T3 - 1) / T3); }
+
+__device__ __forceinline__ int pyr_tap(const uint8_t* t, int pitch, int ox, int oy, int x, int y, int cols, int rows)
+{
+    int xi[5];
+#pragma unroll
+    for (int k = 0; k < 5; k++) xi[k] = reflect101(2 * x - 2 + k, cols) - ox;
+    int acc = 0;
+#pragma unroll
+    for (int ky = 0; ky < 5; ky++)
+    {
+        const uint8_t* row = t + (reflect101(2 * y - 2 + ky, rows) - oy) * pitch;
+        const int h = row[xi[0]] + row[xi[4]] + 4 * (row[xi[1]] + row[xi[3]]) + 6 * row[xi[2]];
+        acc += ((ky == 0 || ky == 4) ? 1 : (ky == 2 ? 6 : 4)) * h;
+    }
+    return (acc + 128) >> 8;
+}
+
+template <int NT>
+__device__ __forceinline__ void pyr_fused3_block(const PyrArgs& a, int b, int tid, uint8_t* lds)
+{
+    uint8_t* t0 = lds; uint8_t* t1 = lds + LDS_T1; uint8_t* t2 = lds + LDS_T2;
+    const int nbx = blocks_x(a), by = b / nbx, bx = b - by * nbx;
+    const int x3 = bx * T3, y3 = by * T3;
+    const int o2x = 2 * x3 - 2, o2y = 2 * y3 - 2, o1x = 2 * o2x - 2, o1y = 2 * o2y - 2, o0x = 2 * o1x - 2, o0y = 2 * o1y - 2;
+    const PyrLevel L0 = a.lv[0], L1 = a.lv[1], L2 = a.lv[2], L3 = a.lv[3];
+
+    {
+        constexpr int N0 = (F0 * F0 + NT - 1) / NT;
+        uint8_t v[N0];
+#pragma unroll
+        for (int k = 0; k < N0; k++)
+        {
+            const int i = min(tid + NT * k, F0 * F0 - 1);
+            const int ty = i / F0, tx = i - ty * F0;
+            const int gx = min(max(o0x + tx, 0), L0.cols - 1), gy = min(max(o0y + ty, 0), L0.rows - 1);
+            v[k] = L0.img[(long)gy * L0.step + gx];
+        }
+#pragma unroll
+        for (int k = 0; k < N0; k++)
+        {
+            const int i = tid + NT * k;
+            const int ty = i / F0, tx = i - ty * F0;
+            const int gx = o0x + tx, gy = o0y + ty;
+            if (i < F0 * F0 && gx >= 0 && gy >= 0 && gx < L0.cols && gy < L0.rows) t0[ty * F0P + tx] = v[k];
+        }
+    }
+    __syncthreads();
+    for (int i = tid; i < F1 * F1; i += NT)
+    {
+        const int ty = i / F1, tx = i - ty * F1;
+        const int gx = o1x + tx, gy = o1y + ty;
+        if (gx >= 0 && gy >= 0 && gx < L1.cols && gy < L1.rows)
+        {
+            const int v = pyr_tap(t0, F0P, o0x, o0y, gx, gy, L0.cols, L0.rows);
+            t1[ty * F1P + tx] = (uint8_t)v;
+            if (gx >= 4 * x3 && gx < 4 * x3 + 4 * T3 && gy >= 4 * y3 && gy < 4 * y3 + 4 * T3)
+                const_cast<uint8_t*>(L1.img)[(long)gy * L1.step + gx] = (uint8_t)v;
+        }
+    }
+    __syncthreads();
+    for (int i = tid; i < F2 * F2; i += NT)
+    {
+        const int ty = i / F2, tx = i - ty * F2;
+        const int gx = o2x + tx, gy = o2y + ty;
+        if (gx >= 0 && gy >= 0 && gx < L2.cols && gy < L2.rows)
+        {
+            const int v = pyr_tap(t1, F1P, o1x, o1y, gx, gy, L1.cols, L1.rows);
+            t2[ty * F2P + tx] = (uint8_t)v;
+            if (gx >= 2 * x3 && gx < 2 * x3 + 2 * T3 && gy >= 2 * y3 && gy < 2 * y3 + 2 * T3)
+                const_cast<uint8_t*>(L2.img)[(long)gy * L2.step + gx] = (uint8_t)v;
+        }
+    }
+    __syncthreads();
+    if (tid < T3 * T3)
+    {
+        const int gx = x3 + (tid % T3), gy = y3 + (tid / T3);
+        if (gx < L3.cols && gy < L3.rows)
+            const_cast<uint8_t*>(L3.img)[(long)gy * L3.step + gx] = (uint8_t)pyr_tap(t2, F2P, o2x, o2y, gx, gy, L2.cols, L2.rows);
+    }
+}
+
+}
diff --git a/livevisionkit_amd/csrc/stab_lookahead.hip b/livevisionkit_amd/csrc/stab_lookahead.hip
--- a/livevisionkit_amd/csrc/stab_lookahead.hip
+++ b/livevisionkit_amd/csrc/stab_lookahead.hip
@@ -48,6 +48,7 @@
 }
 
 long long lvk_hip_stab_lookahead_frames(lvk_hip_stab* st) { return st ? (long long)st->lookahead_frames : 0; }
+long long lvk_hip_stab_detect_frame_launches(lvk_hip_stab* st) { return st ? (long long)st->detect_frame_launches : 0; }
 
 int lvk_hip_stab_prefetch_cancel(lvk_hip_stab* st)
 {
diff --git a/livevisionkit_amd/csrc/stab_state.hpp b/livevisionkit_amd/csrc/stab_state.hpp
--- a/livevisionkit_amd/csrc/stab_state.hpp
+++ b/livevisionkit_amd/csrc/stab_state.hpp
@@ -38,7 +38,7 @@
 
 struct HostTrace
 {
-    enum { ENTER, DOWN_PYR_LAUNCH, FAST_SYNC, GRID, LK_LAUNCH, LK_SYNC, FILTER, RANSAC_LAUNCH, RANSAC_SYNC, POST, SMOOTH, REMAP_LAUNCH, EXIT, EMIT_WAITS, EMIT_KERNEL, EMIT_EVENT, EXIT_PRE, EXIT_WAIT, N };
+    enum { ENTER, DOWN_LAUNCH, PYR_LAUNCH, PLAN, PYR_LATE, FAST_SYNC, GRID, LK_LAUNCH, LK_SYNC, FILTER, RANSAC_LAUNCH, RANSAC_SYNC, POST, SMOOTH, REMAP_LAUNCH, EXIT, EMIT_WAITS, EMIT_KERNEL, EMIT_EVENT, EXIT_PRE, EXIT_WAIT, N };
     bool on = std::getenv("LVK_HIP_HOST_TRACE") != nullptr;
     double acc[N] = {0}; long cnt[N] = {0};
     std::chrono::steady_clock::time_point last;
@@ -52,13 +52,13 @@
     void dump() const
     {
         if (!on) return;
-        static const char* names[N] = {"enter", "downscale+pyramid launch", "fast launch+sync", "grid (host)", "lk upload+launch", "lk sync", "filter (host)",
+        static const char* names[N] = {"enter", "downscale launch", "pyramid launch", "post+plan (host), detect-frame push", "post+plan (host), late pyramid launch", "fast launch+sync", "grid (host)", "lk upload+launch", "lk sync", "filter (host)",
                                        "ransac upload+launch", "ransac sync", "post (host)", "qa+smoother (host)", "remap launch", "exit",
                                        "  emit: stream waits", "  emit: remap kernel launch", "  emit: slot event record", "  exit: up to the conversion wait", "  exit: conversion wait"};
-        double total = 0; long frames = cnt[DOWN_PYR_LAUNCH] ? cnt[DOWN_PYR_LAUNCH] : 1;
+        double total = 0; long frames = cnt[DOWN_LAUNCH] ? cnt[DOWN_LAUNCH] : 1;
         for (int i = 0; i < N; i++) total += acc[i];
         std::fprintf(stderr, "[lvk host trace] %ld frames, %.1f us/frame inside push\n", frames, total / frames);
-        for (int i = 0; i < N; i++) if (cnt[i]) std::fprintf(stderr, "  %-28s %8.1f us/frame (%ld marks)\n", names[i], acc[i] / frames, cnt[i]);
+        for (int i = 0; i < N; i++) if (cnt[i]) std::fprintf(stderr, "  %-40s %8.1f us/frame (%ld marks, %.1f us each)\n", names[i], acc[i] / frames, cnt[i], acc[i] / cnt[i]);
     }
 };
 
@@ -114,6 +114,7 @@
     uint32_t* h_occ = nullptr; uint32_t* h_new_kp = nullptr; int* h_insert = nullptr;
     bool device_grid = [] { const char* e = std::getenv("LVK_HIP_HOST_GRID"); return !(e && e[0] == '1'); }();
     long device_grid_frames = 0, host_grid_frames = 0;
+    long detect_frame_launches = 0;
     float2* d_und = nullptr;
     uint32_t* h_fast_out = nullptr; int* h_fast_counts = nullptr; FastRegion* h_regions = nullptr;
     float2 *h_pts = nullptr, *h_matched = nullptr, *h_p1 = nullptr; uint8_t* h_status = nullptr;
@@ -228,6 +229,7 @@
     void tracker_restart();
     void reset_context() { tracker_restart(); smoother.restart(); }
     int post_n = -1, post_m = 0;
+    size_t post_inliers = 0;
     bool post_error = false;
     void finish_post();
     int track(const QueuedFrame& f, const void* luma, int luma_step, int luma_pix, int luma_channel, WarpMeshF& motion, bool& have_motion);
diff --git a/livevisionkit_amd/csrc/stabilizer.hip b/livevisionkit_amd/csrc/stabilizer.hip
--- a/livevisionkit_amd/csrc/stabilizer.hip
+++ b/livevisionkit_amd/csrc/stabilizer.hip
@@ -24,15 +24,29 @@
         pe = prof_begin(LVK_STAGE_DOWNSCALE);
         if ((rc = lvk_launch_luma_area_resize(ctx, luma, luma_step, luma_pix, luma_channel, f.rows, f.cols, const_cast<uint8_t*>(C.args.lv[0].img), C.args.lv[0].step, cur_h, cur_w)) != LVK_HIP_OK) return rc;
         prof_end(pe);
-        pe = prof_begin(LVK_STAGE_PYRAMID);
-        if ((rc = C.build(ctx)) != LVK_HIP_OK) return rc;
-        prof_end(pe);
-    }
-    trace.mark(HostTrace::DOWN_PYR_LAUNCH);
+    }
+    trace.mark(HostTrace::DOWN_LAUNCH);
+    bool pyramid_due = !built_ahead;
+    auto build_pyramid = [&]() -> int
+    {
+        if (!pyramid_due) return LVK_HIP_OK;
+        pyramid_due = false;
+        const int e = prof_begin(LVK_STAGE_PYRAMID);
+        const int r = C.build(ctx);
+        if (r == LVK_HIP_OK) prof_end(e);
+        return r;
+    };
+    const bool expect_detection = pyramid_due && initialized && device_grid && C.args.nlevels == 4 && grid.likely_due(post_n >= 0, (size_t)std::max(post_n, 0), post_inliers);
+    if (!expect_detection) { if ((rc = build_pyramid()) != LVK_HIP_OK) return rc; trace.mark(HostTrace::PYR_LAUNCH); }
     finish_post();
-    if (post_error) { post_error = false; return fail(LVK_HIP_ERR_RUNTIME, "GPU-side fast_filter disagrees with the host's"); }
+    if (post_error) { post_error = false; (void)build_pyramid(); return fail(LVK_HIP_ERR_RUNTIME, "GPU-side fast_filter disagrees with the host's"); }
     auto leave_early = [&]() -> int { if (luma_pix != 3) LVK_HIP_CHECK(ctx, hipStreamSynchronize(st)); return LVK_HIP_OK; };
-    if (!initialized || cur_w != prev_w || cur_h != prev_h) { initialized = true; return leave_early(); }
+    if (!initialized || cur_w != prev_w || cur_h != prev_h)
+    {
+        if ((rc = build_pyramid()) != LVK_HIP_OK) return rc;
+        initialized = true;
+        return leave_early();
+    }
 
     grid.plan(plan);
     bool any = false;
@@ -42,6 +56,9 @@
     const bool dev_insert = any && device_grid && grid.device_insert_ok() && (int)plan.size() <= LVK_FAST_INLINE_REGIONS &&
                             lvk_fast_insert_fits((int)grid.capacity(), (int)plan.size(), fast_max_rw, fast_max_rh, cur_w, cur_h) && n_bound >= 1 && n_bound <= 4096;
     float distribution = 0.0f;
+    const bool fuse = dev_insert && pyramid_due && C.args.nlevels == 4;
+    if (fuse) { pyramid_due = false; trace.mark(HostTrace::PLAN); }
+    else if (pyramid_due) { if ((rc = build_pyramid()) != LVK_HIP_OK) return rc; trace.mark(HostTrace::PYR_LATE); }
     if (dev_insert)
     {
         for (size_t i = 0; i < n_held; i++) h_pts[i] = make_float2(grid.held[i].x, grid.held[i].y);
@@ -51,9 +68,10 @@
                                s.min_motion_samples, s.uniformity_threshold, HOMOGRAPHY_DISTRIBUTION_THRESHOLD, h_pts, h_new_kp, h_insert, d_n_points, d_full, h_fast_counts};
         pe = prof_begin(LVK_STAGE_FAST);
         if ((rc = lvk_launch_fast_insert(ctx, C.args.lv[0].img, C.args.lv[0].step, cur_h, cur_w, h_regions, (int)plan.size(), fast_max_rw, fast_max_rh,
-                                         d_fast_masks, d_fast_scores, d)) != LVK_HIP_OK) return rc;
+                                         d, fuse ? &C.args : nullptr)) != LVK_HIP_OK) { if (fuse) (void)C.build(ctx); return rc; }
         prof_end(pe);
         device_grid_frames++;
+        if (fuse) detect_frame_launches++;
     }
     else
     {
@@ -196,7 +214,7 @@
         for (int i = 0; i < m; i++) inliers += h_mask[i] ? 1 : 0;
         tracking_stability = (float)inliers / (float)m;
         have_motion = true;
-        post_n = n; post_m = m;
+        post_n = n; post_m = m; post_inliers = inliers;
         trace.mark(HostTrace::POST);
         return LVK_HIP_OK;
     }
diff --git a/livevisionkit_amd/stabilization.py b/livevisionkit_amd/stabilization.py
--- a/livevisionkit_amd/stabilization.py
+++ b/livevisionkit_amd/stabilization.py
@@ -303,6 +303,9 @@
     def lookahead_frames(self):
         return int(self.lib.lvk_hip_stab_lookahead_frames(self.handle))
 
+    def detect_frame_launches(self):
+        return int(self.lib.lvk_hip_stab_detect_frame_launches(self.handle))
+
     def prefetch_cancel(self):
         self.ctx._check(self.lib.lvk_hip_stab_prefetch_cancel(self.handle))
 
```

Result: no change. 9773 (-0.8%).
